# CILAB-MA/gpudrive_lab

Measured on AMD Instinct MI355X. Metric: agent-steps/sec at 1024 worlds x 64 agents; achieved HBM GB/s on obs kernel, higher is better.
Workload: dtype f32

## Files before the change

gpudrive_lab_amd/csrc/engine.cpp:

```cpp
#include <hip/hip_runtime.h>

#include <algorithm>
#include <cmath>
#include <cstdlib>
#include <cstdio>
#include <cstring>
#include <map>
#include <memory>
#include <stdexcept>
#include <atomic>
#include <exception>
#include <string>
#include <thread>
#include <vector>

#include "dev_mem.hpp"
#include "engine.hpp"
#include "gd_math.hpp"
#include "scene.hpp"
#ifdef GD_CLOCKS
namespace gd { void set_clocks_read(unsigned long long *out); void step_clocks_read(unsigned long long *out); }
#endif
#ifndef GD_GRID_MIN_CELL
#define GD_GRID_MIN_CELL 16.f
// ... 724 lines not shown
        d.pack_weights = rows ? weights : nullptr;
    }

    bool direct_pack_supported() const {
        if (params.disableClassicalObs) return false;
        if (params.roadObservationAlgorithm != GD_ROADS_K_NEAREST) return d.lin_on != 0;
        return true;
    }

    static void build_road_grid(WorldHost &world) {
        const std::vector<float> &xy = world.xy;
        const size_t n = xy.size() / 2;
        gd::GridHdr g{0.f, 0.f, 1.f, 1, 1, 0, 0, 0};
        std::vector<int32_t> off(2, 0);
        std::vector<uint16_t> items(n);
        if (n) {
            float minx = xy[0], maxx = xy[0], miny = xy[1], maxy = xy[1];
            for (size_t r = 1; r < n; r++) {
                minx = std::min(minx, xy[2 * r]); maxx = std::max(maxx, xy[2 * r]);
                miny = std::min(miny, xy[2 * r + 1]); maxy = std::max(maxy, xy[2 * r + 1]);
            }
            const float cell = std::max(GD_GRID_MIN_CELL, std::max(maxx - minx, maxy - miny) / 64.f + 1e-3f);
            g.ox = minx; g.oy = miny; g.inv_cell = 1.f / cell;
            g.nx = std::max(1, std::min(64, static_cast<int>((maxx - minx) * g.inv_cell) + 1));
            g.ny = std::max(1, std::min(64, static_cast<int>((maxy - miny) * g.inv_cell) + 1));
            const int nc = g.nx * g.ny;
            std::vector<int32_t> cell_of(n);
            off.assign(nc + 1, 0);
            for (size_t r = 0; r < n; r++) {
                const int cx = std::max(0, std::min(g.nx - 1, static_cast<int>((xy[2 * r] - g.ox) * g.inv_cell)));
                const int cy = std::max(0, std::min(g.ny - 1, static_cast<int>((xy[2 * r + 1] - g.oy) * g.inv_cell)));
                cell_of[r] = cy * g.nx + cx;
                off[cell_of[r] + 1]++;
            }
            for (int c = 0; c < nc; c++) off[c + 1] += off[c];
            std::vector<int32_t> fill(off.begin(), off.end() - 1);
            for (size_t r = 0; r < n; r++) items[fill[cell_of[r]]++] = static_cast<uint16_t>(r);
        }
        world.rgrid = g;
        world.rcell_off = std::move(off);
        world.rcell_items = std::move(items);
    }

    void upload_road_grids() {
        size_t ncell = 0, nitem = 0;
        std::vector<gd::GridHdr> hdr(W);
        for (int w = 0; w < W; w++) {
            world_host[w].rgrid.cell_base = static_cast<int>(ncell);
            world_host[w].rgrid.item_base = static_cast<int>(nitem);
            hdr[w] = world_host[w].rgrid;
            ncell += world_host[w].rcell_off.size();
            nitem += world_host[w].rcell_items.size();
        }
        rcell_off.fit(ncell, d.rcell_off);
        rcell_items.fit(nitem, d.rcell_items);
        rcell_xy.fit(nitem, d.rcell_xy);
        rcell_pos.fit(nitem, d.rcell_pos);
        std::vector<int32_t> co(ncell);
        std::vector<uint16_t> ci(nitem);
        std::vector<float> cxy(nitem * 2);
        std::vector<uint16_t> cpos(nitem);
        for (int w = 0; w < W; w++) {
            const WorldHost &x = world_host[w];
            std::copy(x.rcell_off.begin(), x.rcell_off.end(), co.begin() + hdr[w].cell_base);
            std::copy(x.rcell_items.begin(), x.rcell_items.end(), ci.begin() + hdr[w].item_base);
            for (size_t k = 0; k < x.rcell_items.size(); k++) {
                const size_t r = x.rcell_items[k], o = (static_cast<size_t>(hdr[w].item_base) + k) * 2;
                cxy[o] = x.xy[2 * r];
                cxy[o + 1] = x.xy[2 * r + 1];
                cpos[static_cast<size_t>(hdr[w].item_base) + r] = static_cast<uint16_t>(k);
            }
        }
        rcell_off.upload(co.data(), ncell);
        rcell_items.upload(ci.data(), nitem);
        rcell_xy.upload(cxy.data(), nitem);
        rcell_pos.upload(cpos.data(), nitem);
        HIP_CHECK(hipMemcpy(d_rgrid, hdr.data(), sizeof(gd::GridHdr) * W, hipMemcpyHostToDevice));
        std::vector<float> prev(static_cast<size_t>(W) * A * 4, 0.f);
        for (size_t i = 0; i < static_cast<size_t>(W) * A; i++) prev[i * 4 + 2] = INFINITY;
        HIP_CHECK(hipMemcpy(d.knn_prev, prev.data(), prev.size() * sizeof(float), hipMemcpyHostToDevice));
    }

    void reset_rank_state() {
        HIP_CHECK(hipMemset(d.cp_hdr, 0, sizeof(float4) * 2 * static_cast<size_t>(W) * A));
        HIP_CHECK(hipMemset(d.rk_fallback, 0, sizeof(int32_t) * (static_cast<size_t>(W) * A / 32)));
        HIP_CHECK(hipMemset(d.rk_streak, 0, sizeof(int32_t) * (static_cast<size_t>(W) * A / 32)));
        HIP_CHECK(hipMemset(d.rk_hist, 0, sizeof(int32_t) * GD_RANK_AUDIT));
        HIP_CHECK(hipMemset(d.rk_hist + GD_RH_LONG, 0, sizeof(int32_t) * (GD_RH_SIZE - GD_RH_LONG)));
    }

    void do_reset(const std::vector<int32_t> &flags) {
        upload_flags(d.reset_flags, flags);
        reset_flagged(false);
    }

    void reset_flagged(bool gated) {
        d.gate_any = gated ? 1 : 0;
        if (!gated) full_pass_next = false;
        try {
            launch(gd::KERNEL_RESET, false);
            run_rest(false);
        } catch (...) {
            d.gate_any = 0;
            throw;
        }
        d.gate_any = 0;
    }
};

namespace {

template <typename F>
int guarded(F &&f) {
    try {
        f();
        return GD_OK;
    } catch (const HipError &e) {
        return fail(GD_ERR_DEVICE, e.what());
    } catch (const std::invalid_argument &e) {
        const std::string m = e.what();
        return fail(m.find("cannot open") != std::string::npos ? GD_ERR_IO : GD_ERR_INVALID, m);
    } catch (const std::exception &e) {
        return fail(GD_ERR_PARSE, e.what());
    }
}

}

extern "C" {

const char *gd_version(void) { return "gpudrive_amd 0.1 (gfx950)"; }
const char *gd_last_error(void) { return g_last_error.c_str(); }

void gd_default_params(gd_params *p) {
    std::memset(p, 0, sizeof(*p));
    p->collisionBehaviour = GD_COLLISION_AGENT_STOP;
    p->maxNumControlledAgents = 10000;
    p->IgnoreNonVehicles = 0;
    p->roadObservationAlgorithm = GD_ROADS_K_NEAREST;
    p->initOnlyValidAgentsAtFirstStep = 1;
    p->isStaticAgentControlled = 0;
    p->dynamicsModel = GD_DYNAMICS_CLASSIC;
}

int gd_tensor_shape(int32_t id, int32_t W, int32_t A, gd_tensor_desc *out) {
    if (!out || id < 0 || id >= GD_T_COUNT || W < 1 || A < 2) return fail(GD_ERR_INVALID, "gd_tensor_shape: bad argument");
    const TensorSpec s = tensor_spec(id, W, A);
    out->data = nullptr;
    out->dtype = s.dtype;
    out->ndim = s.ndim;
    for (int i = 0; i < 5; i++) out->dims[i] = i < s.ndim ? s.dims[i] : 1;
    out->nbytes = spec_bytes(s);
    return GD_OK;
}

int gd_create(const gd_config *cfg, const gd_params *params, const char *const *scenes, gd_sim **out) {
    if (!cfg || !params || !scenes || !out) return fail(GD_ERR_INVALID, "gd_create: null argument");
    if (cfg->num_worlds < 1) return fail(GD_ERR_INVALID, "gd_create: num_worlds must be >= 1");
    if (cfg->max_agents != 64 && cfg->max_agents != 128)
        return fail(GD_ERR_INVALID, "gd_create: max_agents must be 64 or 128");
    if (params->rewardType == GD_REWARD_DENSE)
        return fail(GD_ERR_UNSUPPORTED, "RewardType::Dense is assert(false) in the reference (src/sim.cpp:579-583)");
    *out = nullptr;
    std::unique_ptr<gd_sim> s(new gd_sim());
    const int rc = guarded([&]() {
        int ndev = 0;
        HIP_CHECK(hipGetDeviceCount(&ndev));
        if (ndev < 1) throw HipError("no HIP device visible: the HIP path is mandatory, there is no CPU fallback");
        HIP_CHECK(hipSetDevice(cfg->device_id));
        s->cfg = *cfg;
        s->params = *params;
        s->W = cfg->num_worlds;
        s->A = cfg->max_agents;
        s->stream = static_cast<hipStream_t>(cfg->stream);
        const int W = s->W, A = s->A;
        for (int w = 0; w < W; w++) {
            if (!scenes[w]) throw std::invalid_argument("gd_create: null scene path");
            s->scenes.emplace_back(scenes[w]);
        }
        s->deleted.assign(static_cast<size_t>(W) * A, -1);
        s->world_host.resize(W);
        for (int id = 0; id < GD_T_COUNT; id++) {
            if (id == GD_T_BEV && !cfg->alloc_bev && !cfg->external[id]) continue;
            const int64_t bytes = spec_bytes(tensor_spec(id, W, A));
            if (!cfg->external[id]) s->exported_mem[id] = gd::DevMem(bytes);
            s->exported[id] = cfg->external[id] ? cfg->external[id] : s->exported_mem[id].get();
            HIP_CHECK(hipMemset(s->exported[id], 0, bytes));
        }
        gd::DevSim &d = s->d;
        d.W = W;
        d.A = A;
        d.p = *params;
        d.knn_order = cfg->knn_order;
        d.split_partner = (s->stream != nullptr && std::getenv("GPUDRIVE_SPLIT_PARTNER") != nullptr) ? 1 : 0;
        hipStream_t side = nullptr;
        HIP_CHECK(hipStreamCreateWithFlags(&side, hipStreamNonBlocking));
        s->side.reset(side);
        s->ev_fork = make_event(hipEventDisableTiming);
        s->ev_join = make_event(hipEventDisableTiming);
        d.step_dbg = 0;
#ifdef GD_DIAG
        if (const char *e = std::getenv("GPUDRIVE_STEP_DBG")) d.step_dbg = std::atoi(e);
#endif
        {
            (void)hipDeviceGetAttribute(&s->cu_count, hipDeviceAttributeMultiprocessorCount, cfg->device_id);
            d.set_fused_rows = 0;
            d.set_apw = 16;
        }
        d.lidar_half_angle = cfg->lidar_half_angle;
        {
            const float r = params->observationRadius;
            float k = r * r;
            while (k > 0.f && sqrtf(k) > r) k = std::nextafterf(k, 0.f);
            while (sqrtf(std::nextafterf(k, INFINITY)) <= r) k = std::nextafterf(k, INFINITY);
            d.radius_key_max = r >= 0.f ? k : -1.f;
        }
        d.action = static_cast<float *>(s->exported[GD_T_ACTION]);
        d.reward = static_cast<float *>(s->exported[GD_T_REWARD]);
        d.done = static_cast<int32_t *>(s->exported[GD_T_DONE]);
        d.info = static_cast<int32_t *>(s->exported[GD_T_INFO]);
        d.self_obs = static_cast<float *>(s->exported[GD_T_SELF_OBS]);
        d.abs_obs = static_cast<float *>(s->exported[GD_T_ABS_OBS]);
        d.partner = static_cast<float *>(s->exported[GD_T_PARTNER_OBS]);
        d.agent_map = static_cast<float *>(s->exported[GD_T_AGENT_MAP_OBS]);
        d.map_obs = static_cast<float *>(s->exported[GD_T_MAP_OBS]);
        d.lidar = static_cast<float *>(s->exported[GD_T_LIDAR]);
        d.bev = static_cast<float *>(s->exported[GD_T_BEV]);
        d.steps = static_cast<uint32_t *>(s->exported[GD_T_STEPS_REMAINING]);
        d.shape = static_cast<int32_t *>(s->exported[GD_T_SHAPE]);
        d.controlled = static_cast<int32_t *>(s->exported[GD_T_CONTROLLED_STATE]);
        d.resp_export = static_cast<int32_t *>(s->exported[GD_T_RESPONSE_TYPE]);
        d.traj = static_cast<float *>(s->exported[GD_T_EXPERT_TRAJECTORY]);
        d.means = static_cast<float *>(s->exported[GD_T_WORLD_MEANS]);
        d.metadata = static_cast<int32_t *>(s->exported[GD_T_METADATA]);
        d.deleted = static_cast<int32_t *>(s->exported[GD_T_DELETED_AGENTS]);
        d.map_name = static_cast<int32_t *>(s->exported[GD_T_MAP_NAME]);
        d.scenario_id = static_cast<int32_t *>(s->exported[GD_T_SCENARIO_ID]);
        const size_t WA = static_cast<size_t>(W) * A;
        d.px = s->alloc_internal<float>(WA); d.py = s->alloc_internal<float>(WA); d.pz = s->alloc_internal<float>(WA);
        d.qw = s->alloc_internal<float>(WA); d.qz = s->alloc_internal<float>(WA);
        d.vx = s->alloc_internal<float>(WA); d.vy = s->alloc_internal<float>(WA); d.vz = s->alloc_internal<float>(WA);
        d.collided = s->alloc_internal<int32_t>(WA);
        d.len = s->alloc_internal<float>(WA); d.wid = s->alloc_internal<float>(WA); d.hgt = s->alloc_internal<float>(WA);
        d.sc0 = s->alloc_internal<float>(WA); d.sc1 = s->alloc_internal<float>(WA);
        d.goal_x = s->alloc_internal<float>(WA); d.goal_y = s->alloc_internal<float>(WA);
        d.etype = s->alloc_internal<int32_t>(WA); d.agent_id = s->alloc_internal<int32_t>(WA);
        d.resp = s->alloc_internal<int32_t>(WA);
        d.sel_idx = s->alloc_internal<uint16_t>(static_cast<size_t>(WA) * GD_MAP_OBS_K);
        d.sel_hdr = s->alloc_internal<float4>(static_cast<size_t>(WA) * 2);
        d.sel_slot = s->alloc_internal<uint8_t>(static_cast<size_t>(WA) * GD_MAP_OBS_K);
        d.reset_flags = s->alloc_internal<int32_t>(W);
        d.rebuilt_flags = s->alloc_internal<int32_t>(W);
        d.any_reset = s->alloc_internal<int32_t>(1);
        d.gate_any = 0;
        d.road_off = s->d_road_off = s->alloc_internal<int32_t>(W + 1);
        d.live_list = s->alloc_internal<int32_t>(WA);
        d.live_count = 0;
        d.set_groups = s->alloc_internal<int32_t>(WA);
        d.set_group_count = 0;
        d.wave_order = s->alloc_internal<int32_t>(static_cast<size_t>(W) * (A / GD_MAP_OBS_AW));
        d.wave_cost = s->alloc_internal<uint32_t>(static_cast<size_t>(W) * (A / GD_MAP_OBS_AW));
        d.box_off = s->d_box_off = s->alloc_internal<int32_t>(W + 1);
        d.grid = s->d_grid = s->alloc_internal<gd::GridHdr>(W);
        d.rgrid = s->d_rgrid = s->alloc_internal<gd::GridHdr>(W);
        d.knn_prev = s->alloc_internal<float4>(WA);
        d.road_bbox = s->d_road_bbox = s->alloc_internal<float4>(W);
        d.road_rbmax = s->d_road_rbmax = s->alloc_internal<float>(W);
        d.bev_dirty = s->alloc_internal<int32_t>(WA);
        d.bev_list = s->alloc_internal<int32_t>(WA);
        d.bev_count = s->alloc_internal<int32_t>(2);
        d.bev_all_dirty = 0;
        HIP_CHECK(hipMemset(d.bev_dirty, 1, sizeof(int32_t) * WA));
        d.lidar_dirty = s->alloc_internal<int32_t>(WA);
        d.lidar_head = s->alloc_internal<float>(WA);
        HIP_CHECK(hipMemset(d.lidar_dirty, 1, sizeof(int32_t) * WA));
        HIP_CHECK(hipMemset(d.lidar_head, 0xff, sizeof(float) * WA));
        d.lin_apw = 2;
        if (const char *e = std::getenv("GPUDRIVE_LIN_AGENTS_PER_WAVE")) d.lin_apw = std::min(A / 4, std::max(1, std::atoi(e)));
        s->lin_cap = (static_cast<size_t>(W) + 64) * static_cast<size_t>(A) + 8 * 4 * static_cast<size_t>(d.lin_apw) + 64;
        s->d_lin_list = s->alloc_internal<int32_t>(s->lin_cap);
        s->d_lin_list_dyn = s->alloc_internal<int32_t>(s->lin_cap);
        d.lin_list = s->d_lin_list; d.lin_list_dyn = s->d_lin_list_dyn;
        d.lin_blocks = 0; d.lin_blocks_dyn = 0; d.lin_dyn_off = 0;
        d.lin_on = std::getenv("GPUDRIVE_LINEAR_LEGACY") == nullptr ? 1 : 0;
        d.pose_stamp = s->alloc_internal<uint4>(WA);
        d.pose_skip = std::getenv("GPUDRIVE_NO_POSE_SKIP") == nullptr ? 1 : 0;
        d.stat_skipped = s->alloc_internal<unsigned long long>(GD_SKIP_SLOTS);
        s->d_row_of_slot = s->alloc_internal<int32_t>(WA);
        s->d_slot_of_row = s->alloc_internal<int32_t>(WA);
        s->d_row_count = s->alloc_internal<int32_t>(1);
        d.bad_actions = s->alloc_internal<unsigned long long>(1);
        d.blk_off = s->d_blk_off = s->alloc_internal<int32_t>(W + 1);
        d.warm_k = 0;
        d.warm_all = 0;
        d.warm_flags = s->alloc_internal<int32_t>(W);
        d.warm_count = s->alloc_internal<unsigned long long>(1);
        d.rk_on = 0;
        d.rk_dbg = 0;
        d.rk_min_roads = 1536;
        d.rk_waves = 0;
        if (const char *e = std::getenv("GPUDRIVE_RANK_WAVES")) d.rk_waves = std::min(std::max((std::atoi(e) + 7) / 8 * 8, 8), GD_RANK_GRID);
        d.rk_scan_rows = 0;
        if (const char *e = std::getenv("GPUDRIVE_RANK_SCAN_ROWS")) d.rk_scan_rows = std::atoi(e) != 0 ? 1 : 0;
        d.rk_resident = std::max(gd::rank_resident_waves(A) / 8, 1);
        s->rk_possible = GD_MAP_OBS_AW == 32 && cfg->knn_order != GD_KNN_SET_ORDER &&
                         params->roadObservationAlgorithm == GD_ROADS_K_NEAREST && std::getenv("GPUDRIVE_NO_RANK_REPLAY") == nullptr;
#ifdef GD_DIAG
        if (const char *e = std::getenv("GPUDRIVE_RANK_DBG")) d.rk_dbg = std::atoi(e);
#endif
        for (int i = 0; i < gd_sim::kRing; i++) {
            void *pinned = nullptr;
            HIP_CHECK(hipHostMalloc(&pinned, sizeof(int32_t) * W, hipHostMallocDefault));
            s->h_flags[i].reset(static_cast<int32_t *>(pinned));
            s->flag_ev[i] = make_event(hipEventDisableTiming);
        }
        std::vector<int> all(W);
        for (int w = 0; w < W; w++) all[w] = w;
        s->rebuild_worlds(all);
        s->do_reset(std::vector<int32_t>(W, 1));
        HIP_CHECK(hipStreamSynchronize(s->stream));
    });
    if (rc != GD_OK) return rc;
    *out = s.release();
    return GD_OK;
}

void gd_destroy(gd_sim *sim) { delete sim; }

int gd_step(gd_sim *s) {
    if (!s) return fail(GD_ERR_INVALID, "gd_step: null sim");
    return guarded([&]() { s->step(); });
}

int gd_reset(gd_sim *s, const int32_t *idx, int32_t n) {
    if (!s || (n > 0 && !idx)) return fail(GD_ERR_INVALID, "gd_reset: bad argument");
    std::vector<int32_t> flags(s->W, 0);
    for (int i = 0; i < n; i++) {
        if (idx[i] < 0 || idx[i] >= s->W) return fail(GD_ERR_INVALID, "gd_reset: world index out of range");
        flags[idx[i]] = 1;
    }
    return guarded([&]() { s->do_reset(flags); });
}

int gd_set_maps(gd_sim *s, const char *const *scenes, int32_t n) {
    if (!s || !scenes) return fail(GD_ERR_INVALID, "gd_set_maps: null argument");
    if (n != s->W) return fail(GD_ERR_INVALID, "gd_set_maps: len(maps) must equal the number of worlds");
    const std::vector<std::string> old_scenes = s->scenes;
    const std::vector<int32_t> old_deleted = s->deleted;
    const int rc = guarded([&]() {
        for (int w = 0; w < n; w++) {
            if (!scenes[w]) throw std::invalid_argument("gd_set_maps: null scene path");
            s->scenes[w] = scenes[w];
        }
        std::fill(s->deleted.begin(), s->deleted.end(), -1);
        std::vector<int> all(s->W);
        for (int w = 0; w < s->W; w++) all[w] = w;
        s->rebuild_worlds(all);
        s->do_reset(std::vector<int32_t>(s->W, 1));
    });
    if (rc != GD_OK && rc != GD_ERR_DEVICE) {
        s->scenes = old_scenes;
        s->deleted = old_deleted;
    }
    return rc;
}

int gd_delete_agents(gd_sim *s, const int32_t *worlds, const int32_t *offsets, const int32_t *ids, int32_t nw) {
    if (!s || (nw > 0 && (!worlds || !offsets))) return fail(GD_ERR_INVALID, "gd_delete_agents: null argument");
    std::vector<int> touched;
    for (int i = 0; i < nw; i++) {
        const int w = worlds[i], cnt = offsets[i + 1] - offsets[i];
        if (w < 0 || w >= s->W) return fail(GD_ERR_INVALID, "gd_delete_agents: world index out of range");
        if (cnt < 0 || cnt > s->A) return fail(GD_ERR_INVALID, "gd_delete_agents: too many ids for one world");
    }
    return guarded([&]() {
        for (int i = 0; i < nw; i++) {
            const int w = worlds[i], cnt = offsets[i + 1] - offsets[i];
            for (int k = 0; k < cnt; k++) s->deleted[static_cast<size_t>(w) * s->A + k] = ids[offsets[i] + k];
            touched.push_back(w);
        }
        s->rebuild_worlds(touched);
        s->do_reset(std::vector<int32_t>(s->W, 1));
    });
}

int gd_tensor(gd_sim *s, int32_t id, gd_tensor_desc *out) {
    if (!s || !out || id < 0 || id >= GD_T_COUNT) return fail(GD_ERR_INVALID, "gd_tensor: bad argument");
    if (!s->exported[id]) return fail(GD_ERR_UNSUPPORTED, "tensor not allocated (set gd_config.alloc_bev for the BEV tensor)");
    gd_tensor_shape(id, s->W, s->A, out);
    out->data = s->exported[id];
    return GD_OK;
}

int gd_pack_observations(gd_sim *s, float *out, int64_t out_bytes) {
    if (!s || !out) return fail(GD_ERR_INVALID, "gd_pack_observations: null argument");
    const int64_t D = 6 + static_cast<int64_t>(s->A - 1) * 6 + GD_MAP_OBS_K * 13;
    const int64_t need = static_cast<int64_t>(s->W) * s->A * D * 4;
    if (out_bytes < need) return fail(GD_ERR_INVALID, "gd_pack_observations: output buffer too small");
    if (s->d.pack && s->d.pack_rows && s->d.pack_only)
        return fail(GD_ERR_UNSUPPORTED, "gd_pack_observations: learner rows are attached with only = 1: the raw rows are stale");
    return guarded([&]() {
        if (s->d.pack && !s->d.pack_rows) {
            if (out != s->d.pack) HIP_CHECK(hipMemcpyAsync(out, s->d.pack, need, hipMemcpyDeviceToDevice, s->stream));
            return;
        }
        gd::launch_pack_obs(s->d, s->stream, out);
        HIP_CHECK(hipGetLastError());
    });
}

int gd_attach_packed(gd_sim *s, float *out, int64_t out_bytes, int32_t only) {
    if (!s) return fail(GD_ERR_INVALID, "gd_attach_packed: null sim");
    const int64_t D = 6 + static_cast<int64_t>(s->A - 1) * 6 + GD_MAP_OBS_K * 13;
    if (out && out_bytes < static_cast<int64_t>(s->W) * s->A * D * 4)
        return fail(GD_ERR_INVALID, "gd_attach_packed: output buffer too small");
    if (out && !s->direct_pack_supported())
        return fail(GD_ERR_UNSUPPORTED, "gd_attach_packed: not available with disableClassicalObs or GPUDRIVE_LINEAR_LEGACY=1: use gd_pack_observations");
    return guarded([&]() {
        if (!out) s->detach_packed();
        else s->attach_packed(out, only != 0, false);
    });
}

int gd_set_learner_rows(gd_sim *s, const uint8_t *mask, int32_t n_rows) {
    if (!s) return fail(GD_ERR_INVALID, "gd_set_learner_rows: null sim");
    const size_t WA = static_cast<size_t>(s->W) * s->A;
    if (mask && (n_rows < 0 || static_cast<size_t>(n_rows) > WA))
        return fail(GD_ERR_INVALID, "gd_set_learner_rows: n_rows out of range");
    int32_t count = 0;
    const int rc = guarded([&]() {
        if (s->d.pack && s->d.pack_rows) s->detach_packed();
        HIP_CHECK(hipStreamSynchronize(s->stream));
        s->drop_graph();
        s->d.row_of_slot = nullptr;
        s->d.slot_of_row = nullptr;
        s->d.n_rows = 0;
        if (!mask) return;
        gd::launch_learner_rows(s->stream, mask, WA, s->d_row_of_slot, s->d_slot_of_row, s->d_row_count);
        HIP_CHECK(hipGetLastError());
        HIP_CHECK(hipMemcpyAsync(&count, s->d_row_count, sizeof(count), hipMemcpyDeviceToHost, s->stream));
        HIP_CHECK(hipStreamSynchronize(s->stream));
    });
    if (rc != GD_OK || !mask) return rc;
    if (count != n_rows) return fail(GD_ERR_INVALID, "gd_set_learner_rows: n_rows differs from the number of true slots of the mask");
    s->d.row_of_slot = s->d_row_of_slot;
    s->d.slot_of_row = s->d_slot_of_row;
    s->d.n_rows = count;
    return GD_OK;
}

int gd_attach_packed_rows(gd_sim *s, float *out, int64_t out_bytes, int32_t only) {
    if (!s || !out) return fail(GD_ERR_INVALID, "gd_attach_packed_rows: null argument (gd_attach_packed(sim, NULL, 0, 0) detaches)");
    if (!s->d.row_of_slot) return fail(GD_ERR_INVALID, "gd_attach_packed_rows: no learner rows set (gd_set_learner_rows)");
    const int64_t D = 6 + static_cast<int64_t>(s->A - 1) * 6 + GD_MAP_OBS_K * 13;
    if (out_bytes < static_cast<int64_t>(s->d.n_rows) * D * 4) return fail(GD_ERR_INVALID, "gd_attach_packed_rows: output buffer too small");
    if (!s->direct_pack_supported())
        return fail(GD_ERR_UNSUPPORTED, "gd_attach_packed_rows: not available with disableClassicalObs or GPUDRIVE_LINEAR_LEGACY=1");
    return guarded([&]() { s->attach_packed(out, only != 0, true); });
}

int gd_attach_packed_rows_conditioned(gd_sim *s, float *out, int64_t out_bytes, int32_t only, const float *weights) {
    if (!s || !out || !weights)
        return fail(GD_ERR_INVALID, "gd_attach_packed_rows_conditioned: null argument (gd_attach_packed(sim, NULL, 0, 0) detaches)");
    if (!s->d.row_of_slot) return fail(GD_ERR_INVALID, "gd_attach_packed_rows_conditioned: no learner rows set (gd_set_learner_rows)");
    const int64_t R = 6 + static_cast<int64_t>(s->A - 1) * 6 + GD_MAP_OBS_K * 13 + 3;
    if (out_bytes < static_cast<int64_t>(s->d.n_rows) * R * 4)
        return fail(GD_ERR_INVALID, "gd_attach_packed_rows_conditioned: output buffer too small");
    if (!s->direct_pack_supported())
        return fail(GD_ERR_UNSUPPORTED, "gd_attach_packed_rows_conditioned: not available with disableClassicalObs or GPUDRIVE_LINEAR_LEGACY=1");
    return guarded([&]() { s->attach_packed(out, only != 0, true, weights); });
}

int gd_set_discrete_actions(gd_sim *s, const int64_t *indices, const float *table, int32_t n_actions) {
    if (!s) return fail(GD_ERR_INVALID, "gd_set_discrete_actions: null sim");
    if (s->d.p.dynamicsModel == GD_DYNAMICS_STATE)
        return fail(GD_ERR_UNSUPPORTED, "gd_set_discrete_actions: the State dynamics model has no discrete action space");
    if (!s->d.row_of_slot) return fail(GD_ERR_INVALID, "gd_set_discrete_actions: no learner rows set (gd_set_learner_rows)");
    if (n_actions < 0 || (s->d.n_rows > 0 && (!indices || !table)))
        return fail(GD_ERR_INVALID, "gd_set_discrete_actions: bad argument");
    return guarded([&]() {
        gd::launch_discrete_actions(s->d, s->stream, indices, table, n_actions);
        HIP_CHECK(hipGetLastError());
    });
}

int gd_pack_observations_conditioned(gd_sim *s, const float *weights, float *out, int64_t out_bytes) {
    if (!s || !weights || !out) return fail(GD_ERR_INVALID, "gd_pack_observations_conditioned: null argument");
    const int64_t R = 6 + static_cast<int64_t>(s->A - 1) * 6 + GD_MAP_OBS_K * 13 + 3;
    if (out_bytes < static_cast<int64_t>(s->W) * s->A * R * 4)
        return fail(GD_ERR_INVALID, "gd_pack_observations_conditioned: output buffer too small");
    if (s->d.pack && s->d.pack_rows && s->d.pack_only)
        return fail(GD_ERR_UNSUPPORTED, "gd_pack_observations_conditioned: learner rows are attached with only = 1: the raw rows are stale");
    return guarded([&]() {
        gd::launch_pack_obs_conditioned(s->d, s->stream, weights, out);
        HIP_CHECK(hipGetLastError());
    });
}

int gd_expert_actions(gd_sim *s, float *actions, int32_t action_cols, float *pos_xy, float *vel_xy, float *yaw,
                      int32_t *valids) {
    if (!s) return fail(GD_ERR_INVALID, "gd_expert_actions: null sim");
    const int cols = s->d.p.dynamicsModel == GD_DYNAMICS_STATE ? 10 : 3;
    if (actions && action_cols != cols)
        return fail(GD_ERR_INVALID, "gd_expert_actions: action_cols does not match the dynamics model (10 for State, else 3)");
    return guarded([&]() {
        gd::launch_expert_actions(s->d, s->stream, actions, pos_xy, vel_xy, yaw, valids);
        HIP_CHECK(hipGetLastError());
    });
}

int gd_advance_log_playback(gd_sim *s, int32_t init_steps) {
    if (!s) return fail(GD_ERR_INVALID, "gd_advance_log_playback: null sim");
    if (init_steps < 0 || init_steps >= GD_EPISODE_LEN)
        return fail(GD_ERR_INVALID, "gd_advance_log_playback: the expert trajectory has 91 steps, init_steps must be < 91");
    return guarded([&]() {
        for (int t = 0; t < init_steps; t++) {
            gd::launch_set_log_actions(s->d, s->stream, t);
            HIP_CHECK(hipGetLastError());
            s->step();
        }
    });
}

int gd_record_expert(gd_sim *s, const gd_record_buffers *b, int32_t n_steps) {
    if (!s || !b) return fail(GD_ERR_INVALID, "gd_record_expert: null argument");
    if (!b->row_slot || !b->obs || !b->actions || !b->dead_mask || !b->partner_mask || !b->road_mask || !b->ego_global_pos ||
        !b->ego_global_rot || !b->dead || !b->goal_achieved || !b->off_road || !b->veh_collision || !b->any_alive)
        return fail(GD_ERR_INVALID, "gd_record_expert: every buffer is required");
    if (b->n_rows < 0) return fail(GD_ERR_INVALID, "gd_record_expert: n_rows must be >= 0");
    if (n_steps < 1 || n_steps > GD_EPISODE_LEN)
        return fail(GD_ERR_INVALID, "gd_record_expert: the expert trajectory has 91 steps, n_steps must be in [1, 91]");
    if (s->d.p.dynamicsModel == GD_DYNAMICS_STATE)
        return fail(GD_ERR_INVALID, "gd_record_expert: the State dynamics model's actions have 10 columns, the dataset's have 3");
    if (s->d.pack && s->d.pack_only)
        return fail(GD_ERR_UNSUPPORTED, "gd_record_expert: a packed buffer is attached with only = 1: the raw rows are stale");
    return guarded([&]() {
        std::vector<Event> ev;
        auto mark = [&]() {
            if (!b->kernel_ms) return;
            ev.push_back(make_event());
            HIP_CHECK(hipEventRecord(ev.back().get(), s->stream));
        };
        for (int t = 0; t <= n_steps; t++) {
            mark();
            gd::launch_record(s->d, s->stream, *b, t, t < n_steps);
            HIP_CHECK(hipGetLastError());
            mark();
            if (t == n_steps) break;
            gd::launch_set_log_actions(s->d, s->stream, t);
            HIP_CHECK(hipGetLastError());
            s->step();
        }
        if (b->kernel_ms) {
            HIP_CHECK(hipStreamSynchronize(s->stream));
            float sum = 0.f;
            for (size_t i = 0; i + 1 < ev.size(); i += 2) {
                float ms = 0.f;
                HIP_CHECK(hipEventElapsedTime(&ms, ev[i].get(), ev[i + 1].get()));
                sum += ms;
            }
            *b->kernel_ms = sum;
        }
    });
}

namespace {

const char *il_dataset_error(const gd_il_dataset *ds, int64_t *rows) {
    if (!ds) return "null argument";
    if (ds->max_agents != 64 && ds->max_agents != 128) return "max_agents must be 64 or 128";
    if (ds->rollout_len < 1 || ds->pred_len < 1 || ds->rollout_len + ds->pred_len > GD_EPISODE_LEN)
        return "rollout_len >= 1, pred_len >= 1 and rollout_len + pred_len <= 91 are required";
    if (ds->n_shards < 0 || ds->n_shards > GD_IL_MAX_SHARDS) return "0 to 8 shards";
    *rows = 0;
    for (int i = 0; i < ds->n_shards; i++) {
        const gd_il_shard &sh = ds->shard[i];
        if (sh.n_rows < 0) return "a shard's n_rows must be >= 0";
        if (!sh.obs || !sh.actions || !sh.dead_mask || !sh.partner_mask || !sh.road_mask || !sh.keep)
            return "every array of every shard is required";
        if (reinterpret_cast<uintptr_t>(sh.obs) % 16 != 0 || reinterpret_cast<uintptr_t>(sh.road_mask) % 8 != 0)
            return "obs must be 16-byte aligned and road_mask 8-byte aligned";
        *rows += sh.n_rows;
    }
    if (*rows > INT32_MAX / GD_EPISODE_LEN) return "too many rows";
    return nullptr;
}

}

int gd_il_index(const gd_il_dataset *ds, int32_t *counts, int32_t *kept, const int64_t *entry_offset, const int64_t *kept_ordinal,
                int32_t *entries, void *stream) {
    int64_t rows = 0;
    if (const char *e = il_dataset_error(ds, &rows)) return fail(GD_ERR_INVALID, std::string("gd_il_index: ") + e);
    if (entries ? (!entry_offset || !kept_ordinal) : (!counts || !kept))
        return fail(GD_ERR_INVALID, "gd_il_index: counts and kept (first launch) or entry_offset, kept_ordinal and entries "
                                    "(second launch) are required");
    return guarded([&]() {
        gd::launch_il_index(*ds, static_cast<hipStream_t>(stream), rows, counts, kept, entry_offset, kept_ordinal, entries);
        HIP_CHECK(hipGetLastError());
    });
}

int gd_il_batch(const gd_il_dataset *ds, const gd_il_batch_buffers *b, void *stream) {
    int64_t rows = 0;
    if (const char *e = il_dataset_error(ds, &rows)) return fail(GD_ERR_INVALID, std::string("gd_il_batch: ") + e);
    if (!b) return fail(GD_ERR_INVALID, "gd_il_batch: null argument");
// ... 700 lines not shown
        gd::launch_bc_train_rows(o, st, n, o.nll, o.actions, expert_actions, o.grad_nll);
        gd::launch_bc_backward(*p, *g, st, obs, partner_mask, road_mask, n, expert_actions, o.grad_nll, nullptr, o.grad);
        gd::launch_bc_adamw(o, st, o.grad);
        HIP_CHECK(hipGetLastError());
    });
}

int gd_bc_eval_accumulate(int32_t n, const float *nll, const float *actions, const float *expert_actions, float *acc, void *stream) {
    if (!nll || !actions || !expert_actions || !acc) return fail(GD_ERR_INVALID, "gd_bc_eval_accumulate: null argument");
    if (n < 1 || n > (1 << 20)) return fail(GD_ERR_INVALID, "gd_bc_eval_accumulate: n must be in [1, 2^20]");
    if (misaligned(nll, 4) || misaligned(actions, 4) || misaligned(expert_actions, 4) || misaligned(acc, 4))
        return fail(GD_ERR_INVALID, "gd_bc_eval_accumulate: float buffers must be 4-byte aligned");
    return guarded([&]() {
        gd::launch_bc_eval_accumulate(static_cast<hipStream_t>(stream), n, nll, actions, expert_actions, acc);
        HIP_CHECK(hipGetLastError());
    });
}

int gd_bc_hidden(const gd_bc_policy *p, const float *obs, const uint8_t *partner_mask, const uint8_t *road_mask, int32_t n, int32_t tap,
                 float *out, void *stream) {
    gd_bc_outputs none{};
    const char *why = bc_forward_problem(p, obs, partner_mask, road_mask, n, 1, nullptr, nullptr, nullptr, &none);
    if (!why && tap != GD_LP_TAP_FUSION && tap != GD_LP_TAP_RO) why = "tap must be GD_LP_TAP_FUSION or GD_LP_TAP_RO";
    if (!why && (!out || misaligned(out, 16))) why = "out is required, 16-byte aligned";
    if (why) return fail(GD_ERR_INVALID, std::string("gd_bc_hidden: ") + why);
    return guarded([&]() {
        gd::launch_bc_hidden(*p, static_cast<hipStream_t>(stream), obs, partner_mask, road_mask, n, tap, out);
        HIP_CHECK(hipGetLastError());
    });
}

static const char *lp_problem(const gd_bc_policy *p, const gd_lp_probe *lp, const float *obs, const uint8_t *partner_mask,
                              const uint8_t *road_mask, int32_t n, const uint8_t *mask, const int64_t *labels, const gd_lp_rows *rows,
                              int mode, const int32_t *acc) {
    if (!lp || !obs) return "null argument";
    if (lp->model < GD_LP_EARLY || lp->model > GD_LP_BASELINE) return "model must be GD_LP_EARLY, GD_LP_LATE or GD_LP_BASELINE";
    if (lp->exp != GD_IL_FUTURE_OTHER && lp->exp != GD_IL_FUTURE_EGO) return "exp must be GD_IL_FUTURE_OTHER or GD_IL_FUTURE_EGO";
    if (lp->reserved[0] != 0 || lp->reserved[1] != 0) return "reserved must be 0";
    if (lp->max_agents != 64 && lp->max_agents != 128) return "max_agents must be 64 or 128";
    if (lp->num_stack < 1 || lp->num_stack > 8) return "num_stack must be in [1, 8]";
    if (lp->model == GD_LP_BASELINE) {
        if (p) return "the baseline probe takes no policy";
        if (n < 1 || n > (1 << 20)) return "n must be in [1, 2^20]";
        if (misaligned(obs, 4)) return "float and int32 buffers must be 4-byte aligned";
        const int k = (lp->exp == GD_IL_FUTURE_OTHER ? 12 : 6) * lp->num_stack;
        if (k > 64) return "the baseline probe's in_features (12 num_stack for 'other') must not exceed 64";
        if (lp->in_features != k) return "in_features must be 6 num_stack ('ego') or 12 num_stack ('other') for the baseline probe";
    } else {
        gd_bc_outputs none{};
        if (const char *why = bc_forward_problem(p, obs, partner_mask, road_mask, n, 1, nullptr, nullptr, nullptr, &none)) return why;
        if (lp->max_agents != p->max_agents || lp->num_stack != p->num_stack) return "max_agents and num_stack must be the policy's";
        if (lp->in_features != 64) return "in_features must be 64 with a policy";
    }
    if (lp->num_partials < 1 || lp->num_partials > 4096) return "num_partials must be in [1, 4096]";
    if (!lp->packed || misaligned(lp->packed, 16)) return "packed is required, 16-byte aligned";
    if (rows && (misaligned(rows->logits, 16) || misaligned(rows->loss_row, 4) || misaligned(rows->pred, 8)))
        return "logits must be 16-byte aligned, loss_row 4-byte, pred 8-byte";
    if (mode == 0) {
        if (!rows || (!rows->logits && !rows->pred)) return "rows with logits or pred is required";
        if (rows->loss_row) return "loss_row needs labels (gd_lp_update, gd_lp_eval_accumulate)";
        return nullptr;
    }
    if (!mask || !labels || misaligned(labels, 8)) return "mask and labels are required, labels 8-byte aligned";
    if (!lp->part_f || !lp->part_d || !lp->part_i || misaligned(lp->part_f, 4) || misaligned(lp->part_d, 8) || misaligned(lp->part_i, 4))
        return "part_f, part_d and part_i are required (4-, 8- and 4-byte aligned)";
    if (misaligned(lp->stats, 4)) return "float and int32 buffers must be 4-byte aligned";
    if (mode == 2) return !acc || misaligned(acc, 8) ? "acc is required, 8-byte aligned" : nullptr;
    if (!(lp->beta1 >= 0.0 && lp->beta1 < 1.0) || !(lp->beta2 >= 0.0 && lp->beta2 < 1.0)) return "betas must be in [0, 1)";
    if (!(lp->eps > 0.f)) return "eps must be positive";
    if (!(lp->weight_decay >= 0.f) || !std::isfinite(lp->weight_decay)) return "weight_decay must be finite and not negative";
    if (!lp->weight || !lp->exp_avg || !lp->exp_avg_sq || !lp->lr || !lp->step || !lp->beta_pow || !lp->grad || !lp->stats || !lp->sums ||
        !lp->counts || !lp->scal)
        return "weight, exp_avg, exp_avg_sq, lr, step, beta_pow, grad, stats, sums, counts and scal are required";
    if (misaligned(lp->beta_pow, 8) || misaligned(lp->sums, 8) || misaligned(lp->weight, 4) || misaligned(lp->exp_avg, 4) ||
        misaligned(lp->exp_avg_sq, 4) || misaligned(lp->lr, 4) || misaligned(lp->step, 4) || misaligned(lp->grad, 4) ||
        misaligned(lp->counts, 4) || misaligned(lp->scal, 4))
        return "beta_pow and sums must be 8-byte aligned, the other buffers 4-byte aligned";
    return nullptr;
}

int gd_lp_forward(const gd_bc_policy *p, const gd_lp_probe *lp, const float *obs, const uint8_t *partner_mask, const uint8_t *road_mask,
                  int32_t n, const gd_lp_rows *rows, void *stream) {
    if (const char *why = lp_problem(p, lp, obs, partner_mask, road_mask, n, nullptr, nullptr, rows, 0, nullptr))
        return fail(GD_ERR_INVALID, std::string("gd_lp_forward: ") + why);
    return guarded([&]() {
        gd::launch_lp(p, *lp, static_cast<hipStream_t>(stream), obs, partner_mask, road_mask, n, nullptr, nullptr, rows, 0, nullptr);
        HIP_CHECK(hipGetLastError());
    });
}

int gd_lp_update(const gd_bc_policy *p, const gd_lp_probe *lp, const float *obs, const uint8_t *partner_mask, const uint8_t *road_mask,
                 int32_t n, const uint8_t *mask, const int64_t *labels, const gd_lp_rows *rows, void *stream) {
    if (const char *why = lp_problem(p, lp, obs, partner_mask, road_mask, n, mask, labels, rows, 1, nullptr))
        return fail(GD_ERR_INVALID, std::string("gd_lp_update: ") + why);
    return guarded([&]() {
        gd::launch_lp(p, *lp, static_cast<hipStream_t>(stream), obs, partner_mask, road_mask, n, mask, labels, rows, 1, nullptr);
        HIP_CHECK(hipGetLastError());
    });
}

int gd_lp_eval_accumulate(const gd_bc_policy *p, const gd_lp_probe *lp, const float *obs, const uint8_t *partner_mask,
                          const uint8_t *road_mask, int32_t n, const uint8_t *mask, const int64_t *labels, const gd_lp_rows *rows,
                          int32_t *acc, void *stream) {
    if (const char *why = lp_problem(p, lp, obs, partner_mask, road_mask, n, mask, labels, rows, 2, acc))
        return fail(GD_ERR_INVALID, std::string("gd_lp_eval_accumulate: ") + why);
    return guarded([&]() {
        gd::launch_lp(p, *lp, static_cast<hipStream_t>(stream), obs, partner_mask, road_mask, n, mask, labels, rows, 2, acc);
        HIP_CHECK(hipGetLastError());
    });
}

int gd_episode_step(gd_sim *s, const gd_episode_config *cfg, const gd_episode_buffers *b) {
    if (!s || !cfg || !b) return fail(GD_ERR_INVALID, "gd_episode_step: null argument");
    if (!b->controlled_mask || !b->agent_episode_returns || !b->episode_lengths || !b->collided_in_episode ||
        !b->offroad_in_episode || !b->live_agent_mask || !b->reward_out || !b->terminal_out || !b->truncated_out ||
        !b->mask_out || !b->done_worlds || !b->stats || !b->world_stats)
        return fail(GD_ERR_INVALID, "gd_episode_step: every buffer is required");
    if (cfg->reward_type < GD_EPISODE_REWARD_WEIGHTED || cfg->reward_type > GD_EPISODE_REWARD_LOG_DISTANCE)
        return fail(GD_ERR_INVALID, "gd_episode_step: unknown reward_type");
    if (cfg->reward_type == GD_EPISODE_REWARD_CONDITIONED && (!b->reward_weights || !b->weight_draws))
        return fail(GD_ERR_INVALID, "gd_episode_step: reward_conditioned needs reward_weights and weight_draws");
    if (cfg->reward_type == GD_EPISODE_REWARD_CONDITIONED &&
        (cfg->condition_mode < GD_CONDITION_RANDOM || cfg->condition_mode > GD_CONDITION_FIXED))
        return fail(GD_ERR_INVALID, "gd_episode_step: unknown condition_mode");
    if ((b->reward_rows || b->terminal_rows || b->truncated_rows || b->mask_rows) && !s->d.row_of_slot)
        return fail(GD_ERR_INVALID, "gd_episode_step: flat outputs need learner rows (gd_set_learner_rows)");
    return guarded([&]() {
        HIP_CHECK(hipMemsetAsync(s->d.any_reset, 0, sizeof(int32_t), s->stream));
        gd::launch_episode_step(s->d, s->stream, *cfg, *b);
        HIP_CHECK(hipGetLastError());
        if (cfg->auto_reset) s->reset_flagged(true);
    });
}

int gd_episode_set_warmup(gd_sim *s, int32_t init_steps, int32_t scope) {
    if (init_steps < 0 || init_steps >= GD_EPISODE_LEN)
        return fail(GD_ERR_INVALID, "gd_episode_set_warmup: init_steps must be in [0, 90] (the expert trajectory has 91 steps)");
    if (scope != GD_WARMUP_RESET_WORLDS && scope != GD_WARMUP_ALL_WORLDS)
        return fail(GD_ERR_INVALID, "gd_episode_set_warmup: unknown scope (GD_WARMUP_RESET_WORLDS or GD_WARMUP_ALL_WORLDS)");
    if (!s) return fail(GD_ERR_INVALID, "gd_episode_set_warmup: null sim");
    s->d.warm_k = init_steps;
    s->d.warm_all = scope == GD_WARMUP_ALL_WORLDS ? 1 : 0;
    return GD_OK;
}

int gd_episode_draw_weights(gd_sim *s, const gd_episode_config *cfg, const gd_episode_buffers *b, const int32_t *worlds,
                            int32_t n) {
    if (!s || !cfg || !b || !b->reward_weights || !b->weight_draws || (worlds && n < 0))
        return fail(GD_ERR_INVALID, "gd_episode_draw_weights: bad argument");
    if (cfg->condition_mode < GD_CONDITION_RANDOM || cfg->condition_mode > GD_CONDITION_FIXED)
        return fail(GD_ERR_INVALID, "gd_episode_draw_weights: unknown condition_mode");
    std::vector<int32_t> list;
    if (worlds) {
        list.assign(worlds, worlds + n);
        for (const int32_t w : list)
            if (w < 0 || w >= s->W) return fail(GD_ERR_INVALID, "gd_episode_draw_weights: world index out of range");
        std::sort(list.begin(), list.end());
        list.erase(std::unique(list.begin(), list.end()), list.end());
        if (list.empty()) return GD_OK;
    }
    return guarded([&]() {
        if (!worlds) {
            gd::launch_draw_weights(s->d, s->stream, *cfg, *b, nullptr, s->W);
            HIP_CHECK(hipGetLastError());
            return;
        }
        const gd::DevMem dl(list.size() * sizeof(int32_t));
        hipError_t e = hipMemcpyAsync(dl.get(), list.data(), list.size() * sizeof(int32_t), hipMemcpyHostToDevice, s->stream);
        if (e == hipSuccess) {
            gd::launch_draw_weights(s->d, s->stream, *cfg, *b, static_cast<const int32_t *>(dl.get()), static_cast<int>(list.size()));
            e = hipGetLastError();
        }
        const hipError_t es = hipStreamSynchronize(s->stream);
        HIP_CHECK(e);
        HIP_CHECK(es);
    });
}

int gd_sync(gd_sim *s) {
    if (!s) return fail(GD_ERR_INVALID, "gd_sync: null sim");
    return guarded([&]() { HIP_CHECK(hipStreamSynchronize(s->stream)); });
}

int gd_set_stream(gd_sim *s, void *stream) {
    if (!s) return fail(GD_ERR_INVALID, "gd_set_stream: null sim");
    return guarded([&]() {
        HIP_CHECK(hipStreamSynchronize(s->stream));
        s->drop_graph();
        HIP_CHECK(hipStreamSynchronize(s->side.get()));
        s->stream = static_cast<hipStream_t>(stream);
        s->d.split_partner = (s->stream != nullptr && std::getenv("GPUDRIVE_SPLIT_PARTNER") != nullptr) ? 1 : 0;
    });
}

int gd_attach_bev(gd_sim *s, float *bev) {
    if (!s || !bev) return fail(GD_ERR_INVALID, "gd_attach_bev: null argument");
    return guarded([&]() {
        if (s->d.bev && s->d.bev != bev) throw std::runtime_error("gd_attach_bev: a BEV tensor is already attached");
        HIP_CHECK(hipStreamSynchronize(s->stream));
        s->drop_graph();
        s->exported[GD_T_BEV] = bev;
        s->d.bev = bev;
        HIP_CHECK(hipMemsetAsync(s->d.bev_dirty, 1, sizeof(int32_t) * static_cast<size_t>(s->W) * s->A, s->stream));
        if (!s->params.disableClassicalObs) s->launch(gd::KERNEL_BEV, false);
    });
}

int gd_stat(gd_sim *s, int32_t which, int64_t *out) {
#ifdef GD_CLOCKS
    if (s && out && which >= 22 && which <= 29) {
        static unsigned long long clk[8];
        if (which == 22) gd::set_clocks_read(clk);
        *out = (int64_t)clk[which - 22];
        return GD_OK;
    }
#endif
#ifdef GD_CLOCKS
    if (s && out && which >= 32 && which <= 43) {
        static unsigned long long clk[12];
        if (which == 32) gd::step_clocks_read(clk);
        *out = (int64_t)clk[which - 32];
        return GD_OK;
    }
#endif
#ifdef GD_CLOCKS
    if (s && out && which >= 1000 && which < 1256) {
        *out = 0;
        if (s->rk_alloc) {
            int32_t v = 0;
            (void)hipStreamSynchronize(s->stream);
            if (hipMemcpy(&v, s->d.rk_hist + 256 + (which - 1000), sizeof(v), hipMemcpyDeviceToHost) != hipSuccess)
                return fail(GD_ERR_DEVICE, "gd_stat: reading the replay clocks failed");
            *out = v;
        }
        return GD_OK;
    }
#endif
#ifdef GD_WAVE_CLOCKS
    if (s && out && which >= 2000 && which < 2000 + 3 * GD_RANK_GRID) {
        *out = 0;
        if (s->rk_alloc) {
            int32_t v = 0;
            (void)hipStreamSynchronize(s->stream);
            if (hipMemcpy(&v, s->d.rk_hist + GD_RH_WAVES + (which - 2000), sizeof(v), hipMemcpyDeviceToHost) != hipSuccess)
                return fail(GD_ERR_DEVICE, "gd_stat: reading the ranking waves' clocks failed");
            *out = v;
        }
        return GD_OK;
    }
#endif
#if defined(GD_DIAG) || defined(GD_CLOCKS)
    constexpr int32_t kLastStat = 20;
#else
    constexpr int32_t kLastStat = 7;
#endif
    if (s && out && which == 30) {
        std::vector<unsigned long long> v(GD_SKIP_SLOTS, 0);
        (void)hipStreamSynchronize(s->stream);
        if (hipMemcpy(v.data(), s->d.stat_skipped, sizeof(unsigned long long) * v.size(), hipMemcpyDeviceToHost) != hipSuccess ||
            hipMemset(s->d.stat_skipped, 0, sizeof(unsigned long long) * v.size()) != hipSuccess)
            return fail(GD_ERR_DEVICE, "gd_stat: reading the skip counters failed");
        unsigned long long sum = 0;
        for (unsigned long long x : v) sum += x;
        *out = static_cast<int64_t>(sum) + s->host_skipped;
        s->host_skipped = 0;
        return GD_OK;
    }
    if (s && out && which == 31) {
        int32_t c = 0;
        (void)hipStreamSynchronize(s->stream);
        if (hipMemcpy(&c, s->d.bev_count, sizeof(c), hipMemcpyDeviceToHost) != hipSuccess)
            return fail(GD_ERR_DEVICE, "gd_stat: reading the raster count failed");
        *out = c;
        return GD_OK;
    }
    if (s && out && which == 44) {
        std::vector<int32_t> f(static_cast<size_t>(s->W) * s->A), n(static_cast<size_t>(s->W) * 2);
        (void)hipStreamSynchronize(s->stream);
        if (hipMemcpy(f.data(), s->d.lidar_dirty, sizeof(int32_t) * f.size(), hipMemcpyDeviceToHost) != hipSuccess ||
            hipMemcpy(n.data(), s->d.shape, sizeof(int32_t) * n.size(), hipMemcpyDeviceToHost) != hipSuccess)
            return fail(GD_ERR_DEVICE, "gd_stat: reading the LiDAR flags failed");
        int64_t c = 0;
        for (int w = 0; w < s->W; w++)
            for (int a = 0; a < n[static_cast<size_t>(w) * 2] && a < s->A; a++) c += f[static_cast<size_t>(w) * s->A + a] != 0;
        *out = c;
        return GD_OK;
    }
    if (s && out && which == 45) {
        unsigned long long v = 0;
        (void)hipStreamSynchronize(s->stream);
        if (hipMemcpy(&v, s->d.bad_actions, sizeof(v), hipMemcpyDeviceToHost) != hipSuccess)
            return fail(GD_ERR_DEVICE, "gd_stat: reading the action counter failed");
        *out = static_cast<int64_t>(v);
        return GD_OK;
    }
    if (s && out && which == 46) {
        unsigned long long v = 0;
        (void)hipStreamSynchronize(s->stream);
        if (hipMemcpy(&v, s->d.warm_count, sizeof(v), hipMemcpyDeviceToHost) != hipSuccess)
            return fail(GD_ERR_DEVICE, "gd_stat: reading the warm-up counter failed");
        *out = static_cast<int64_t>(v);
        return GD_OK;
    }
    if (s && out && which == 22) {
        *out = 0;
        if (s->rk_alloc) {
            int32_t v = 0;
            (void)hipStreamSynchronize(s->stream);
            if (hipMemcpy(&v, s->d.rk_hist + GD_RH_ROWS, sizeof(v), hipMemcpyDeviceToHost) != hipSuccess)
                return fail(GD_ERR_DEVICE, "gd_stat: reading the row counter failed");
            *out = v;
        }
        return GD_OK;
    }
    if (s && out && which == 21) {
        *out = 0;
        if (s->rk_alloc) {
            int32_t v = 0;
            (void)hipStreamSynchronize(s->stream);
            if (hipMemcpy(&v, s->d.rk_hist + GD_RANK_AUDIT, sizeof(v), hipMemcpyDeviceToHost) != hipSuccess)
                return fail(GD_ERR_DEVICE, "gd_stat: reading the audit counter failed");
            *out = v;
        }
        return GD_OK;
    }
    if (!s || !out || which < 0 || which > kLastStat) return fail(GD_ERR_INVALID, "gd_stat: bad argument");
#if defined(GD_DIAG) || defined(GD_CLOCKS)
    if (which >= 8) {
        *out = 0;
        if (s->rk_alloc) {
            int32_t v = 0;
            (void)hipStreamSynchronize(s->stream);
            (void)hipMemcpy(&v, s->d.rk_hist + 514 + (which - 8), sizeof(v), hipMemcpyDeviceToHost);
            (void)hipMemset(s->d.rk_hist + 514 + (which - 8), 0, sizeof(v));
            *out = v;
        }
        return GD_OK;
    }
#endif
    if (which == 7) {
        *out = s->d.rk_on;
        return GD_OK;
    }
    *out = which == 0 ? s->stat_graph_steps : which == 1 ? s->stat_plain_steps : which == 2 ? s->stat_captures
         : which == 3 ? s->d.set_fused_rows : which == 4 ? s->d.set_apw : which == 5 ? s->d.live_count : GD_MAP_OBS_AW;
    return GD_OK;
}

int gd_kernel_timing_enable(gd_sim *s, int32_t enable) {
    if (!s) return fail(GD_ERR_INVALID, "null sim");
    return guarded([&]() {
        HIP_CHECK(hipStreamSynchronize(s->stream));
        for (int k = 0; k < gd::KERNEL_TIMED; k++) {
            s->collect_timing(k);
            s->ev_ms[k] = 0;
            s->ev_launches[k] = 0;
            while (enable && s->ev_pool[k].size() < gd_sim::kEvRing) {
                s->ev_pool[k].push_back(EventPair{make_event(), make_event()});
            }
        }
        s->timing = enable != 0;
    });
}

int gd_kernel_timing_read(gd_sim *s, int32_t kernel, double *total_ms, int64_t *launches) {
    if (!s || kernel < 0 || kernel >= gd::KERNEL_TIMED) return fail(GD_ERR_INVALID, "gd_kernel_timing_read: bad argument");
    return guarded([&]() {
        HIP_CHECK(hipStreamSynchronize(s->stream));
        s->collect_timing(kernel);
        if (total_ms) *total_ms = s->ev_ms[kernel];
        if (launches) *launches = s->ev_launches[kernel];
    });
}

int gd_debug_get_state(gd_sim *s, float *out) {
    if (!s || !out) return fail(GD_ERR_INVALID, "null argument");
    return guarded([&]() {
        HIP_CHECK(hipStreamSynchronize(s->stream));
        const size_t WA = static_cast<size_t>(s->W) * s->A;
        std::vector<float> plane(WA);
        std::vector<int32_t> iplane(WA);
        const float *src[8] = {s->d.px, s->d.py, s->d.pz, s->d.qw, s->d.qz, s->d.vx, s->d.vy, s->d.vz};
        const int dstcol[8] = {0, 1, 2, 3, 6, 7, 8, 9};
        for (size_t i = 0; i < WA * 11; i++) out[i] = 0.f;
        for (int k = 0; k < 8; k++) {
            HIP_CHECK(hipMemcpy(plane.data(), src[k], WA * 4, hipMemcpyDeviceToHost));
            for (size_t i = 0; i < WA; i++) out[i * 11 + dstcol[k]] = plane[i];
        }
        for (size_t i = 0; i < WA; i++) {
            out[i * 11 + 4] = 0.f * out[i * 11 + 6];
            out[i * 11 + 5] = 0.f * out[i * 11 + 6];
        }
        HIP_CHECK(hipMemcpy(iplane.data(), s->d.collided, WA * 4, hipMemcpyDeviceToHost));
        for (size_t i = 0; i < WA; i++) out[i * 11 + 10] = static_cast<float>(iplane[i]);
    });
}

int gd_debug_road_path(gd_sim *s, int32_t *out) {
    if (!s || !out) return fail(GD_ERR_INVALID, "null argument");
    return guarded([&]() {
        HIP_CHECK(hipStreamSynchronize(s->stream));
        const size_t WA = static_cast<size_t>(s->W) * s->A;
        if (!s->rk_alloc || !s->d.rk_on) {
            for (size_t i = 0; i < WA; i++) out[i] = -2;
            return;
        }
        HIP_CHECK(hipMemcpy(out, s->d.rk_n, WA * sizeof(int32_t), hipMemcpyDeviceToHost));
        std::vector<int32_t> why(WA);
        HIP_CHECK(hipMemcpy(why.data(), s->d.rk_ticket, WA * sizeof(int32_t), hipMemcpyDeviceToHost));
        for (size_t i = 0; i < WA; i++) {
            if (out[i] > 0) out[i] = out[i] == (1 << 30) ? -3 : (out[i] & 0xffff);
            else if (out[i] == -1 && why[i] < -1) out[i] = -10 + (why[i] + 2);
            else if (out[i] == -1 && why[i] >= 0 && ((why[i] >> 30) & 1)) out[i] = -12;
        }
    });
}

int gd_debug_set_state(gd_sim *s, const float *in) {
    if (!s || !in) return fail(GD_ERR_INVALID, "null argument");
    return guarded([&]() {
        HIP_CHECK(hipStreamSynchronize(s->stream));
        const size_t WA = static_cast<size_t>(s->W) * s->A;
        std::vector<float> plane(WA);
        std::vector<int32_t> iplane(WA);
        float *dst[8] = {s->d.px, s->d.py, s->d.pz, s->d.qw, s->d.qz, s->d.vx, s->d.vy, s->d.vz};
        const int srccol[8] = {0, 1, 2, 3, 6, 7, 8, 9};
        for (int k = 0; k < 8; k++) {
            for (size_t i = 0; i < WA; i++) plane[i] = in[i * 11 + srccol[k]];
            HIP_CHECK(hipMemcpy(dst[k], plane.data(), WA * 4, hipMemcpyHostToDevice));
        }
        for (size_t i = 0; i < WA; i++) iplane[i] = in[i * 11 + 10] != 0.f;
        HIP_CHECK(hipMemcpy(s->d.collided, iplane.data(), WA * 4, hipMemcpyHostToDevice));
        s->full_pass_next = (s->params.roadObservationAlgorithm != GD_ROADS_K_NEAREST && s->d.lin_on != 0) || s->d.bev != nullptr ||
                            (s->d.lidar != nullptr && s->params.enableLidar);
    });
}

int gd_host_world_build(const char *scene, const gd_params *params, int32_t A, const int32_t *deleted, int32_t ndel,
                        gd_host_world *out) {
    if (!scene || !params || !out || A < 2 || A > GD_MAX_AGENTS_LIMIT) return fail(GD_ERR_INVALID, "gd_host_world_build: bad argument");
    std::memset(out, 0, sizeof(*out));
    return guarded([&]() {
        auto map = gd::load_scene(scene, params->polylineReductionThreshold);
        gd::HostWorld hw;
        gd::build_host_world(*map, *params, A, deleted, ndel, hw);
        out->num_agents = hw.num_agents;
        out->num_roads = hw.num_roads;
        out->num_collidable_roads = static_cast<int32_t>(hw.boxes.size());
        out->max_agents = A;
        std::memcpy(out->mean, hw.mean, sizeof(hw.mean));
        std::memcpy(out->map_name, hw.map_name, sizeof(hw.map_name));
        std::memcpy(out->scenario_id, hw.scenario_id, sizeof(hw.scenario_id));
        auto dupf = [](const std::vector<float> &v, size_t n) {
            float *p = static_cast<float *>(std::calloc(std::max<size_t>(n, 1), sizeof(float)));
            std::memcpy(p, v.data(), std::min(n, v.size()) * sizeof(float));
            return p;
        };
        auto dupi = [](const std::vector<int32_t> &v) {
            int32_t *p = static_cast<int32_t *>(std::calloc(std::max<size_t>(v.size(), 1), sizeof(int32_t)));
            std::memcpy(p, v.data(), v.size() * sizeof(int32_t));
            return p;
        };
        out->map_obs = dupf(hw.map_obs, static_cast<size_t>(GD_MAX_ROAD_ENTITIES) * 9);
        for (int r = hw.num_roads; r < GD_MAX_ROAD_ENTITIES; r++) { out->map_obs[r * 9 + 7] = -1.f; out->map_obs[r * 9 + 8] = -1.f; }
        out->trajectory = dupf(hw.trajectory, hw.trajectory.size());
        out->vehicle_size = dupf(hw.size, hw.size.size());
        out->goal = dupf(hw.goal, hw.goal.size());
        out->controlled = dupi(hw.controlled);
        out->response_type = dupi(hw.resp);
        out->agent_id = dupi(hw.agent_id);
        out->entity_type = dupi(hw.etype);
        out->metadata = dupi(hw.metadata);
    });
}

int gd_scene_cache_write(const char *scene, float polyline_reduction_threshold, const char *out_path) {
    if (!scene || !out_path) return fail(GD_ERR_INVALID, "gd_scene_cache_write: null argument");
    if (!gd::is_scene_cache_path(out_path)) return fail(GD_ERR_INVALID, "gd_scene_cache_write: the cache path must end in .gdsm");
    return guarded([&]() {
        auto map = gd::load_scene(scene, polyline_reduction_threshold);
        gd::write_scene_cache(*map, polyline_reduction_threshold, out_path);
    });
}

void gd_host_world_free(gd_host_world *w) {
    if (!w) return;
    std::free(w->map_obs); std::free(w->trajectory); std::free(w->vehicle_size); std::free(w->goal);
    std::free(w->controlled); std::free(w->response_type); std::free(w->agent_id); std::free(w->entity_type);
    std::free(w->metadata);
    std::memset(w, 0, sizeof(*w));
}

}
```

gpudrive_lab_amd/csrc/engine.hpp:

```cpp
#pragma once
#include <hip/hip_runtime.h>

#include <cstdint>

#include "../../include/gpudrive_amd.h"

#ifndef GD_MAP_OBS_AW
#define GD_MAP_OBS_AW 32
#endif

#define GD_RANK_CAP 1280
#define GD_RANK_NCP 40
#define GD_RANK_HEAP_DW 104
#define GD_RANK_CAP_LONG 2560
#define GD_RANK_KT_LONG 164
#define GD_RH_LONG 537
#define GD_RH_ROWS 538
#define GD_RH_CURSOR 544
#define GD_RH_CURSOR_STRIDE 32
#define GD_RH_SIZE (GD_RH_CURSOR + 8 * GD_RH_CURSOR_STRIDE)
#define GD_RANK_GRID (256 * 8 * 4)
#ifdef GD_CLOCKS
#define GD_WAVE_CLOCKS
#endif
#ifdef GD_WAVE_CLOCKS
#define GD_RH_WAVES GD_RH_SIZE
#define GD_RH_ALLOC (GD_RH_WAVES + 3 * GD_RANK_GRID)
#else
#define GD_RH_ALLOC GD_RH_SIZE
#endif
#define GD_RK_REC_ROW (1 << 16)
#define GD_RANK_NCH 320
#define GD_RANK_SPL 256
#define GD_RANK_KT 84
#define GD_RANK_AUDIT 536
#define GD_LIN_BLK 16
#define GD_SKIP_SLOTS 4096

#ifdef GD_DIAG
#define GD_DIAG_IS(field, value) ((field) == (value))
#else
#define GD_DIAG_IS(field, value) false
#endif

namespace gd {

enum { KERNEL_STATE = 0, KERNEL_MAP_OBS = 1, KERNEL_LIDAR = 2, KERNEL_BEV = 3, KERNEL_PARTNER = 4, KERNEL_RESET = 5, KERNEL_PADDING = 6, KERNEL_TIMED = 5 };

struct GridHdr {
    float ox, oy, inv_cell;
    int nx, ny;
    int cell_base;
    int item_base;
    int pad;
};

struct DevSim {
    int W, A;
    int knn_order;
    int set_fused_rows;
    int32_t *live_list;
    int live_count;
    int32_t *set_groups;
    int set_group_count;
    int set_apw;
    float lidar_half_angle;
    float radius_key_max;
    gd_params p;
    float *action, *reward, *self_obs, *abs_obs, *partner, *agent_map, *map_obs, *lidar, *bev, *traj, *means;
    int32_t *done, *info, *shape, *controlled, *resp_export, *metadata, *deleted, *map_name, *scenario_id;
    uint32_t *steps;
    float *px, *py, *pz, *qw, *qz, *vx, *vy, *vz;
    int32_t *collided;
    float *len, *wid, *hgt, *sc0, *sc1, *goal_x, *goal_y;
    int32_t *etype, *agent_id, *resp;
    uint16_t *sel_idx;
    float4 *sel_hdr;
    uint8_t *sel_slot;
    int32_t *reset_flags, *rebuilt_flags;
    int32_t *any_reset;
    int gate_any;
    const int32_t *road_off;
    int32_t *wave_order;
    uint32_t *wave_cost;
    const float2 *road_xy;
    const float4 *road_aux;
    const float4 *road_rec;
    const int32_t *box_off;
    const float4 *boxes;
    const GridHdr *grid;
    const int32_t *cell_off;
    const int32_t *cell_items;
    const float4 *cell_hdr;
    const GridHdr *rgrid;
    const int32_t *rcell_off;
    const uint16_t *rcell_items;
    const float2 *rcell_xy;
    const uint16_t *rcell_pos;
    float4 *knn_prev;
    const int32_t *lin_list, *lin_list_dyn;
    int lin_blocks, lin_blocks_dyn;
    int lin_dyn_off;
    const float4 *road_blk;
    const int32_t *blk_off;
    int lin_apw;
    int lin_on;
    uint4 *pose_stamp;
    int pose_skip;
    int32_t *bev_dirty;
    int32_t *bev_list;
    int32_t *bev_count;
    int bev_all_dirty;
    int32_t *lidar_dirty;
    float *lidar_head;
    float *pack;
    int pack_only;
    const int32_t *row_of_slot, *slot_of_row;
    int n_rows;
    int pack_rows;
    unsigned long long *bad_actions;
    unsigned long long *stat_skipped;
    int split_partner;
    int step_dbg;
    int rk_on;
    int rk_max_roads;
    int rk_min_roads;
    int rk_dbg;
    uint16_t *rk_E;
    int rk_nlong;
    int32_t *rk_longlist;
    int32_t *rk_longslot;
    uint16_t *rk_E_long;
    float *rk_kt_long;
    uint16_t *rk_spc;
    float *rk_kt;
    uint32_t *rk_heap;
    uint16_t *rk_cpe;
    int32_t *rk_hist;
    int rk_waves;
    int32_t *rk_ticket;
    int32_t *rk_order;
    int32_t *rk_list;
    uint16_t *rk_cpf;
    float *rk_cpt;
    float4 *rk_rec;
    int rk_scan_rows;
    int rk_resident;
    const float4 *road_bbox;
    const float *road_rbmax;
    int32_t *rk_n;
    int32_t *rk_fallback;
    int32_t *rk_streak;
    uint16_t *cp_road;
    float *cp_T;
    float4 *cp_hdr;
    int warm_k;
    int warm_all;
    int32_t *warm_flags;
    unsigned long long *warm_count;
    const float *pack_weights;
};

void launch_kernel(const DevSim &d, hipStream_t st, int which, bool move);
void launch_map_obs(const DevSim &d, hipStream_t st, bool move);
void launch_map_obs_rank(const DevSim &d, hipStream_t st);
int rank_resident_waves(int A);
void launch_map_obs_linear(const DevSim &d, hipStream_t st, bool move);
void launch_bev(const DevSim &d, hipStream_t st);
void launch_lidar(const DevSim &d, hipStream_t st);
void launch_pack_obs(const DevSim &d, hipStream_t st, float *out);
void launch_expert_actions(const DevSim &d, hipStream_t st, float *actions, float *pos, float *vel, float *yaw, int *valid);
void launch_set_log_actions(const DevSim &d, hipStream_t st, int t);
void launch_episode_step(const DevSim &d, hipStream_t st, const gd_episode_config &c, const gd_episode_buffers &b);
void launch_draw_weights(const DevSim &d, hipStream_t st, const gd_episode_config &c, const gd_episode_buffers &b,
                         const int32_t *worlds, int n);
void launch_pack_obs_rows(const DevSim &d, hipStream_t st, float *out,
                          const float *weights);
void launch_learner_rows(hipStream_t st, const uint8_t *mask, size_t slots, int32_t *row_of_slot, int32_t *slot_of_row,
                         int32_t *count);
void launch_discrete_actions(const DevSim &d, hipStream_t st, const int64_t *indices, const float *table, int n_actions);
void launch_pack_obs_conditioned(const DevSim &d, hipStream_t st, const float *weights, float *out);
void launch_record(const DevSim &d, hipStream_t st, const gd_record_buffers &b, int t, bool pre);
void launch_bc_rollout_row(const DevSim &d, hipStream_t st, const gd_bc_rollout_buffers &b, int t, int num_stack);
void launch_bc_rollout_actions(const DevSim &d, hipStream_t st, const gd_bc_rollout_buffers &b, int t);
void launch_bc_rollout_post(const DevSim &d, hipStream_t st, const gd_bc_rollout_buffers &b, int t, bool more);
void launch_bc_rollout_summary(hipStream_t st, const gd_bc_rollout_buffers &b);
void launch_policy_rollout_actions(const DevSim &d, hipStream_t st, const gd_policy_rollout_buffers &b, int t);
void launch_policy_rollout_book(const DevSim &d, hipStream_t st, const gd_policy_rollout_buffers &b, int t);
void launch_policy_rollout_finish(const DevSim &d, hipStream_t st, const gd_policy_rollout_buffers &b, int n_steps);
void launch_il_index(const gd_il_dataset &ds, hipStream_t st, int64_t rows, int32_t *counts, int32_t *kept,
                     const int64_t *entry_offset, const int64_t *kept_ordinal, int32_t *entries);
void launch_il_batch(const gd_il_dataset &ds, hipStream_t st, const gd_il_batch_buffers &b,
                     int split);
void launch_il_future(const gd_il_dataset &ds, const gd_il_future &fu, hipStream_t st, const gd_il_future_buffers &b,
                      int split);
void launch_rollout_store(const gd_rollout &ro, hipStream_t st, const float *obs, const float *value, const int64_t *action,
                          const float *logprob, const float *reward, const uint8_t *done, const uint8_t *mask,
                          bool streaming);
void launch_rollout_sort(const gd_rollout &ro, hipStream_t st, const int64_t *offset, int64_t *idxs);
void launch_rollout_gae(const gd_rollout &ro, hipStream_t st, const int64_t *idxs, float gamma, float gae_lambda, float *delta,
                        float *coef, float *adv);
void launch_rollout_gather(const gd_rollout &ro, hipStream_t st, const gd_rollout_batch &b);
long long policy_blob_floats(int ego_width, int n_actions);
void launch_policy_forward(const gd_policy &p, hipStream_t st, const float *obs, const float *u, bool deterministic,
                           int64_t *actions, float *logprob, float *entropy, float *value, float *logits_out);
void launch_policy_evaluate(const gd_policy &p, hipStream_t st, const float *obs, const int64_t *actions, unsigned char *winners,
                            float *logprob, float *entropy, float *value);
void launch_policy_forward(const gd_policy &p, const gd_dropout &d, hipStream_t st, const float *obs, const float *u,
                           bool deterministic, int64_t *actions, float *logprob, float *entropy, float *value,
                           float *logits_out);
void launch_policy_evaluate(const gd_policy &p, const gd_dropout &d, hipStream_t st, const float *obs, const int64_t *actions,
                            unsigned char *winners, float *logprob, float *entropy, float *value);
void launch_policy_forward_rows(const gd_policy &p, const gd_dropout *d, hipStream_t st, const float *obs, const float *u,
                                bool deterministic, int64_t *actions, float *logprob, float *entropy, float *value,
                                float *logits_out, const int32_t *rows, const int32_t *count);
void launch_live_rows(hipStream_t st, const uint8_t *mask, int n, int32_t *rows, int32_t *count, int32_t *scratch,
                      int32_t *count_copy);
void launch_policy_backward(const gd_policy &p, const gd_policy_grad &g, const gd_dropout &d, hipStream_t st, const float *obs,
                            const int64_t *actions, const float *d_logprob, const float *d_entropy, const float *d_value,
                            float *grad);
long long policy_grad_floats(int ego_width, int n_actions);
void launch_policy_backward(const gd_policy &p, const gd_policy_grad &g, hipStream_t st, const float *obs, const int64_t *actions,
                            const float *d_logprob, const float *d_entropy, const float *d_value, float *grad);
void launch_ppo_loss(const gd_ppo &o, hipStream_t st, const float *newlogprob, const float *entropy, const float *newvalue,
                     const float *old_logprob, const float *old_value, const float *adv, const float *ret, float *d_logprob,
                     float *d_entropy, float *d_value);
void launch_ppo_adam(const gd_ppo &o, hipStream_t st, const float *grad);
long long bc_blob_floats(int num_stack, int fusion_layers, int branch_layers, int head_layers, int n_components);
long long bc_scratch_floats(int max_agents, int chunk_rows);
void launch_bc_forward(const gd_bc_policy &p, hipStream_t st, const float *obs, const unsigned char *partner_mask,
                       const unsigned char *road_mask, int n, bool deterministic, const float *u, const float *z,
                       const float *expert_actions, const gd_bc_outputs &out);
void launch_bc_eval_accumulate(hipStream_t st, int n, const float *nll, const float *actions, const float *expert_actions,
                               float *acc);
void launch_bc_embed(const gd_bc_policy &p, hipStream_t st, const float *obs, int rows, float *X);
void launch_bc_self_layer(const gd_bc_policy &p, hipStream_t st, const unsigned char *pm, const unsigned char *rm, int rows,
                          int layer, float *X, float *Kb, float *Vb, float *osave, float *ml);
void launch_bc_cross_kv(const gd_bc_policy &p, hipStream_t st, int rows, const float *X, float *Kb, float *Vb);
void launch_bc_head(const gd_bc_policy &p, hipStream_t st, const unsigned char *partner_mask, const unsigned char *road_mask, int r0,
                    int rows, bool deterministic, const float *u, const float *z, const float *expert_actions,
                    const gd_bc_outputs &out, const float *X, const float *Kb, const float *Vb);
long long bc_grad_floats(int num_stack, int fusion_layers, int branch_layers, int head_layers, int n_components);
long long bc_grad_scratch_floats(int max_agents, int chunk_rows, int fusion_layers, int branch_layers, long long blob_floats);
void launch_bc_backward(const gd_bc_policy &p, const gd_bc_grad &g, hipStream_t st, const float *obs, const unsigned char *partner_mask,
                        const unsigned char *road_mask, int n, const float *expert_actions, const float *grad_nll, float *nll,
                        float *grad);
int bc_num_tensors(int fusion_layers, int branch_layers, int head_layers);
void launch_bc_train_rows(const gd_bc_opt &o, hipStream_t st, int n, const float *nll, const float *actions,
                          const float *expert_actions, float *grad_nll);
void launch_bc_adamw(const gd_bc_opt &o, hipStream_t st, const float *grad);
void launch_bc_hidden(const gd_bc_policy &p, hipStream_t st, const float *obs, const unsigned char *partner_mask,
                      const unsigned char *road_mask, int n, int tap, float *out);
void launch_lp(const gd_bc_policy *p, const gd_lp_probe &lp, hipStream_t st, const float *obs, const unsigned char *partner_mask,
               const unsigned char *road_mask, int n, const unsigned char *mask, const int64_t *labels, const gd_lp_rows *rows_out,
               int mode, int *acc);

}
```

gpudrive_lab_amd/csrc/kernels.hip:

```cpp
#include <hip/hip_runtime.h>

#include "engine.hpp"
#include "expert.hpp"
#include "gd_math.hpp"
#include "map_rows.hpp"
#include "pack_cols.hpp"

namespace gd {

namespace {

constexpr int K = GD_MAP_OBS_K;
constexpr int TRAJ = GD_TRAJECTORY_FLOATS;
constexpr int EPISODE = GD_EPISODE_LEN;

__device__ __forceinline__ int current_step(uint32_t t) {
    long long k = (long long)EPISODE - (long long)t;
    if (k < 0 || k > EPISODE) k = EPISODE;
    return (int)k;
}

struct Body {
    float px, py, pz, qw, qz, vx, vy, vz;
};

__device__ __forceinline__ void forward_classic(const float *act, float length, Body &b) {
    const float maxSpeed = FLT_MAX;
    const float dt = 0.1f;
    const float speed = len_3(b.vx, b.vy, b.vz);
    const float yaw = quat_to_yaw(quat_from_wz(b.qw, b.qz));
    const float v = fmaxf(fminf(speed + 0.5f * act[0] * dt, maxSpeed), -maxSpeed);
    const float tanDelta = p_tan(act[1]);
    const float beta = p_atan(0.5f * tanDelta);
    float sn, cs;
    p_sincos(yaw + beta, sn, cs);
    const float dx = v * cs, dy = v * sn;
    const float w = v * p_cos(beta) * tanDelta / length;
    const float new_yaw = angle_add(yaw, w * dt);
    const float new_speed = fmaxf(fminf(speed + act[0] * dt, maxSpeed), -maxSpeed);
    b.px += dx * dt;
    b.py += dy * dt;
    b.pz = 1.f;
    p_sincos(new_yaw / 2.f, b.qz, b.qw);
    p_sincos(new_yaw, sn, cs);
    b.vx = new_speed * cs;
    b.vy = new_speed * sn;
    b.vz = 0.f;
}

__device__ __forceinline__ void forward_bicycle(float *act, Body &b) {
    act[0] = fmaxf(-6.0f, fminf(act[0], 6.0f));
    act[1] = fmaxf(-3.0f, fminf(act[1], 3.0f));
    const float dt = 0.1f;
    const float yaw = quat_to_yaw(quat_from_wz(b.qw, b.qz));
    const float speed = len_3(b.vx, b.vy, b.vz);
    float sn, cs;
    p_sincos(yaw, sn, cs);
    b.px = (float)((double)(b.px + b.vx * dt) + 0.5 * act[0] * cs * dt * dt);
    b.py = (float)((double)(b.py + b.vy * dt) + 0.5 * act[0] * sn * dt * dt);
    const float delta_yaw = (float)(act[1] * ((double)(speed * dt) + 0.5 * act[0] * dt * dt));
    const float new_yaw = angle_add(yaw, delta_yaw);
    const float new_speed = speed + act[0] * dt;
    p_sincos(new_yaw, sn, cs);
    b.vx = new_speed * cs;
    b.vy = new_speed * sn;
    b.vz = 0.f;
    p_sincos(new_yaw / 2.f, b.qz, b.qw);
}

__device__ __forceinline__ void forward_delta(const float *act, Body &b) {
    const float dt = 0.1f;
    const float yaw = quat_to_yaw(quat_from_wz(b.qw, b.qz));
    float c, s;
    p_sincos(yaw, s, c);
    const float dx = act[0] * c - act[1] * s;
    const float dy = act[0] * s + act[1] * c;
    b.px = b.px + dx;
    b.py = b.py + dy;
    b.vx = dx / dt;
    b.vy = dy / dt;
    b.vz = 0.f;
    const float new_yaw = angle_add(yaw, act[2]);
    p_sincos(new_yaw / 2.f, b.qz, b.qw);
}

__device__ __forceinline__ void forward_state(const float *act, Body &b) {
    b.px = act[0]; b.py = act[1]; b.pz = act[2];
    b.vx = act[4]; b.vy = act[5]; b.vz = act[6];
    p_sincos(act[3] / 2.f, b.qz, b.qw);
}

__device__ __forceinline__ void reset_agent(const DevSim &d, size_t i) {
    const float *t = d.traj + i * TRAJ;
    d.px[i] = t[0];
    d.py[i] = t[1];
    d.pz[i] = 1.f;
    const float heading = t[4 * 91];
    d.qw[i] = p_cos(heading / 2.f);
    d.qz[i] = p_sin(heading / 2.f);
    const bool is_static = d.resp[i] == RESP_Static;
    d.vx[i] = is_static ? 0.f : t[2 * 91 + 0];
    d.vy[i] = is_static ? 0.f : t[2 * 91 + 1];
    d.vz[i] = 0.f;
    float *act = d.action + i * 10;
#pragma unroll
    for (int k = 0; k < 10; k++) act[k] = 0.f;
    if (d.p.dynamicsModel == GD_DYNAMICS_STATE) act[2] = 1.f;
    d.steps[i] = EPISODE;
    d.done[i] = 0;
    d.reward[i] = 0.f;
    int32_t *info = d.info + i * 5;
    info[0] = 0; info[1] = 0; info[2] = 0; info[3] = 0;
    info[4] = d.etype[i];
    d.resp_export[i] = d.resp[i];
    d.collided[i] = 0;
}

template <int A_T>
__global__ __launch_bounds__(A_T) void k_reset_worlds(DevSim d) {
    const int w = blockIdx.x, a = threadIdx.x;
    if (d.reset_flags[w] == 0) return;
    const int n = d.shape[w * 2 + 0];
    const size_t i = (size_t)w * A_T + a;
    if (a < n) reset_agent(d, i);
    __syncthreads();
    if (a == 0) d.reset_flags[w] = 0;
}

template <int A_T>
__global__ __launch_bounds__(A_T) void k_init_padding_rows(DevSim d) {
    const int w = blockIdx.x;
    if (d.rebuilt_flags[w] == 0) return;
    const int n = d.shape[w * 2 + 0];
    const int npad = A_T - n;
    for (int a = n + threadIdx.x; a < A_T; a += blockDim.x) {
        const size_t i = (size_t)w * A_T + a;
        d.steps[i] = 0;
        d.done[i] = 1;
        d.reward[i] = 0.f;
        int32_t *info = d.info + i * 5;
        info[0] = 0; info[1] = 0; info[2] = 0; info[3] = 0; info[4] = ET_None;
        d.resp_export[i] = RESP_Static;
        d.collided[i] = 0;
        float *so = d.self_obs + i * 8;
        so[0] = 0; so[1] = 0; so[2] = 0; so[3] = 0; so[4] = 0; so[5] = 0; so[6] = 0; so[7] = -1.f;
    }
    {
        float *base = d.partner + ((size_t)w * A_T + n) * (A_T - 1) * 9;
        const int total = npad * (A_T - 1) * 9;
        for (int e = threadIdx.x; e < total; e += blockDim.x) {
            const int c = e % 9;
            base[e] = c == 8 ? -1.f : 0.f;
        }
    }
    {
        float *base = d.agent_map + ((size_t)w * A_T + n) * K * 9;
        const int total = npad * K * 9;
        for (int e = threadIdx.x; e < total; e += blockDim.x) {
            const int c = e % 9;
            base[e] = c >= 7 ? -1.f : 0.f;
        }
    }
    __syncthreads();
    if (threadIdx.x == 0) d.rebuilt_flags[w] = 0;
}

constexpr int STEP_THREADS = 256;

#ifdef GD_CLOCKS
__device__ unsigned long long g_step_clk[8];
__device__ unsigned long long g_step_cnt[4];
#define STEP_PHASE(n) do { if (a == 0) { const unsigned long long t_ = __builtin_amdgcn_s_memtime(); atomicAdd(&g_step_clk[n], t_ - clk_prev); clk_prev = t_; } } while (0)
#else
#define STEP_PHASE(n) do {} while (0)
#endif

__device__ __forceinline__ void partner_row(float *o, const DevSim &d, int ego, int k, const float *s_px, const float *s_py, const float *s_qw,
                                            const float *s_qz, const float *s_speed, const float *s_len, const float *s_wid,
                                            const float *s_hgt, const int *s_etype, const int *s_id) {
    const int j = k < ego ? k : k + 1;
    const float ew = s_qw[ego], ez = s_qz[ego];
    const V2 r = rotate_yaw(ew, -ez, s_px[j] - s_px[ego], s_py[j] - s_py[ego]);
    if (r.x * r.x + r.y * r.y > d.radius_key_max) {
        o[0] = 0; o[1] = 0; o[2] = 0; o[3] = 0; o[4] = 0; o[5] = 0; o[6] = 0; o[7] = (float)ET_None; o[8] = -1.f;
        return;
    }
    const float rw = s_qw[j], rz = s_qz[j], iz = -ez;
    const float pw = ew * rw - iz * rz, pz = ew * rz + iz * rw;
    const float wz = pw * pz;
    float heading;
    if (wz != 0.f) heading = atan2f(2.0f * wz, 1.0f - 2.0f * (pz * pz));
    else heading = quat_to_yaw_row(quat_mul(quat_inv(quat_from_wz(ew, ez)), quat_from_wz(rw, rz)));
    o[0] = s_speed[j];
    o[1] = r.x; o[2] = r.y;
    o[3] = heading;
    o[4] = s_len[j]; o[5] = s_wid[j]; o[6] = s_hgt[j];
    o[7] = (float)s_etype[j];
    o[8] = (float)s_id[j];
}

template <int A_T>
__device__ __forceinline__ void partner_rows(const DevSim &d, int w, int n, int a, const float *s_px, const float *s_py,
                                             const float *s_qw, const float *s_qz, const float *s_speed, const float *s_len,
                                             const float *s_wid, const float *s_hgt, const int *s_etype, const int *s_id,
                                             bool write_const, float *s_rows) {
    float *base = d.partner + (size_t)w * A_T * (A_T - 1) * 9;
    typedef float f4 __attribute__((ext_vector_type(4)));
    if (!write_const && n < A_T) {
        const int m = n - 1;
        const int rows = n * m;
        for (int p0 = 0; p0 < rows; p0 += STEP_THREADS) {
            if (GD_DIAG_IS(d.step_dbg, 3)) break;
            const int p = p0 + a;
            if (p < rows) {
                const int ego = p / m;
                partner_row(s_rows + a * 9, d, ego, p - ego * m, s_px, s_py, s_qw, s_qz, s_speed, s_len, s_wid, s_hgt, s_etype, s_id);
            }
            __syncthreads();
            const int nf = min(STEP_THREADS, rows - p0) * 9;
            for (int f = a; f < nf; f += STEP_THREADS) {
                const int gf = p0 * 9 + f, ego = gf / (m * 9);
                __builtin_nontemporal_store(s_rows[f], base + (size_t)ego * (A_T - 1) * 9 + (gf - ego * m * 9));
            }
            __syncthreads();
        }
        return;
    }
    const int rows = n * (A_T - 1);
    for (int p0 = 0; p0 < rows; p0 += STEP_THREADS) {
        if (GD_DIAG_IS(d.step_dbg, 3)) break;
        const int p = p0 + a;
        if (p < rows) {
            const int ego = p / (A_T - 1), k = p - ego * (A_T - 1);
            float *o = s_rows + a * 9;
            if (k >= n - 1) {
                o[0] = 0; o[1] = 0; o[2] = 0; o[3] = 0; o[4] = 0; o[5] = 0; o[6] = 0; o[7] = (float)ET_None; o[8] = -2.f;
            } else {
                partner_row(o, d, ego, k, s_px, s_py, s_qw, s_qz, s_speed, s_len, s_wid, s_hgt, s_etype, s_id);
            }
        }
        __syncthreads();
        const int nf = min(STEP_THREADS, rows - p0) * 9;
        float *out = base + (size_t)p0 * 9;
        for (int q = a; q * 4 < nf; q += STEP_THREADS) {
            if (q * 4 + 4 <= nf) {
                __builtin_nontemporal_store(*reinterpret_cast<const f4 *>(s_rows + q * 4), reinterpret_cast<f4 *>(out + q * 4));
            } else {
                for (int e = q * 4; e < nf; e++) out[e] = s_rows[e];
            }
        }
        __syncthreads();
    }
}


template <int A_T, bool ROWS, bool COND = false>
__device__ __forceinline__ void packed_head(const DevSim &d, int w, int n, int a, const float *s_px, const float *s_py,
                                            const float *s_qw, const float *s_qz, const float *s_speed, const float *s_len,
                                            const float *s_wid, const float *s_self) {
    static_assert(ROWS || !COND, "the conditioned layout exists for the learner rows only");
    constexpr int D = 6 + (A_T - 1) * 6 + K * 13, PITCH = COND ? D + 3 : D;
    __shared__ __attribute__((aligned(16))) float s_head[STEP_THREADS / 64][COND ? 64 * 6 + 4 : 64 * 6];
    const int wave = a >> 6, lane = a & 63;
    float *stage = s_head[wave];
    typedef float f4 __attribute__((ext_vector_type(4)));
    for (int ego = wave; ego < n; ego += STEP_THREADS / 64) {
        size_t prow = (size_t)w * A_T + ego;
        if (ROWS) {
            const int r = d.row_of_slot[prow];
            if (r < 0) continue;
            prow = (size_t)r;
        }
        float *out = d.pack + prow * PITCH;
#pragma unroll
        for (int h = 0; h < A_T / 64; h++) {
            const int r = h * 64 + lane;
            float *o = stage + lane * 6 + (COND && h == 0 && lane > 0 ? 3 : 0);
            if (r == 0) {
#pragma unroll
                for (int c = 0; c < 6; c++) o[c] = pack_ego_col(s_self + ego * 8, c);
                if (COND) {
                    const float *wt = d.pack_weights + ((size_t)w * A_T + ego) * 3;
                    o[6] = wt[0]; o[7] = wt[1]; o[8] = wt[2];
                }
            } else {
                const int k = r - 1;
                float raw[6] = {0.f, 0.f, 0.f, 0.f, 0.f, 0.f};
                if (k < n - 1) {
                    const int j = k < ego ? k : k + 1;
                    const float ew = s_qw[ego], ez = s_qz[ego];
                    const V2 rel = rotate_yaw(ew, -ez, s_px[j] - s_px[ego], s_py[j] - s_py[ego]);
                    if (!(rel.x * rel.x + rel.y * rel.y > d.radius_key_max)) {
                        const float rw = s_qw[j], rz = s_qz[j], iz = -ez;
                        const float pw = ew * rw - iz * rz, pz = ew * rz + iz * rw;
                        const float wz = pw * pz;
                        float heading;
                        if (wz != 0.f) heading = atan2f(2.0f * wz, 1.0f - 2.0f * (pz * pz));
                        else heading = quat_to_yaw_row(quat_mul(quat_inv(quat_from_wz(ew, ez)), quat_from_wz(rw, rz)));
                        raw[0] = s_speed[j]; raw[1] = rel.x; raw[2] = rel.y; raw[3] = heading; raw[4] = s_len[j]; raw[5] = s_wid[j];
                    }
                }
                pack_partner_row(raw, o);
            }
            wave_sync();
            if (COND) {
                store_span(stage, out + (h == 0 ? 0 : h * (64 * 6) + 3), h == 0 ? 64 * 6 + 3 : 64 * 6, lane, 64);
            } else {
                for (int q = lane; q < 64 * 6 / 4; q += 64)
                    __builtin_nontemporal_store(*reinterpret_cast<const f4 *>(stage + q * 4), reinterpret_cast<f4 *>(out + h * (64 * 6) + q * 4));
            }
            wave_sync();
        }
    }
}

enum { WS_STEP = 0, WS_WARMUP = 1, WS_AFTER_WARMUP = 2 };

template <int A_T, bool MOVE, bool ROWS = false, int MODE = WS_STEP, bool COND = false>
__global__ __launch_bounds__(STEP_THREADS) void k_world_step(DevSim d) {
    constexpr bool OBS = MODE != WS_WARMUP;
    const int w = blockIdx.x, a = threadIdx.x;
    if (!MOVE && d.gate_any && *d.any_reset == 0) return;
    const int n = d.shape[w * 2 + 0];
    const size_t i = (size_t)w * A_T + a;
    const bool live = a < n;
    const GridHdr gh = d.grid[w];
    const int bbase = d.box_off[w];

    __shared__ float s_px[A_T], s_py[A_T], s_qw[A_T], s_qz[A_T], s_speed[A_T];
    __shared__ float s_len[A_T], s_wid[A_T], s_hgt[A_T], s_rad[A_T];
    __shared__ int s_etype[A_T], s_id[A_T], s_flags[A_T];
    __shared__ float s_obb[14][A_T];
    __shared__ int s_hit[A_T];
    __shared__ float s_self[A_T * 8];
    __shared__ __attribute__((aligned(16))) float s_stage[STEP_THREADS * 9];
    float *const s_opx = s_stage, *const s_opy = s_stage + A_T;
    unsigned long long *const s_moved = reinterpret_cast<unsigned long long *>(s_stage + 2 * A_T);
    constexpr int SVCAP = 6 * STEP_THREADS;
    static_assert(SVCAP <= STEP_THREADS * 9 && 3 * A_T <= STEP_THREADS * 9, "the staging buffer holds each of its tenants");
    unsigned int *const s_sv = reinterpret_cast<unsigned int *>(s_stage);
    __shared__ int s_nsv[2];
    __shared__ int s_c0[A_T], s_coff[A_T], s_wtot[A_T / 64];

#ifdef GD_CLOCKS
    unsigned long long clk_prev = __builtin_amdgcn_s_memtime();
    if (a == 0) atomicAdd(&g_step_clk[7], 1ull);
#endif
    int first = 0, last = 1;
    bool skip_collision = false;
    if (MODE == WS_WARMUP) {
        const bool flagged = d.reset_flags[w] != 0;
        const bool warm = flagged || d.warm_all != 0;
        if (flagged && live) reset_agent(d, i);
        __syncthreads();
        if (a == 0) {
            d.warm_flags[w] = warm ? 1 : 0;
            if (flagged) d.reset_flags[w] = 0;
            if (warm) atomicAdd(d.warm_count, 1ull);
        }
        if (!warm) return;
        first = -1;
        last = d.warm_k;
    }
    if (MODE == WS_AFTER_WARMUP) skip_collision = d.warm_flags[w] != 0;
    int it = first;
    do {
        const bool moving = MODE == WS_WARMUP ? it >= 0 : MOVE;
        if (MODE == WS_WARMUP && moving && a < A_T) {
            const int model = d.p.dynamicsModel;
            float act[10];
            expert_action(d.traj + i * TRAJ, it, model, act);
            const int cols = model == GD_DYNAMICS_STATE ? 10 : 3;
            for (int c = 0; c < cols; c++) d.action[i * 10 + c] = act[c];
        }
        Body b{};
        int collided = 0, done = 0, resp = RESP_Static, controlled = 0, etype = 0;
        uint32_t steps = 0;
        int32_t info0 = 0, info1 = 0, info2 = 0, info3 = 0;
        float sc0 = 0.f, sc1 = 0.f, length = 0.f, width = 0.f, height = 0.f, gx = 0.f, gy = 0.f;

        if (a < A_T) {
            b.px = d.px[i]; b.py = d.py[i]; b.pz = d.pz[i];
            b.qw = d.qw[i]; b.qz = d.qz[i];
            b.vx = d.vx[i]; b.vy = d.vy[i]; b.vz = d.vz[i];
            collided = d.collided[i];
            done = d.done[i];
            resp = d.resp[i];
            controlled = d.controlled[i];
            etype = d.etype[i];
            steps = d.steps[i];
            const int32_t *info = d.info + i * 5;
            info0 = info[0]; info1 = info[1]; info2 = info[2]; info3 = info[3];
            sc0 = d.sc0[i]; sc1 = d.sc1[i];
            length = d.len[i]; width = d.wid[i]; height = d.hgt[i];
            gx = d.goal_x[i]; gy = d.goal_y[i];
        }

#ifdef GD_CLOCKS
        asm volatile("s_waitcnt vmcnt(0)" ::: "memory");
#endif
        STEP_PHASE(0);
        if (moving && live) {
            if (collided) {
                if (d.p.collisionBehaviour == GD_COLLISION_AGENT_STOP) {
                    done = 1;
                    b.vx = 0.f; b.vy = 0.f; b.vz = 0.f;
                } else if (d.p.collisionBehaviour == GD_COLLISION_AGENT_REMOVED) {
                    done = 1;
                    b.px = kPadX; b.py = kPadY; b.pz = kPadZ;
                    b.vx = 0.f; b.vy = 0.f; b.vz = 0.f;
                } else {
                    collided = 0;
                    info0 = 0; info1 = 0; info2 = 0;
                }
            }
            if (resp != RESP_Static) {
                if (done) {
                    b.px = kPadX; b.py = kPadY; b.pz = kPadZ;
                    b.vx = 0.f; b.vy = 0.f; b.vz = 0.f;
                } else if (controlled) {
                    float act[10];
                    float *ap = d.action + i * 10;
#pragma unroll
                    for (int k = 0; k < 10; k++) act[k] = ap[k];
                    switch (d.p.dynamicsModel) {
                    case GD_DYNAMICS_INVERTIBLE_BICYCLE:
                        forward_bicycle(act, b);
                        ap[0] = act[0];
                        ap[1] = act[1];
                        break;
                    case GD_DYNAMICS_DELTA_LOCAL: forward_delta(act, b); break;
                    case GD_DYNAMICS_STATE: forward_state(act, b); break;
                    default: forward_classic(act, length, b); break;
                    }
                } else {
                    const float *t = d.traj + i * TRAJ;
                    const int k = current_step(steps);
                    b.px = t[2 * k]; b.py = t[2 * k + 1]; b.pz = 1.f;
                    b.vx = t[2 * 91 + 2 * k]; b.vy = t[2 * 91 + 2 * k + 1]; b.vz = 0.f;
                    const float heading = t[4 * 91 + k];
                    p_sincos(heading / 2.f, b.qz, b.qw);
                }
            }
        }

        STEP_PHASE(1);
        bool active = false, moved = false;
        const bool track_moves = OBS && (d.bev != nullptr || (d.lidar != nullptr && d.p.enableLidar != 0));
        float theta = 0.f;
        if (a < A_T) s_hit[a] = 0;
        if (live) {
            theta = quat_to_yaw(quat_from_wz(b.qw, b.qz));
            bool invalid;
            if (!controlled) {
                const float *t = d.traj + i * TRAJ;
                invalid = !(t[5 * 91 + current_step(steps)] != 0.f);
            } else {
                invalid = done && !collided;
            }
            active = !skip_collision && !(b.pz == kPadZ) && !invalid;
            s_px[a] = b.px; s_py[a] = b.py; s_qw[a] = b.qw; s_qz[a] = b.qz;
            s_speed[a] = len_3(b.vx, b.vy, b.vz);
            s_len[a] = length; s_wid[a] = width; s_hgt[a] = height;
            s_etype[a] = etype;
            s_id[a] = d.agent_id[i];
            s_rad[a] = sqrtf(sc0 * sc0 + sc1 * sc1);
            s_flags[a] = (active ? 1 : 0) | (resp == RESP_Static ? 2 : 0);
            if (track_moves) {
                const float old_px = d.px[i], old_py = d.py[i], old_pz = d.pz[i], old_qw = d.qw[i], old_qz = d.qz[i];
                s_opx[a] = old_px; s_opy[a] = old_py;
                moved = __float_as_uint(old_px) != __float_as_uint(b.px) || __float_as_uint(old_py) != __float_as_uint(b.py) ||
                        __float_as_uint(old_pz) != __float_as_uint(b.pz) ||
                        __float_as_uint(old_qw) != __float_as_uint(b.qw) || __float_as_uint(old_qz) != __float_as_uint(b.qz);
            }
            if (active) {
                const Obb o = obb_from_yaw(b.px, b.py, theta, sc0, sc1);
                const float *of = reinterpret_cast<const float *>(&o);
#pragma unroll
                for (int k = 0; k < 14; k++) s_obb[k][a] = of[k];
            }
        }
        if (track_moves && a < A_T) {
            const unsigned long long mv = __ballot(moved);
            if ((a & 63) == 0) s_moved[a >> 6] = mv;
        }
        __syncthreads();
        STEP_PHASE(2);
        if (OBS && d.bev != nullptr && live) {
            int dirty = (!moving || d.pose_skip == 0 || d.bev_all_dirty != 0 || moved) ? 1 : 0;
            if (!dirty) {
                const float rr = d.p.observationRadius * 1.001f + 0.05f, r2 = rr * rr;
                const float mx = s_px[a], my = s_py[a];
#pragma unroll
                for (int h = 0; h < A_T / 64; h++) {
                    for (unsigned long long m = s_moved[h]; m != 0ull && !dirty; m &= m - 1ull) {
                        const int j = h * 64 + __ffsll((long long)m) - 1;
                        const float dx = s_px[j] - mx, dy = s_py[j] - my, ox = s_opx[j] - mx, oy = s_opy[j] - my;
                        if (!(dx * dx + dy * dy > r2) || !(ox * ox + oy * oy > r2)) dirty = 1;
                    }
                }
            }
            d.bev_dirty[i] = dirty;
        }
        if (OBS && d.lidar != nullptr && d.p.enableLidar != 0 && live) {
            const float head = controlled ? d.action[i * 10 + 2] : 0.f;
            int dirty = (!moving || d.pose_skip == 0 || d.bev_all_dirty != 0 || moved || __float_as_uint(head) != __float_as_uint(d.lidar_head[i])) ? 1 : 0;
            if (!dirty) {
                const float mx = s_px[a], my = s_py[a];
#pragma unroll
                for (int h = 0; h < A_T / 64; h++) {
                    for (unsigned long long m = s_moved[h]; m != 0ull && !dirty; m &= m - 1ull) {
                        const int j = h * 64 + __ffsll((long long)m) - 1;
                        const float rr = (200.f + s_rad[j]) * 1.001f + 0.1f, r2 = rr * rr;
                        const float dx = s_px[j] - mx, dy = s_py[j] - my, ox = s_opx[j] - mx, oy = s_opy[j] - my;
                        if (!(dx * dx + dy * dy > r2) || !(ox * ox + oy * oy > r2)) dirty = 1;
                    }
                }
            }
            d.lidar_dirty[i] = dirty;
        }

        {
            constexpr int P = STEP_THREADS / A_T;
            const int ag = a % A_T, part = a / A_T;
            const int my_fl = ag < n ? s_flags[ag] : 0;
            if (my_fl & 1) {
                Obb me;
                {
                    float *mf = reinterpret_cast<float *>(&me);
#pragma unroll
                    for (int k = 0; k < 14; k++) mf[k] = s_obb[k][ag];
                }
                const float mx = s_px[ag], my = s_py[ag], my_rad = s_rad[ag];
                const int my_type = s_etype[ag];
                const bool me_static = (my_fl & 2) != 0;
                int hit = 0;
                for (int j = part; j < n; j += P) {
                    if (GD_DIAG_IS(d.step_dbg, 2)) break;
                    if (j == ag) continue;
                    const int fl = s_flags[j];
                    if (!(fl & 1)) continue;
                    if (me_static && (fl & 2)) continue;
                    const float dx = mx - s_px[j], dy = my - s_py[j];
                    const float rr = (my_rad + s_rad[j]) * 1.001f + 0.01f;
                    if (dx * dx + dy * dy > rr * rr) continue;
                    Obb ot;
                    float *of = reinterpret_cast<float *>(&ot);
#pragma unroll
                    for (int k = 0; k < 14; k++) of[k] = s_obb[k][j];
                    if (!obb_collided(me, ot)) continue;
                    const int otype = s_etype[j];
                    if (collision_pair_filtered(my_type, otype)) continue;
                    hit |= 1;
                    if (otype > ET_None && otype <= ET_StopSign) hit |= 2;
                    else if (otype == ET_Vehicle) hit |= 4;
                    else if (otype <= ET_Cyclist) hit |= 8;
                }
                if (hit) atomicOr(&s_hit[ag], hit);
            }
            STEP_PHASE(3);
            {
                int cnt = 0, c0 = 0;
                if (a < A_T && (my_fl & 1) && !(my_fl & 2) && !GD_DIAG_IS(d.step_dbg, 1)) {
                    const float fx = (s_px[a] - gh.ox) * gh.inv_cell, fy = (s_py[a] - gh.oy) * gh.inv_cell;
                    if (gh.nx > 0 && fx >= 0.f && fy >= 0.f && fx < (float)gh.nx && fy < (float)gh.ny) {
                        const int cell = (int)fy * gh.nx + (int)fx;
                        c0 = d.cell_off[gh.cell_base + cell];
                        cnt = d.cell_off[gh.cell_base + cell + 1] - c0;
                        c0 += gh.item_base;
                    }
                }
                int incl = cnt;
                incl += __builtin_amdgcn_update_dpp(0, incl, 0x111, 0xf, 0xf, false);
                incl += __builtin_amdgcn_update_dpp(0, incl, 0x112, 0xf, 0xf, false);
                incl += __builtin_amdgcn_update_dpp(0, incl, 0x114, 0xf, 0xf, false);
                incl += __builtin_amdgcn_update_dpp(0, incl, 0x118, 0xf, 0xf, false);
                incl += __builtin_amdgcn_update_dpp(0, incl, 0x142, 0xa, 0xf, false);
                incl += __builtin_amdgcn_update_dpp(0, incl, 0x143, 0xc, 0xf, false);
                constexpr int AW = A_T / 64;
                if (a < A_T && (a & 63) == 63) s_wtot[a >> 6] = incl;
                if (a == 0) s_nsv[0] = 0;
                __syncthreads();
                if (a < A_T) {
                    int base = 0;
#pragma unroll
                    for (int k = 0; k < AW; k++) base += (k < (a >> 6)) ? s_wtot[k] : 0;
                    s_c0[a] = c0;
                    s_coff[a] = base + incl - cnt;
                }
                int total = 0;
#pragma unroll
                for (int k = 0; k < AW; k++) total += s_wtot[k];
                __syncthreads();
#ifdef GD_CLOCKS
                if (a == 0) atomicAdd(&g_step_cnt[0], (unsigned long long)total);
#endif
                auto box_test = [&](unsigned int entry) {
#ifdef GD_CLOCKS
                    atomicAdd(&g_step_cnt[1], 1ull);
#endif
                    const int g = (int)(entry & 0xffu), rtype = (int)(entry >> 28);
                    const size_t r = (size_t)(bbase + (int)((entry >> 8) & 0xfffffu));
                    const float4 q1 = d.boxes[r * 5 + 1], q2 = d.boxes[r * 5 + 2], q3 = d.boxes[r * 5 + 3], q4 = d.boxes[r * 5 + 4];
                    const float tmp[16] = {q1.x, q1.y, q1.z, q1.w, q2.x, q2.y, q2.z, q2.w, q3.x, q3.y, q3.z, q3.w, q4.x, q4.y, q4.z, q4.w};
                    Obb ro, me;
                    float *of = reinterpret_cast<float *>(&ro), *mf = reinterpret_cast<float *>(&me);
#pragma unroll
                    for (int k = 0; k < 14; k++) { of[k] = tmp[k]; mf[k] = s_obb[k][g]; }
                    if (obb_collided(me, ro)) atomicOr(&s_hit[g], 1 | ((rtype > ET_None && rtype <= ET_StopSign) ? 2 : 0));
                };
                constexpr int U = SVCAP / STEP_THREADS;
                int trip = 0;
#pragma clang loop unroll(disable)
                for (int t0 = 0; t0 < total; t0 += SVCAP, trip ^= 1) {
                    int agu[U];
                    float4 hdr[U];
                    bool on[U];
#pragma unroll
                    for (int u = 0; u < U; u++) {
                        const int t = t0 + u * STEP_THREADS + a;
                        on[u] = t < total;
                        int lo = 0;
#pragma unroll
                        for (int st = A_T / 2; st > 0; st >>= 1)
                            if (s_coff[lo + st] <= t) lo += st;
                        agu[u] = lo;
                        hdr[u] = d.cell_hdr[on[u] ? s_c0[lo] + (t - s_coff[lo]) : 0];
                    }
#pragma unroll
                    for (int u = 0; u < U; u++) {
                        const int g = agu[u];
                        const unsigned int packed = __float_as_uint(hdr[u].w);
                        const int rtype = (int)(packed & 0xffu);
                        const float dx = s_px[g] - hdr[u].x, dy = s_py[g] - hdr[u].y;
                        const float rr = (s_rad[g] + hdr[u].z) * 1.001f + 0.01f;
                        if (on[u] && !collision_pair_filtered(s_etype[g], rtype) && !(dx * dx + dy * dy > rr * rr))
                            s_sv[atomicAdd(&s_nsv[trip], 1)] = (unsigned int)g | (packed >> 8) << 8 | (packed & 0xfu) << 28;
                    }
                    __syncthreads();
                    const int nsv = s_nsv[trip];
                    if (a == 0) s_nsv[trip ^ 1] = 0;
                    for (int e = a; e < nsv; e += STEP_THREADS) box_test(s_sv[e]);
                    __syncthreads();
                }
            }
            __syncthreads();
            STEP_PHASE(4);
            if (live && active) {
                const int hit = s_hit[a];
                if (hit & 1) collided = 1;
                if (hit & 2) info0 = 1;
                if (hit & 4) info1 = 1;
                if (hit & 8) info2 = 1;
            }
        }

        if (live) {
            const float dist = len_2(b.px - gx, b.py - gy);
            if (d.p.rewardType == GD_REWARD_DISTANCE_BASED) d.reward[i] = -dist;
            else if (d.p.rewardType == GD_REWARD_ON_GOAL_ACHIEVED) d.reward[i] = dist < d.p.distanceToGoalThreshold ? 1.f : 0.f;
            if (moving) --steps;
            const int32_t num_remaining = (int32_t)steps;
            if (num_remaining == EPISODE && done != 1) {
                done = 0;
            } else {
                if (num_remaining == 0) done = 1;
                if (done != 1 || info3 != 1) {
                    if (dist < d.p.distanceToGoalThreshold) { done = 1; info3 = 1; }
                }
            }
            d.px[i] = b.px; d.py[i] = b.py; d.pz[i] = b.pz;
            d.qw[i] = b.qw; d.qz[i] = b.qz;
            d.vx[i] = b.vx; d.vy[i] = b.vy; d.vz[i] = b.vz;
            d.collided[i] = collided;
            d.done[i] = done;
            d.steps[i] = steps;
            int32_t *info = d.info + i * 5;
            info[0] = info0; info[1] = info1; info[2] = info2; info[3] = info3;

            if (OBS) {
                const Quat rot = quat_from_wz(b.qw, b.qz);
                const V3 g = quat_rotate(quat_inv(rot), V3{gx - b.px, gy - b.py, 0.f});
                float *so = d.self_obs + i * 8;
                so[0] = s_speed[a];
                so[1] = length; so[2] = width; so[3] = height;
                so[4] = g.x; so[5] = g.y;
                so[6] = collided ? 1.f : 0.f;
                so[7] = (float)s_id[a];
                if (d.pack != nullptr) {
                    float *ss = s_self + a * 8;
                    ss[0] = s_speed[a]; ss[1] = length; ss[2] = width; ss[3] = height; ss[4] = g.x; ss[5] = g.y; ss[6] = collided ? 1.f : 0.f;
                }
                float *ao = d.abs_obs + i * 14;
                ao[0] = b.px; ao[1] = b.py; ao[2] = b.pz;
                ao[3] = rot.w; ao[4] = rot.x; ao[5] = rot.y; ao[6] = rot.z;
                ao[7] = theta;
                ao[8] = gx; ao[9] = gy;
                ao[10] = length; ao[11] = width; ao[12] = height;
                ao[13] = (float)s_id[a];
            }
        }

#ifdef GD_CLOCKS
        asm volatile("s_waitcnt vmcnt(0)" ::: "memory");
#endif
        STEP_PHASE(5);
        if (OBS && !d.p.disableClassicalObs && !d.split_partner && !d.pack_only)
            partner_rows<A_T>(d, w, n, a, s_px, s_py, s_qw, s_qz, s_speed, s_len, s_wid, s_hgt, s_etype, s_id, !moving || d.pose_skip == 0, s_stage);
        if (OBS && d.pack != nullptr && !d.p.disableClassicalObs) {
            __syncthreads();
            packed_head<A_T, ROWS, COND>(d, w, n, a, s_px, s_py, s_qw, s_qz, s_speed, s_len, s_wid, s_self);
        }
#ifdef GD_CLOCKS
        asm volatile("s_waitcnt vmcnt(0)" ::: "memory");
#endif
        STEP_PHASE(6);
        if (MODE == WS_WARMUP) __syncthreads();
    } while (MODE == WS_WARMUP && ++it < last);
}

template <int A_T>
__global__ __launch_bounds__(STEP_THREADS) void k_partner_rows(DevSim d) {
    const int w = blockIdx.x, a = threadIdx.x;
    if (d.gate_any && *d.any_reset == 0) return;
    const int n = d.shape[w * 2 + 0];
    __shared__ float s_px[A_T], s_py[A_T], s_qw[A_T], s_qz[A_T], s_speed[A_T], s_len[A_T], s_wid[A_T], s_hgt[A_T];
    __shared__ int s_etype[A_T], s_id[A_T];
    if (a < n) {
        const size_t i = (size_t)w * A_T + a;
        s_px[a] = d.px[i]; s_py[a] = d.py[i]; s_qw[a] = d.qw[i]; s_qz[a] = d.qz[i];
        s_speed[a] = len_3(d.vx[i], d.vy[i], d.vz[i]);
        s_len[a] = d.len[i]; s_wid[a] = d.wid[i]; s_hgt[a] = d.hgt[i];
        s_etype[a] = d.etype[i];
        s_id[a] = d.agent_id[i];
    }
    __syncthreads();
    __shared__ __attribute__((aligned(16))) float s_rows[STEP_THREADS * 9];
    partner_rows<A_T>(d, w, n, a, s_px, s_py, s_qw, s_qz, s_speed, s_len, s_wid, s_hgt, s_etype, s_id, true, s_rows);
}

}

#ifdef GD_CLOCKS
void step_clocks_read(unsigned long long *out) {
    unsigned long long z[8] = {0, 0, 0, 0, 0, 0, 0, 0};
    (void)hipDeviceSynchronize();
    (void)hipMemcpyFromSymbol(out, HIP_SYMBOL(g_step_clk), sizeof(z));
    (void)hipMemcpyToSymbol(HIP_SYMBOL(g_step_clk), z, sizeof(z));
    (void)hipMemcpyFromSymbol(out + 8, HIP_SYMBOL(g_step_cnt), 4 * sizeof(unsigned long long));
    (void)hipMemcpyToSymbol(HIP_SYMBOL(g_step_cnt), z, 4 * sizeof(unsigned long long));
}
#endif

template <int A_T>
static void launch_all(const DevSim &d, hipStream_t st, int which, bool move) {
    const dim3 grid(d.W), block(A_T);
    const bool warmup = d.gate_any && d.warm_k > 0;
    switch (which) {
    case KERNEL_RESET:
        if (warmup) hipLaunchKernelGGL((k_world_step<A_T, false, false, WS_WARMUP>), grid, dim3(STEP_THREADS), 0, st, d);
        else hipLaunchKernelGGL(k_reset_worlds<A_T>, grid, block, 0, st, d);
        break;
    case KERNEL_PADDING: hipLaunchKernelGGL(k_init_padding_rows<A_T>, grid, block, 0, st, d); break;
    case KERNEL_STATE:
        if (warmup && !move) {
            if (d.pack != nullptr && d.pack_rows && d.pack_weights)
                hipLaunchKernelGGL((k_world_step<A_T, false, true, WS_AFTER_WARMUP, true>), grid, dim3(STEP_THREADS), 0, st, d);
            else if (d.pack != nullptr && d.pack_rows) hipLaunchKernelGGL((k_world_step<A_T, false, true, WS_AFTER_WARMUP>), grid, dim3(STEP_THREADS), 0, st, d);
            else hipLaunchKernelGGL((k_world_step<A_T, false, false, WS_AFTER_WARMUP>), grid, dim3(STEP_THREADS), 0, st, d);
            break;
        }
        if (d.pack != nullptr && d.pack_rows && d.pack_weights) {
            if (move) hipLaunchKernelGGL((k_world_step<A_T, true, true, WS_STEP, true>), grid, dim3(STEP_THREADS), 0, st, d);
            else hipLaunchKernelGGL((k_world_step<A_T, false, true, WS_STEP, true>), grid, dim3(STEP_THREADS), 0, st, d);
            break;
        }
        if (d.pack != nullptr && d.pack_rows) {
            if (move) hipLaunchKernelGGL((k_world_step<A_T, true, true>), grid, dim3(STEP_THREADS), 0, st, d);
            else hipLaunchKernelGGL((k_world_step<A_T, false, true>), grid, dim3(STEP_THREADS), 0, st, d);
            break;
        }
        if (move) hipLaunchKernelGGL((k_world_step<A_T, true>), grid, dim3(STEP_THREADS), 0, st, d);
        else hipLaunchKernelGGL((k_world_step<A_T, false>), grid, dim3(STEP_THREADS), 0, st, d);
        break;
    case KERNEL_MAP_OBS: launch_map_obs(d, st, move); break;
    case KERNEL_PARTNER: hipLaunchKernelGGL(k_partner_rows<A_T>, grid, dim3(STEP_THREADS), 0, st, d); break;
    }
}

void launch_kernel(const DevSim &d, hipStream_t st, int which, bool move) {
    if (d.A == 64) launch_all<64>(d, st, which, move);
    else launch_all<128>(d, st, which, move);
}

}
```

gpudrive_lab_amd/csrc/map_obs_rank.hip:

```cpp
#include <hip/hip_runtime.h>

#include <algorithm>
#include <type_traits>

#include "engine.hpp"
#include "gd_math.hpp"
#include "rank_cand.hpp"
#include "rank_heap.hpp"

namespace gd {

namespace {

constexpr int K = GD_MAP_OBS_K;
constexpr int CAP = GD_RANK_CAP;
constexpr int NCP = GD_RANK_NCP;
constexpr int SPL = GD_RANK_SPL;
constexpr int KT = GD_RANK_KT;
constexpr int TILE = 32;
constexpr int CAP_LONG = GD_RANK_CAP_LONG;
template <int CAP_T>
struct RankGeo {
    static constexpr bool LONG = CAP_T > CAP;
    static constexpr int NG = CAP_T / 64;
    static constexpr int NMAX = CAP_T - 8;
    static constexpr int NB = CAP_T;
    static constexpr int NLIN = CAP_T * 3 / 5;
    static constexpr int TSH = LONG ? 6 : 5;
    static constexpr int RSH = LONG ? 4 : 5;
    static constexpr int KTN = LONG ? GD_RANK_KT_LONG : GD_RANK_KT;
};
constexpr int NB = RankGeo<CAP>::NB;
static_assert(K + (NCP - 1) * TILE >= CAP && K + (NCP - 1) * 64 >= CAP_LONG, "a checkpoint slot for every tile of candidates");
static_assert(CAP % 64 == 0 && NB % 128 == 0 && CAP < 2047 && CAP_LONG % 640 == 0 && CAP_LONG < 4095, "geometry; less + 1 fits 11 / 12 bits");
static_assert(SPL >= K + 31 && SPL <= CAP && KT >= CAP / 16 + 1, "every slot the finish looks up; an entry per 16 slots + the last");
constexpr int RK_FAR = 1 << 30;
constexpr int RK_TIES = 1 << 30;

__device__ __forceinline__ void wave_sync() {
    __builtin_amdgcn_fence(__ATOMIC_RELEASE, "wavefront");
    __builtin_amdgcn_wave_barrier();
    __builtin_amdgcn_fence(__ATOMIC_ACQUIRE, "wavefront");
}

__device__ __forceinline__ int wave_incl_scan(int v) {
    v += __builtin_amdgcn_update_dpp(0, v, 0x111, 0xf, 0xf, false);
    v += __builtin_amdgcn_update_dpp(0, v, 0x112, 0xf, 0xf, false);
    v += __builtin_amdgcn_update_dpp(0, v, 0x114, 0xf, 0xf, false);
    v += __builtin_amdgcn_update_dpp(0, v, 0x118, 0xf, 0xf, false);
    v += __builtin_amdgcn_update_dpp(0, v, 0x142, 0xa, 0xf, false);
    v += __builtin_amdgcn_update_dpp(0, v, 0x143, 0xc, 0xf, false);
    return v;
}

__device__ __forceinline__ int wave_incl_max_nonneg(int v) {
    v = max(v, __builtin_amdgcn_update_dpp(0, v, 0x111, 0xf, 0xf, false));
    v = max(v, __builtin_amdgcn_update_dpp(0, v, 0x112, 0xf, 0xf, false));
    v = max(v, __builtin_amdgcn_update_dpp(0, v, 0x114, 0xf, 0xf, false));
    v = max(v, __builtin_amdgcn_update_dpp(0, v, 0x118, 0xf, 0xf, false));
    v = max(v, __builtin_amdgcn_update_dpp(0, v, 0x142, 0xa, 0xf, false));
    v = max(v, __builtin_amdgcn_update_dpp(0, v, 0x143, 0xc, 0xf, false));
    return v;
}

#define GD_DPP_SELF(v, ctrl, rows) __builtin_amdgcn_update_dpp((v), (v), (ctrl), (rows), 0xf, false)
__device__ __forceinline__ int wave_max(int v) {
    v = max(v, GD_DPP_SELF(v, 0x111, 0xf));
    v = max(v, GD_DPP_SELF(v, 0x112, 0xf));
    v = max(v, GD_DPP_SELF(v, 0x114, 0xf));
    v = max(v, GD_DPP_SELF(v, 0x118, 0xf));
    v = max(v, GD_DPP_SELF(v, 0x142, 0xa));
    v = max(v, GD_DPP_SELF(v, 0x143, 0xc));
    return __builtin_amdgcn_readlane(v, 63);
}
__device__ __forceinline__ float wave_max_nonneg(float f) { return __int_as_float(wave_max(__float_as_int(f))); }
__device__ __forceinline__ float wave_min_nonneg(float f) { return __int_as_float(~wave_max(~__float_as_int(f))); }
__device__ __forceinline__ int wave_sum(int v) { return __builtin_amdgcn_readlane(wave_incl_scan(v), 63); }
__device__ __forceinline__ unsigned long long wave_ballot(bool p) { return __builtin_amdgcn_ballot_w64(p); }
__device__ __forceinline__ int bits_below_lane(unsigned long long b) {
    return (int)__builtin_amdgcn_mbcnt_hi((unsigned int)(b >> 32), __builtin_amdgcn_mbcnt_lo((unsigned int)b, 0u));
}

#ifndef GD_NT_FINISH_LOAD
#define GD_NT_FINISH_LOAD 1
#endif
#ifndef GD_NT_REPLAY_LOAD
#define GD_NT_REPLAY_LOAD 1
#endif
typedef unsigned int u4v __attribute__((ext_vector_type(4)));
typedef unsigned int u2v __attribute__((ext_vector_type(2)));
template <typename T>
__device__ __forceinline__ T stream_load(const T *p) { return __builtin_nontemporal_load(p); }
template <typename T>
__device__ __forceinline__ void stream_store(T v, T *p) { __builtin_nontemporal_store(v, p); }
__device__ __forceinline__ uint4 stream_load(const uint4 *p) {
    const u4v v = __builtin_nontemporal_load(reinterpret_cast<const u4v *>(p));
    return make_uint4(v.x, v.y, v.z, v.w);
}
__device__ __forceinline__ void stream_store(uint4 v, uint4 *p) {
    u4v t; t.x = v.x; t.y = v.y; t.z = v.z; t.w = v.w;
    __builtin_nontemporal_store(t, reinterpret_cast<u4v *>(p));
}
__device__ __forceinline__ uint2 stream_load(const uint2 *p) {
    const u2v v = __builtin_nontemporal_load(reinterpret_cast<const u2v *>(p));
    return make_uint2(v.x, v.y);
}
__device__ __forceinline__ void stream_store(uint2 v, uint2 *p) {
    u2v t; t.x = v.x; t.y = v.y;
    __builtin_nontemporal_store(t, reinterpret_cast<u2v *>(p));
}

__device__ __forceinline__ int audited(const DevSim &d, int idx, int size) {
    if ((unsigned int)idx < (unsigned int)size) return idx;
    atomicAdd(&d.rk_hist[GD_RANK_AUDIT], 1);
    return idx < 0 ? 0 : size - 1;
}

__device__ __forceinline__ bool rank_lt(unsigned int a, unsigned int b, unsigned int tm = 31u) { return (a | tm) < b; }

template <int A_T>
__global__ __launch_bounds__(256) void k_knn_scan(DevSim d) {
    if (d.gate_any && *d.any_reset == 0) return;
    constexpr int HALVES = A_T / 64;
    const int w = blockIdx.x / HALVES, a0 = (blockIdx.x % HALVES) * 64;
    const int xl = d.rk_scan_rows ? (int)(blockIdx.x & 7) : rank_cand::deal_list((int)blockIdx.x, (int)gridDim.x);
    if (blockIdx.x == 0 && threadIdx.x == 0) d.rk_hist[GD_RH_ROWS] = 0;
    const int tid = threadIdx.x, wave = tid >> 6, lane = tid & 63;
    const int n = d.shape[w * 2 + 0];
    if (a0 >= n) return;
    const int a = a0 + lane;
    const bool live = a < n;
    const size_t i = (size_t)w * A_T + a;
    const size_t WA = (size_t)d.W * A_T;
    const int r0 = d.road_off[w];
    const int R = d.road_off[w + 1] - r0;

    __shared__ unsigned short s_first[NCP][64];
    __shared__ float s_thr[NCP][64];
    __shared__ int s_ncp[64];
    __shared__ unsigned int s_needy[2];
    __shared__ float4 s_hdr[64];
    __shared__ float s_bx[64], s_by[64], s_bm[64];
    __shared__ unsigned int s_hist[4][256];

    float ex = 0.f, ey = 0.f;
    if (live) { ex = d.px[i]; ey = d.py[i]; }
    unsigned long long ranked = 0ull;
    bool own_cp = false;
    bool listed = false;
    int list_base = 0;
    if (wave == 0) {
        int ncp = 0;
        float4 h0 = make_float4(0.f, 0.f, __int_as_float(0), 0.f), h1 = h0;
        if (live) { h0 = d.cp_hdr[i]; h1 = d.cp_hdr[WA + i]; }
        s_hdr[lane] = h0;
        wave_sync();
        if (live) {
            const float4 bb = d.road_bbox[w];
            const float ddx = fmaxf(fmaxf(bb.x - ex, ex - bb.z), 0.f), ddy = fmaxf(fmaxf(bb.y - ey, ey - bb.w), 0.f);
            const float far = d.p.observationRadius * 1.01f + 1.f;
            int state = 1, reason = -1;
            if (R >= K && ddx * ddx + ddy * ddy > far * far) {
                state = RK_FAR;
                d.sel_hdr[i * 2] = make_float4(ex, ey, d.qw[i], d.qz[i]);
                d.sel_hdr[i * 2 + 1] = make_float4(__int_as_float(0), __int_as_float(r0), 0.f, 0.f);
                d.cp_hdr[i] = make_float4(ex, ey, __int_as_float(0), 0.f);
            } else {
                const int n0 = __float_as_int(h0.z), n1 = __float_as_int(h1.z);
                const float m0 = n0 > 0 ? sqrtf((ex - h0.x) * (ex - h0.x) + (ey - h0.y) * (ey - h0.y)) : __builtin_inff();
                const float m1 = n1 > 0 ? sqrtf((ex - h1.x) * (ex - h1.x) + (ey - h1.y) * (ey - h1.y)) : __builtin_inff();
                int set = m1 < m0 ? 1 : 0;
                float move = set ? m1 : m0;
                int n_cp = set ? n1 : n0;
                size_t src = i;
                if (move > rank_cand::CP_MOVE_MAX) {
                    float best = move;
                    int donor = -1;
                    for (int j = 0; j < 64; j++) {
                        const float4 hj = s_hdr[j];
                        const float dj = __float_as_int(hj.z) > 0 ? sqrtf((ex - hj.x) * (ex - hj.x) + (ey - hj.y) * (ey - hj.y)) : __builtin_inff();
                        if (dj < best) { best = dj; donor = j; }
                    }
                    if (donor >= 0) {
                        move = best;
                        set = 0;
                        n_cp = __float_as_int(s_hdr[donor].z);
                        src = (size_t)w * A_T + a0 + donor;
                    }
                }
                const bool eligible = R >= K && R >= d.rk_min_roads && R <= d.rk_max_roads;
                const int grp = (int)(i / 32);
                const bool bypass = eligible && d.rk_streak[grp] >= 3 && ((d.rk_hist[513] + grp) & 63) != 0;
                const float iw = d.qw[i], iz = d.qz[i];
                const float z2 = iz * iz;
                const float det = (1.f - 2.f * z2) * (1.f - 2.f * z2) + 4.f * z2 * (iw * iw);
                const float margin = 1.00001f / fminf(det, 1.f);
                if (!eligible || bypass) {
                    state = 0;
                    ncp = 0;
                    reason = bypass ? -5 : -2;
                    d.rk_fallback[i / 32] = 1;
                } else if (n_cp <= 0 || move > rank_cand::CP_MOVE_MAX) {
                    ncp = -1;
                    s_bx[lane] = ex; s_by[lane] = ey; s_bm[lane] = margin;
                } else if (src == i && !d.rk_scan_rows) {
                    ncp = n_cp;
                    own_cp = true;
                    d.rk_rec[i] = make_float4(move, margin, __int_as_float(n_cp | set << 8), 0.f);
                } else {
                    ncp = n_cp;
                    float t = 1.f;
                    const unsigned short *cr = d.cp_road + ((size_t)set * WA + src) * NCP;
                    const float *ct = d.cp_T + ((size_t)set * WA + src) * NCP;
                    unsigned int fmax = 0u;
                    for (int q = 0; q < ncp; q++) {
                        t = ct[q];
                        fmax = rank_cand::running_max(fmax, cr[q]);
                        s_first[q][lane] = (unsigned short)fmax;
                        s_thr[q][lane] = rank_cand::cp_threshold(t, move, margin);
                    }
                    d.rk_rec[i] = make_float4(move, t, __int_as_float(n_cp | GD_RK_REC_ROW), 0.f);
                }
            }
            d.rk_n[i] = state;
            d.rk_ticket[i] = reason;
            if (state == RK_FAR) ncp = 0;
        }
        s_ncp[lane] = own_cp ? 0 : ncp;
        {
            const unsigned long long nd = __ballot(ncp < 0);
            if (lane == 0) { s_needy[0] = (unsigned int)nd; s_needy[1] = (unsigned int)(nd >> 32); }
        }
        if (ncp < 0) ncp = 1;
        ranked = __ballot(ncp > 0);
        listed = ncp > 0;
        if (ranked != 0ull && lane == 0) list_base = atomicAdd(&d.rk_hist[528 + xl], __popcll(ranked));
    }
    __syncthreads();
    {
        const unsigned long long needy = (unsigned long long)s_needy[0] | (unsigned long long)s_needy[1] << 32;
        if (needy != 0ull) {
            constexpr int BASE = (127 - 2) << 4;
            unsigned int *hist = s_hist[wave];
            int turn = 0;
            for (unsigned long long rest = needy; rest != 0ull; rest &= rest - 1ull, turn++) {
                if ((turn & 3) != wave) continue;
                const int al = __ffsll((long long)rest) - 1;
                const float bx = s_bx[al], by = s_by[al], mg = s_bm[al];
#pragma unroll
                for (int k = 0; k < 4; k++) hist[k * 64 + lane] = 0u;
                if (lane == 0) { s_first[0][al] = (unsigned short)((K / 32) * 32); s_thr[0][al] = __builtin_inff(); }
                const float ratio = exp2f(log2f(fmaxf((float)R / 256.f, 1.f)) / (float)(NCP - 2));
                float pf = 256.f, tlast = __builtin_inff();
                int pq = 256, q = 1;
                float2 nxt = lane < R ? d.road_xy[r0 + lane] : make_float2(0.f, 0.f);
                for (int rb = 0; rb < R; rb += 64) {
                    const float2 xy = nxt;
                    if (rb + 64 + lane < R) nxt = d.road_xy[r0 + rb + 64 + lane];
                    if (rb + lane < R) {
                        const float dx = xy.x - bx, dy = xy.y - by;
                        const float d2 = __builtin_fmaf(dx, dx, dy * dy);
                        atomicAdd(&hist[min(255, max(0, (int)(__float_as_uint(d2) >> 19) - BASE))], 1u);
                    }
                    if (rb + 64 == pq && q < NCP && pq < R) {
                        wave_sync();
                        const uint4 h = reinterpret_cast<const uint4 *>(hist)[lane];
                        const int own = (int)(h.x + h.y + h.z + h.w);
                        const int incl = wave_incl_scan(own), excl = incl - own;
                        int jb = 0, before = excl;
                        if (before + (int)h.x < K) { before += (int)h.x; jb = 1;
                            if (before + (int)h.y < K) { before += (int)h.y; jb = 2;
                                if (before + (int)h.z < K) { jb = 3; } } }
                        const unsigned long long cross = __ballot(excl < K && incl >= K);
                        const int Lc = __ffsll((long long)cross) - 1;
                        const int bucket = 4 * Lc + __builtin_amdgcn_readlane(jb, Lc);
                        const float T = bucket >= 255 ? __builtin_inff() : __uint_as_float((unsigned int)(bucket + 1 + BASE) << 19);
                        if (lane == 0) {
                            const float reach = sqrtf(T) * 1.0001f + 1e-3f;
                            float thr = reach * reach * 1.0001f * mg * 1.001f;
                            if (!(thr >= 0.f)) thr = __builtin_inff();
                            s_first[q][al] = (unsigned short)min(pq, 65535);
                            s_thr[q][al] = thr;
                        }
                        tlast = T;
                        q++;
                        pf *= ratio;
                        pq = max(pq + 64, ((int)pf + 63) & ~63);
                    }
                }
                if (lane == 0) {
                    s_ncp[al] = q;
                    d.rk_rec[(size_t)w * A_T + a0 + al] = make_float4(0.f, tlast < 1e30f ? tlast : 1.f, __int_as_float(q | GD_RK_REC_ROW), 0.f);
                }
            }
            __syncthreads();
        }
    }
    if (wave == 0 && ranked != 0ull) {
        list_base = __builtin_amdgcn_readfirstlane(list_base);
        if (listed)
            d.rk_list[(size_t)xl * WA + audited(d, list_base + __popcll(ranked & ((1ull << lane) - 1ull)), (int)WA)] = (int)i;
    }
    const int ncp = s_ncp[lane];
    if (__syncthreads_or(ncp > 0 ? 1 : 0) == 0) return;
    {
        unsigned short *rowf = d.rk_cpf + ((size_t)w * A_T + a0) * NCP;
        float *rowt = d.rk_cpt + ((size_t)w * A_T + a0) * NCP;
        for (int e = tid; e < 64 * NCP; e += 256) {
            const int ag = e / NCP, q = e - ag * NCP;
            if (q < s_ncp[ag]) {
                rowf[e] = s_first[q][ag];
                rowt[e] = s_thr[q][ag];
            }
        }
    }
}

template <int CAP_T>
struct RankLds {
    union {
        struct {
            float ckey[CAP_T];
            unsigned short cidx[CAP_T];
        } c;
        struct {
            float skey[CAP_T];
            unsigned short spos[CAP_T];
        } s;
        unsigned short spc[CAP_T];
    };
    unsigned int cnt2[RankGeo<CAP_T>::NB / 2];
};
static_assert(sizeof(RankLds<CAP>) <= 10240 && sizeof(RankLds<CAP_LONG>) <= 20480, "sixteen / eight waves per CU");
constexpr int LSTN = (GD_MAX_ROAD_ENTITIES + GD_LIN_BLK - 1) / GD_LIN_BLK + 15;
constexpr int LSTN4 = (LSTN + 3) & ~3;
static_assert(LSTN4 <= 1024 && NCP < 64 && rank_cand::CHUNK % GD_LIN_BLK == 0 && 64 % GD_LIN_BLK == 0, "block and count share 16 bits; a block inside one chunk; whole blocks per pass");
constexpr size_t CAND_TABLES = LSTN4 * sizeof(unsigned short) + (NCP + 2) * sizeof(float);
static_assert(CAND_TABLES <= sizeof(RankLds<CAP>::cnt2) && CAND_TABLES <= sizeof(RankLds<CAP_LONG>::cnt2), "the tables fit the idle counters of both instantiations");
constexpr int CP_EPL = ((GD_MAX_ROAD_ENTITIES + rank_cand::CHUNK - 1) / rank_cand::CHUNK + 63) / 64;
static_assert(64 * CP_EPL * (sizeof(unsigned int) + sizeof(uint2)) <= sizeof(float) * CAP, "the chunk table fits the candidate keys of both instantiations");

struct RankIn {
    int i, state, r0, R, b0, li;
    float ex, ey, iw, iz;
    unsigned int cfirst;
    float cthr;
    float rec_move, rec_y;
    int rec_pack;
};
template <typename T>
__device__ __forceinline__ T uniform_load(const T *p) {
    return *reinterpret_cast<const __attribute__((address_space(4))) T *>(reinterpret_cast<uintptr_t>(p));
}
template <int A_T>
__device__ __forceinline__ RankIn rank_fetch(const DevSim &d, const int *list, int li, int count, int lane) {
    RankIn in;
    in.li = li;
    in.i = li < count ? uniform_load(list + li) : 0;
    in.state = li < count ? uniform_load(d.rk_n + in.i) : 0;
    const int w = in.i / A_T;
    in.r0 = uniform_load(d.road_off + w);
    in.R = uniform_load(d.road_off + w + 1) - in.r0;
    in.ex = uniform_load(d.px + in.i); in.ey = uniform_load(d.py + in.i);
    in.iw = uniform_load(d.qw + in.i); in.iz = -uniform_load(d.qz + in.i);
    in.b0 = uniform_load(d.blk_off + w);
    const float *rec = reinterpret_cast<const float *>(d.rk_rec + in.i);
    in.rec_move = uniform_load(rec); in.rec_y = uniform_load(rec + 1); in.rec_pack = __float_as_int(uniform_load(rec + 2));
    const bool has_row = (in.rec_pack & GD_RK_REC_ROW) != 0;
    const size_t own = ((size_t)((in.rec_pack >> 8) & 1) * d.W * A_T + in.i) * NCP, row = (size_t)in.i * NCP;
    const unsigned short *pf = has_row ? d.rk_cpf + row : d.cp_road + own;
    const float *pt = has_row ? d.rk_cpt + row : d.cp_T + own;
    in.cfirst = rank_cand::NO_CP;
    in.cthr = __builtin_inff();
    if (in.state == 1 && lane < min(in.rec_pack & 0xff, NCP)) {
        in.cfirst = pf[(unsigned int)lane];
        in.cthr = pt[(unsigned int)lane];
    }
    return in;
}

#ifdef GD_CLOCKS
struct PhaseClock {
    unsigned int prev, sum[8];
    __device__ __forceinline__ void mark(int n) {
        const unsigned int t = (unsigned int)__builtin_amdgcn_s_memtime();
        sum[n] += t - prev;
        prev = t;
    }
};
#define GD_PHASE(n) clk.mark(n)
#else
struct PhaseClock {};
#define GD_PHASE(n)
#endif
__device__ __forceinline__ int rank_draw(int *cursor, int lane) {
    int e = 0;
    if (lane == 0) e = atomicAdd(cursor, 1);
    return e;
}
template <int A_T, int CAP_T>
__device__ __forceinline__ void rank_agent(const DevSim &d, const RankIn &in, int lane, RankLds<CAP_T> &L, PhaseClock &clk, int drawn,
                                           int count, const int *list, RankIn &nxt) {
    using G = RankGeo<CAP_T>;
    constexpr int NB = G::NB, NLIN = G::NLIN, NMAX = G::NMAX;
    constexpr unsigned int TM = (1u << G::RSH) - 1u;
    if (__builtin_amdgcn_readfirstlane(in.state) != 1) {
        nxt = rank_fetch<A_T>(d, list, __builtin_amdgcn_readfirstlane(drawn), count, lane);
        return;
    }
    auto uni = [](int v) -> int { return __builtin_amdgcn_readfirstlane(v); };
    auto unif = [](float v) -> float { return __int_as_float(__builtin_amdgcn_readfirstlane(__float_as_int(v))); };
    const int i = uni(in.i), r0 = uni(in.r0), R = uni(in.R);
    const int group = i / 32;
    constexpr int NG = G::NG;

    const float ex = unif(in.ex), ey = unif(in.ey), iw = unif(in.iw), iz = unif(in.iz);
    unsigned short *const lst = reinterpret_cast<unsigned short *>(L.cnt2);
    float *const tthr = reinterpret_cast<float *>(L.cnt2) + LSTN4 / 2;
    unsigned int cfirst = in.cfirst;
    float cthr = in.cthr, t_last_in = unif(in.rec_y);
    if (!(uni(in.rec_pack) & GD_RK_REC_ROW)) {
        const int n_own = min(uni(in.rec_pack) & 0xff, NCP);
        const bool have = lane < n_own;
        t_last_in = __int_as_float(__builtin_amdgcn_readlane(__float_as_int(cthr), n_own - 1));
        const unsigned int fmax = (unsigned int)wave_incl_max_nonneg(have ? (int)cfirst : 0);
        cthr = have ? rank_cand::cp_threshold(cthr, unif(in.rec_move), unif(in.rec_y)) : __builtin_inff();
        cfirst = have ? fmax : rank_cand::NO_CP;
    }
    if (lane <= NCP) tthr[lane + 1] = lane < NCP ? cthr : t_last_in;
    if (lane == 63) tthr[0] = __builtin_inff();
    const float creach = rank_cand::block_reach(cthr);
    const int nblk = (R + GD_LIN_BLK - 1) / GD_LIN_BLK;
    const int nch = rank_cand::chunks_of(R), epl = (nch + 63) >> 6;
    unsigned int *const tmax = reinterpret_cast<unsigned int *>(L.c.ckey);
    uint2 *const tcp = reinterpret_cast<uint2 *>(L.c.ckey + 64 * CP_EPL);
#pragma unroll
    for (int u = 0; u < CP_EPL; u++)
        if (u < epl) tmax[u * 64 + lane] = 0u;
    wave_sync();
    if (lane < NCP && rank_cand::cp_table_takes(cfirst, nch)) atomicMax(&tmax[rank_cand::cp_table_chunk(cfirst)], rank_cand::cp_table_entry(lane));
    wave_sync();
    {
        int own[CP_EPL], run = 0;
#pragma unroll
        for (int u = 0; u < CP_EPL; u++) own[u] = u < epl ? (int)tmax[lane * epl + u] : 0;
#pragma unroll
        for (int u = 0; u < CP_EPL; u++) { run = max(run, own[u]); own[u] = run; }
        const int before = __builtin_amdgcn_ds_bpermute(((lane - 1) & 63) << 2, wave_incl_max_nonneg(run));
#pragma unroll
        for (int u = 0; u < CP_EPL; u++)
            if (u < epl) {
                const int cnt = lane ? max(own[u], before) : own[u];
                const int reach = __builtin_amdgcn_ds_bpermute(((cnt - 1) & 63) << 2, __float_as_int(creach));
                tcp[lane * epl + u] = make_uint2((unsigned int)cnt, (unsigned int)reach);
            }
    }
    wave_sync();
    const float4 *blk = d.road_blk + uni(in.b0);
    int nsv = 0;
    constexpr int CU = 4;
#pragma clang loop unroll(disable)
    for (int b0 = 0; b0 < nblk; b0 += 64 * CU) {
        float4 c[CU];
        uint2 cp[CU];
#pragma unroll
        for (int u = 0; u < CU; u++) {
            const int bc = min(b0 + u * 64 + lane, nblk - 1);
            c[u] = blk[(unsigned int)bc];
            cp[u] = tcp[rank_cand::chunk_base_of_block(bc, GD_LIN_BLK) / rank_cand::CHUNK];
        }
        static_assert(CU == 4, "operand list");
        asm volatile("" : "+v"(c[0].x), "+v"(c[0].y), "+v"(c[0].z), "+v"(c[1].x), "+v"(c[1].y), "+v"(c[1].z), "+v"(c[2].x), "+v"(c[2].y), "+v"(c[2].z),
                     "+v"(c[3].x), "+v"(c[3].y), "+v"(c[3].z));
#pragma unroll
        for (int u = 0; u < CU; u++) {
            const int bb = b0 + u * 64;
            if (bb < nblk) {
                const int b = bb + lane;
                const bool sv = b < nblk && rank_cand::block_survives(b, GD_LIN_BLK, K, c[u].x, c[u].y, c[u].z, ex, ey, __uint_as_float(cp[u].y));
                const unsigned long long m = wave_ballot(sv);
                const int upto = nsv + __popcll(m);
                if (upto <= LSTN4) {
                    if (sv) lst[nsv + bits_below_lane(m)] = (unsigned short)((unsigned int)b | cp[u].x << 10);
                    nsv = upto;
                } else if (lane == 0) {
                    atomicAdd(&d.rk_hist[GD_RANK_AUDIT], 1);
                }
            }
        }
    }
    wave_sync();
    const int next_entry = uni(drawn);
    int nin = 0;
    {
        constexpr int BPP = 64 / GD_LIN_BLK, PB = 2;
        const int np = (nsv + BPP - 1) / BPP, nfast = np - 1;
        const int sub = lane / GD_LIN_BLK, o = lane % GD_LIN_BLK;
        const float2 *rxy = d.road_xy + r0;
        auto store = [&](bool cand, int r, float key, unsigned long long m, bool guard) {
            const int pos = nin + bits_below_lane(m);
            if (cand && (!guard || pos < CAP_T)) {
                L.c.cidx[pos] = (unsigned short)r;
                L.c.ckey[pos] = key;
            }
            nin += __popcll(m);
        };
        int p = 0;
        if (nfast >= 2 * PB) {
            const unsigned int *lsub = reinterpret_cast<const unsigned int *>(L.cnt2) + sub / 2;
            const unsigned int sh = (unsigned int)(sub & 1) * 16u;
            const unsigned int o8 = (unsigned int)o * (unsigned int)sizeof(float2);
            static_assert(BPP == 4, "two words per pass");
            struct Ents { unsigned int e[PB]; };
            struct Batch { unsigned int off[PB]; float thr[PB]; float2 xy[PB]; };
            auto entries = [&](Ents &en, int p0) {
#pragma unroll
                for (int u = 0; u < PB; u++) en.e[u] = lsub[min(p0 + u, nfast - 1) * (BPP / 2)];
            };
            auto issue = [&](Batch &bt, const Ents &en) {
#pragma unroll
                for (int u = 0; u < PB; u++) {
                    bt.off[u] = __builtin_amdgcn_ubfe(en.e[u], sh, 10u) * (unsigned int)(GD_LIN_BLK * sizeof(float2)) + o8;
                    bt.thr[u] = tthr[__builtin_amdgcn_ubfe(en.e[u], sh + 10u, 6u)];
                    bt.xy[u] = *reinterpret_cast<const float2 *>(reinterpret_cast<const char *>(rxy) + bt.off[u]);
                }
            };
            auto take = [&](const Batch &bt) {
#pragma unroll
                for (int u = 0; u < PB; u++) {
                    const int r = (int)(bt.off[u] / (unsigned int)sizeof(float2));
                    __builtin_assume(r >= 0 && r < R);
                    const bool cand = rank_cand::is_candidate(r, K, R, bt.xy[u].x, bt.xy[u].y, ex, ey, bt.thr[u]);
                    store(cand, r, ego_dist2(ex, ey, iw, iz, bt.xy[u].x, bt.xy[u].y), wave_ballot(cand), false);
                }
            };
            Ents ea, eb;
            Batch ba, bb;
            entries(ea, 0);
            entries(eb, PB);
            issue(ba, ea);
#pragma clang loop unroll(disable)
            for (; p + 2 * PB <= nfast && nin + 2 * PB * 64 <= CAP_T; p += 2 * PB) {
                issue(bb, eb);
                entries(ea, p + 2 * PB);
                take(ba);
                issue(ba, ea);
                entries(eb, p + 3 * PB);
                take(bb);
            }
        }
#pragma clang loop unroll(disable)
        for (; p < np; p += 2 * PB) {
            int r[2 * PB];
            float thr[2 * PB];
            float2 xy[2 * PB];
#pragma unroll
            for (int u = 0; u < 2 * PB; u++) {
                r[u] = R; thr[u] = 0.f; xy[u] = make_float2(0.f, 0.f);
                if (p + u < np) {
                    const int e = (p + u) * BPP + sub;
                    const unsigned int ent = lst[min(e, LSTN4 - 1)];
                    const bool on = e < nsv;
                    r[u] = on ? (int)(ent & 1023u) * GD_LIN_BLK + o : R;
                    thr[u] = tthr[on ? min((int)(ent >> 10), NCP) : 0];
                    xy[u] = rxy[(unsigned int)min(r[u], R - 1)];
                }
            }
#pragma unroll
            for (int u = 0; u < 2 * PB; u++) {
                if (p + u < np) {
                    const bool cand = rank_cand::is_candidate(r[u], K, R, xy[u].x, xy[u].y, ex, ey, thr[u]);
                    store(cand, r[u], ego_dist2(ex, ey, iw, iz, xy[u].x, xy[u].y), wave_ballot(cand), true);
                }
            }
        }
    }
    wave_sync();
    nxt = rank_fetch<A_T>(d, list, next_entry, count, lane);
    {
        const int total = nin;
        if (total > NMAX) {
            if (lane == 0) {
                bool passed_on = false;
                if (!G::LONG && total <= RankGeo<CAP_LONG>::NMAX) {
                    const int slot = atomicAdd(&d.rk_hist[GD_RH_LONG], 1);
                    if (slot < d.rk_nlong) {
                        d.rk_longlist[slot] = i;
                        passed_on = true;
                    }
                }
                if (!passed_on) {
                    d.rk_n[i] = 0;
                    d.rk_ticket[i] = -3;
                    d.rk_fallback[group] = 1;
                }
            }
            return;
        }
    }
#ifdef GD_CLOCKS
    clk.sum[7] += (unsigned int)((nsv + 3) / 4) << 8;
#endif
    const int bin = 255 - min(255, (nin - K) / 5);
    int ticket = 0;
    if (lane == 0) ticket = bin << 20 | atomicAdd(&d.rk_hist[bin], 1);
    GD_PHASE(1);
    if (GD_DIAG_IS(d.rk_dbg, 1)) return;
    if (lane <= (nin - K) >> G::TSH) {
        const int road = (int)L.c.cidx[K - 1 + (lane << G::TSH)];
        d.cp_road[(size_t)i * NCP + lane] = (unsigned short)(lane ? min(65535, (road + 1 + 31) & ~31) : (K / 32) * 32);
    }
    constexpr int GQ = 5;
    static_assert(NG % GQ == 0, "whole groups");
    const float kmax = d.radius_key_max;
    int ci[NG];
    float key[NG];
    const float t_last = unif(tthr[NCP + 1]);
    float split = (t_last > 0.f && t_last < 1e30f) ? t_last * 1.5f : 1.f;
// ... 392 lines not shown
        }
        if (lane < AWR) rank_heap::fill_pairs<K>(H, w);
        if (wave_ties && __ballot(on && rank_heap::any_tie(w, tm)) != 0ull) {
            tt = rank_heap::track_of(w, tm);
            if (!on) tt.tg = rank_heap::NO_TIE;
        }
    }
    const bool heap_ties = __ballot(tt.tl()) != 0ull;
    GD_RPHASE(1);
    if (on) {
        if (heap_ties) rank_heap::make_heap<K, true>(H, tm);
        else rank_heap::make_heap<K, false>(H, tm);
    }
    GD_RPHASE(2);
    unsigned int r[8];
#pragma unroll
    for (int j = 1; j < 8; j++) r[j] = H.get(j);
    unsigned int last = H.get(K);
    if (lane < AWR) H.set(K, 0u);
    unsigned short *cpe = d.rk_cpe + (size_t)i * NCP;
    if (on) cpe[0] = (unsigned short)r[1];

    int nmax = n;
#pragma unroll
    for (int off = 32; off > 0; off >>= 1) nmax = max(nmax, __shfl_xor(nmax, off));
    const uint4 *blocks = reinterpret_cast<const uint4 *>(E + K);
    uint4 cur = on ? (GD_NT_REPLAY_LOAD ? stream_load(blocks) : blocks[0]) : make_uint4(0u, 0u, 0u, 0u);
    uint4 nxt = on ? (GD_NT_REPLAY_LOAD ? stream_load(blocks + 1) : blocks[1]) : make_uint4(0u, 0u, 0u, 0u);
#ifdef GD_CLOCKS
    int n_ins = 0;
    int blk_all = 0, blk_ties = 0, blk_checked = 0;
    int n_chk = 0, n_redo = 0;
    const auto wave_any = [&](bool f) -> bool {
        const bool a = __ballot(f) != 0ull;
        n_chk++;
        n_redo += a ? 1 : 0;
        return a;
    };
#else
    const auto wave_any = [](bool f) -> bool { return __ballot(f) != 0ull; };
#endif
    auto replay = [&](auto mixed_tag) {
        constexpr bool MIXED = decltype(mixed_tag)::value;
        static_assert(TILE == 32, "four blocks of eight candidates per checkpoint");
#pragma clang loop unroll(disable)
        for (int p0 = K; p0 < nmax; p0 += TILE) {
#pragma clang loop unroll(disable)
            for (int pb = p0; pb < min(p0 + TILE, nmax); pb += 8) {
                const uint4 w8 = cur;
                cur = nxt;
                nxt = GD_NT_REPLAY_LOAD ? stream_load(blocks + ((pb - K) >> 3) + 2) : blocks[((pb - K) >> 3) + 2];
                const unsigned int wd[4] = {w8.x, w8.y, w8.z, w8.w};
                const int left = n - pb;
                int ins;
                if (MIXED && __ballot(on && rank_heap::block_has_tie(wd, left, tm)) != 0ull) {
                    ins = rank_heap::block_rounds<K, rank_heap::TIES>(H, r, last, wd, left, tm, tt);
#ifdef GD_CLOCKS
                    blk_ties++;
#endif
                } else if (MIXED && __ballot(tt.tl()) != 0ull) {
                    ins = rank_heap::block_rounds<K, rank_heap::CHECKED>(H, r, last, wd, left, tm, tt, wave_any);
#ifdef GD_CLOCKS
                    blk_checked++;
#endif
                } else {
                    ins = rank_heap::block_rounds<K, rank_heap::PLAIN>(H, r, last, wd, left, tm, tt);
                }
#ifdef GD_CLOCKS
                n_ins += ins;
                blk_all++;
#else
                (void)ins;
#endif
            }
            const int after = p0 - K + TILE;
            if (p0 + TILE - 1 < n && (after & ((1 << tsh) - 1)) == 0) cpe[after >> tsh] = (unsigned short)r[1];
        }
    };
    if (wave_ties) replay(std::true_type{});
    else replay(std::false_type{});
    GD_RPHASE(3);
#ifdef GD_CLOCKS
    {
        const int tot_ins = wave_sum(n_ins), tot_cand = wave_sum(on ? n - K : 0), longest = wave_max(on ? n - K : 0);
        if (lane == 0) {
            atomicAdd(&d.rk_hist[526], tot_ins);
            atomicAdd(&d.rk_hist[525], tot_cand);
            if (blockIdx.x == 0) atomicAdd(&d.rk_hist[524], longest);
        }
    }
#endif
    if (lane < AWR) {
        H.set(K, last);
#pragma unroll
        for (int j = 1; j < 8; j++) H.set(j, r[j]);
    }
    if (on) {
        unsigned int *out = d.rk_heap + (size_t)i * GD_RANK_HEAP_DW;
#pragma clang loop unroll(disable)
        for (int j = 0; j < GD_RANK_HEAP_DW; j += 4) {
            uint4 v;
            v.x = j + 0 <= K / 2 ? H.pair(j + 0) : 0u;
            v.y = j + 1 <= K / 2 ? H.pair(j + 1) : 0u;
            v.z = j + 2 <= K / 2 ? H.pair(j + 2) : 0u;
            v.w = j + 3 <= K / 2 ? H.pair(j + 3) : 0u;
            stream_store(v, reinterpret_cast<uint4 *>(out + j));
        }
    }
#ifdef GD_CLOCKS
    GD_RPHASE(4);
    const int w_chk = wave_sum(n_chk), w_redo = wave_sum(n_redo);
    if (lane == 0) {
        const int total = (int)(rclk.prev - rclk.first);
        if (blockIdx.x < 32) {
            int *row = d.rk_hist + 256 + blockIdx.x * 7;
            for (int k = 0; k < 5; k++) row[k] = (int)rclk.ph[k];
            row[5] = (wave_ties ? 1 : 0) | (blk_ties << 1) | (blk_checked << 10) | (blk_all << 20);
            row[6] = total;
        }
        atomicAdd(&d.rk_hist[480], wave_ties ? 1 : 0);
        atomicAdd(&d.rk_hist[481], 1);
        atomicMax(&d.rk_hist[482], total);
        atomicMax(&d.rk_hist[wave_ties ? 483 : 484], total);
        atomicAdd(&d.rk_hist[485], blk_ties);
        atomicAdd(&d.rk_hist[486], wave_ties ? blk_all : 0);
        atomicAdd(&d.rk_hist[487], blk_checked);
        atomicAdd(&d.rk_hist[488], w_chk);
        atomicAdd(&d.rk_hist[489], w_redo);
    }
#endif
}

template <int A_T>
__global__ __launch_bounds__(256) void k_knn_finish(DevSim d) {
    if (d.gate_any && *d.any_reset == 0) return;
    const int tid = threadIdx.x, wave = tid >> 6, lane = tid & 63;
    const int li = blockIdx.x * 4 + wave;
    const int ranked_agents = d.rk_hist[512];
    const int i = d.rk_order[min(li, d.W * A_T - 1)];
    constexpr int NP = (K + 63) / 64;
    const int w = i / A_T;
    const int fell_back = d.rk_fallback[i / 32];
    const int packed = d.rk_n[i];
    const int r0 = d.road_off[w], r1 = d.road_off[w + 1];
    const float ex = d.px[i], ey = d.py[i];
    const float qw = d.qw[i], qz = d.qz[i];
    const uint32_t steps_left = d.steps[i];
    const int long_slot = d.rk_longslot[i];
    const unsigned int *hp = d.rk_heap + (size_t)i * GD_RANK_HEAP_DW;
    unsigned int hpair[NP];
#pragma unroll
    for (int ps = 0; ps < NP; ps++) hpair[ps] = GD_NT_FINISH_LOAD ? stream_load(hp + min((ps * 64 + lane + 1) >> 1, GD_RANK_HEAP_DW - 1)) : hp[min((ps * 64 + lane + 1) >> 1, GD_RANK_HEAP_DW - 1)];
    static_assert(SPL == 256, "four slots per lane");
    const uint2 spc4 = GD_NT_FINISH_LOAD ? stream_load(reinterpret_cast<const uint2 *>(d.rk_spc + (size_t)i * SPL) + lane) : reinterpret_cast<const uint2 *>(d.rk_spc + (size_t)i * SPL)[lane];
    const unsigned int cp_e = d.rk_cpe[(size_t)i * NCP + min(lane, NCP - 1)];
    const unsigned short cp_r = d.cp_road[(size_t)i * NCP + min(lane, NCP - 1)];
    static_assert(NP == 4, "operand list");
    asm volatile("" ::"v"(fell_back), "v"(packed), "v"(ex), "v"(ey), "v"(qw), "v"(qz), "v"(steps_left), "v"(long_slot), "v"(hpair[0]),
                 "v"(hpair[1]), "v"(hpair[2]), "v"(hpair[3]), "v"(spc4.x), "v"(spc4.y), "v"(cp_e), "v"(cp_r), "s"(r0), "s"(r1));
    if (li >= ranked_agents || fell_back != 0) return;
    const int n = packed & 0xffff, nle = (packed >> 16) & 0xfff;
    if (packed <= 0 || packed == RK_FAR || n < K) return;
    const bool is_long = ((packed >> 29) & 1) != 0;
    const int rsh = is_long ? 4 : 5, tsh = is_long ? 6 : 5;
    const unsigned int tm = (1u << rsh) - 1u;
    const int cp_slot = (int)(cp_e >> rsh) - 1 + (int)(cp_e & tm);
    const int ncp = 1 + ((n - K) >> tsh);
    const float *kt_row = is_long ? d.rk_kt_long + (size_t)long_slot * GD_RANK_KT_LONG : d.rk_kt + (size_t)i * KT;
    float cp_t = 0.f;
    if (lane < ncp) cp_t = kt_row[min(max((cp_slot + 15) >> 4, 0), (n + 15) >> 4)];
    __shared__ unsigned short s_spc[4][SPL];
    __shared__ unsigned short s_don[4][K];
    __shared__ unsigned int s_bm[4][GD_RANK_NCH];
    __shared__ unsigned short s_wp[4][GD_RANK_NCH];
    __shared__ unsigned int s_sorted[4][K];
    unsigned short *don = s_don[wave];
    unsigned int *bm = s_bm[wave];
    const unsigned long long lower = (1ull << lane) - 1ull;
    {
        reinterpret_cast<uint2 *>(s_spc[wave])[lane] = spc4;
#pragma unroll
        for (int k = 0; k < GD_RANK_NCH / 64; k++) bm[k * 64 + lane] = 0u;
    }
    wave_sync();

    int road[NP];
    bool inr[NP];
    unsigned long long fl[NP];
    int m = 0;
#pragma unroll
    for (int ps = 0; ps < NP; ps++) {
        const int t = ps * 64 + lane, g = t + 1;
        road[ps] = 0;
        inr[ps] = false;
        if (t < K) {
            const unsigned int p2 = hpair[ps];
            const unsigned int e = (g & 1) ? p2 >> 16 : p2 & 0xffffu;
            const int less = (int)(e >> rsh) - 1;
            road[ps] = s_spc[wave][audited(d, less + (int)(e & tm), min(n, SPL))];
            inr[ps] = less < nle;
        }
        fl[ps] = __ballot(inr[ps]);
        m += __popcll(fl[ps]);
    }
    if (m < K) {
        int above = 0;
#pragma unroll
        for (int ps = NP - 1; ps >= 0; ps--) {
            const int t = ps * 64 + lane;
            if (t < K && t >= m && inr[ps]) don[above + __popcll(fl[ps] & ~lower & ~(1ull << lane))] = (unsigned short)road[ps];
            above += __popcll(fl[ps]);
        }
        wave_sync();
        int before = 0;
        int in_before = 0;
#pragma unroll
        for (int ps = 0; ps < NP; ps++) {
            const int t = ps * 64 + lane;
            if (t < m && !inr[ps]) {
                const int h = (t - before) - __popcll(fl[ps] & lower) + (before - in_before);
                road[ps] = don[h];
            }
            before += 64;
            in_before += __popcll(fl[ps]);
        }
    }
    const int R = r1 - r0;
#pragma unroll
    for (int ps = 0; ps < NP; ps++) {
        const int t = ps * 64 + lane;
        if (t < m) atomicOr(&bm[audited(d, road[ps], R) >> 5], 1u << (road[ps] & 31));
    }
    wave_sync();
    {
        constexpr int WL = GD_RANK_NCH / 64;
        unsigned int own[WL];
        int sum = 0;
#pragma unroll
        for (int k = 0; k < WL; k++) { own[k] = bm[lane * WL + k]; sum += __popc(own[k]); }
        int run = wave_incl_scan(sum) - sum;
#pragma unroll
        for (int k = 0; k < WL; k++) { s_wp[wave][lane * WL + k] = (unsigned short)run; run += __popc(own[k]); }
    }
    wave_sync();
#pragma unroll
    for (int ps = 0; ps < NP; ps++) {
        const int t = ps * 64 + lane;
        if (t < m) {
            const int rd = min(max(road[ps], 0), R - 1);
            const int place = (int)s_wp[wave][rd >> 5] + __popc(bm[rd >> 5] & ((1u << (rd & 31)) - 1u));
            s_sorted[wave][audited(d, place, m)] = (unsigned int)rd | (unsigned int)t << 16;
        }
    }
    wave_sync();
#pragma unroll
    for (int ps = 0; ps < NP; ps++) {
        const int q = ps * 64 + lane;
        if (q < K) {
            const unsigned int v = q < m ? s_sorted[wave][q] : (unsigned int)q << 16;
            d.sel_idx[(size_t)i * K + q] = (unsigned short)(v & 0xffffu);
            d.sel_slot[(size_t)i * K + q] = (unsigned char)(v >> 16);
        }
    }
    const bool at_start = steps_left == (uint32_t)GD_EPISODE_LEN;
    const size_t WA = (size_t)d.W * A_T;
    if (lane < ncp) {
        (void)audited(d, cp_slot, n);
        d.cp_T[(size_t)i * NCP + lane] = cp_t;
        if (at_start) {
            d.cp_T[(WA + i) * NCP + lane] = cp_t;
            d.cp_road[(WA + i) * NCP + lane] = cp_r;
        }
    }
    if (lane == 0) {
        d.rk_streak[i / 32] = 0;
        d.cp_hdr[i] = make_float4(ex, ey, __int_as_float(ncp), 0.f);
        if (at_start) d.cp_hdr[WA + i] = make_float4(ex, ey, __int_as_float(ncp), 0.f);
        d.sel_hdr[(size_t)i * 2] = make_float4(ex, ey, qw, qz);
        d.sel_hdr[(size_t)i * 2 + 1] = make_float4(__int_as_float(m), __int_as_float(r0), __int_as_float(1), 0.f);
    }
}

}

#ifndef GD_RANK_LONG_GRID
#define GD_RANK_LONG_GRID 2048
#endif
int rank_resident_waves(int A) {
    int per_cu = 0, dev = 0;
    hipDeviceProp_t prop;
    const hipError_t e = A == 64 ? hipOccupancyMaxActiveBlocksPerMultiprocessor(&per_cu, k_knn_rank<64, CAP>, 64, 0)
                                 : hipOccupancyMaxActiveBlocksPerMultiprocessor(&per_cu, k_knn_rank<128, CAP>, 64, 0);
    if (e != hipSuccess || hipGetDevice(&dev) != hipSuccess || hipGetDeviceProperties(&prop, dev) != hipSuccess) {
        (void)hipGetLastError();
        return GD_RANK_GRID;
    }
    return std::max(per_cu, 1) * std::max(prop.multiProcessorCount, 1);
}

void launch_map_obs_rank(const DevSim &d, hipStream_t st) {
    if (d.live_count == 0) return;
    const dim3 glong(std::min(std::max(d.rk_nlong, 1), GD_RANK_LONG_GRID));
    const dim3 gr(d.rk_waves > 0 ? d.rk_waves : std::min((d.live_count + 7) / 8 * 8, GD_RANK_GRID)), g4((d.live_count + 3) / 4), gw(d.W * (d.A / 64));
    if (d.A == 64) {
        hipLaunchKernelGGL((k_knn_scan<64>), gw, dim3(256), 0, st, d);
        hipLaunchKernelGGL((k_knn_rank<64, CAP>), gr, dim3(64), 0, st, d);
        if (d.rk_nlong > 0) hipLaunchKernelGGL((k_knn_rank<64, CAP_LONG>), glong, dim3(64), 0, st, d);
    } else {
        hipLaunchKernelGGL((k_knn_scan<128>), gw, dim3(256), 0, st, d);
        hipLaunchKernelGGL((k_knn_rank<128, CAP>), gr, dim3(64), 0, st, d);
        if (d.rk_nlong > 0) hipLaunchKernelGGL((k_knn_rank<128, CAP_LONG>), glong, dim3(64), 0, st, d);
    }
    hipLaunchKernelGGL(k_knn_order, dim3((d.live_count + 255) / 256), dim3(256), 0, st, d);
    hipLaunchKernelGGL(k_knn_replay, dim3((d.live_count + AWR - 1) / AWR), dim3(64), 0, st, d);
    if (d.A == 64) hipLaunchKernelGGL((k_knn_finish<64>), g4, dim3(256), 0, st, d);
    else hipLaunchKernelGGL((k_knn_finish<128>), g4, dim3(256), 0, st, d);
}

}
```

Before: 70.41 million.

## Fold the k-NN rank setup (scan) into the world-step kernel

```diff
diff --git a/gpudrive_lab_amd/csrc/engine.cpp b/gpudrive_lab_amd/csrc/engine.cpp
--- a/gpudrive_lab_amd/csrc/engine.cpp
+++ b/gpudrive_lab_amd/csrc/engine.cpp
@@ -1050,6 +1050,8 @@
         if (const char *e = std::getenv("GPUDRIVE_RANK_WAVES")) d.rk_waves = std::min(std::max((std::atoi(e) + 7) / 8 * 8, 8), GD_RANK_GRID);
         d.rk_scan_rows = 0;
         if (const char *e = std::getenv("GPUDRIVE_RANK_SCAN_ROWS")) d.rk_scan_rows = std::atoi(e) != 0 ? 1 : 0;
+        d.rk_scan_kernel = 0;
+        if (const char *e = std::getenv("GPUDRIVE_RANK_SCAN_KERNEL")) d.rk_scan_kernel = std::atoi(e) != 0 ? 1 : 0;
         d.rk_resident = std::max(gd::rank_resident_waves(A) / 8, 1);
         s->rk_possible = GD_MAP_OBS_AW == 32 && cfg->knn_order != GD_KNN_SET_ORDER &&
                          params->roadObservationAlgorithm == GD_ROADS_K_NEAREST && std::getenv("GPUDRIVE_NO_RANK_REPLAY") == nullptr;
@@ -2356,6 +2358,10 @@
         *out = static_cast<int64_t>(v);
         return GD_OK;
     }
+    if (s && out && which == 47) {
+        *out = gd::rank_setup_folded(s->d) ? 1 : 0;
+        return GD_OK;
+    }
     if (s && out && which == 22) {
         *out = 0;
         if (s->rk_alloc) {
diff --git a/gpudrive_lab_amd/csrc/engine.hpp b/gpudrive_lab_amd/csrc/engine.hpp
--- a/gpudrive_lab_amd/csrc/engine.hpp
+++ b/gpudrive_lab_amd/csrc/engine.hpp
@@ -145,6 +145,7 @@
     float *rk_cpt;
     float4 *rk_rec;
     int rk_scan_rows;
+    int rk_scan_kernel;
     int rk_resident;
     const float4 *road_bbox;
     const float *road_rbmax;
@@ -160,6 +161,11 @@
     unsigned long long *warm_count;
     const float *pack_weights;
 };
+
+inline bool rank_setup_folded(const DevSim &d) {
+    return d.rk_scan_kernel == 0 && d.rk_on != 0 && d.live_count != 0 && d.p.disableClassicalObs == 0 &&
+           d.p.roadObservationAlgorithm == GD_ROADS_K_NEAREST && d.knn_order != GD_KNN_SET_ORDER;
+}
 
 void launch_kernel(const DevSim &d, hipStream_t st, int which, bool move);
 void launch_map_obs(const DevSim &d, hipStream_t st, bool move);
diff --git a/gpudrive_lab_amd/csrc/kernels.hip b/gpudrive_lab_amd/csrc/kernels.hip
--- a/gpudrive_lab_amd/csrc/kernels.hip
+++ b/gpudrive_lab_amd/csrc/kernels.hip
@@ -5,6 +5,7 @@
 #include "gd_math.hpp"
 #include "map_rows.hpp"
 #include "pack_cols.hpp"
+#include "rank_setup.hpp"
 
 namespace gd {
 
@@ -254,15 +255,17 @@
 }
 
 
-template <int A_T, bool ROWS, bool COND = false>
+template <bool COND>
+constexpr int HEAD_STAGE = COND ? 64 * 6 + 4 : 64 * 6;
+template <int A_T, bool ROWS, bool COND = false, bool EXT = false>
 __device__ __forceinline__ void packed_head(const DevSim &d, int w, int n, int a, const float *s_px, const float *s_py,
                                             const float *s_qw, const float *s_qz, const float *s_speed, const float *s_len,
-                                            const float *s_wid, const float *s_self) {
+                                            const float *s_wid, const float *s_self, float *ext = nullptr) {
     static_assert(ROWS || !COND, "the conditioned layout exists for the learner rows only");
     constexpr int D = 6 + (A_T - 1) * 6 + K * 13, PITCH = COND ? D + 3 : D;
-    __shared__ __attribute__((aligned(16))) float s_head[STEP_THREADS / 64][COND ? 64 * 6 + 4 : 64 * 6];
+    __shared__ __attribute__((aligned(16))) float s_head[EXT ? 1 : STEP_THREADS / 64][EXT ? 4 : HEAD_STAGE<COND>];
     const int wave = a >> 6, lane = a & 63;
-    float *stage = s_head[wave];
+    float *stage = EXT ? ext + wave * HEAD_STAGE<COND> : s_head[wave];
     typedef float f4 __attribute__((ext_vector_type(4)));
     for (int ego = wave; ego < n; ego += STEP_THREADS / 64) {
         size_t prow = (size_t)w * A_T + ego;
@@ -316,9 +319,10 @@
 
 enum { WS_STEP = 0, WS_WARMUP = 1, WS_AFTER_WARMUP = 2 };
 
-template <int A_T, bool MOVE, bool ROWS = false, int MODE = WS_STEP, bool COND = false>
+template <int A_T, bool MOVE, bool ROWS = false, int MODE = WS_STEP, bool COND = false, bool FOLD = false>
 __global__ __launch_bounds__(STEP_THREADS) void k_world_step(DevSim d) {
     constexpr bool OBS = MODE != WS_WARMUP;
+    static_assert(OBS || !FOLD, "the set-up runs where the observation phases do");
     const int w = blockIdx.x, a = threadIdx.x;
     if (!MOVE && d.gate_any && *d.any_reset == 0) return;
     const int n = d.shape[w * 2 + 0];
@@ -330,16 +334,31 @@
     __shared__ float s_px[A_T], s_py[A_T], s_qw[A_T], s_qz[A_T], s_speed[A_T];
     __shared__ float s_len[A_T], s_wid[A_T], s_hgt[A_T], s_rad[A_T];
     __shared__ int s_etype[A_T], s_id[A_T], s_flags[A_T];
-    __shared__ float s_obb[14][A_T];
+    __shared__ float s_obb_own[FOLD ? 1 : 14][FOLD ? 1 : A_T];
     __shared__ int s_hit[A_T];
     __shared__ float s_self[A_T * 8];
-    __shared__ __attribute__((aligned(16))) float s_stage[STEP_THREADS * 9];
+    constexpr int STAGE_OBB = STEP_THREADS * 9, STAGE_HEAD = STAGE_OBB + 14 * A_T, STAGE_TENANTS = STAGE_HEAD + (STEP_THREADS / 64) * HEAD_STAGE<COND>;
+    constexpr int STAGE_FLOATS = !FOLD ? STEP_THREADS * 9 : STAGE_TENANTS * sizeof(float) >= sizeof(rank_setup::Rows) ? STAGE_TENANTS : (int)(sizeof(rank_setup::Rows) / sizeof(float));
+    static_assert(STAGE_OBB % 4 == 0 && STAGE_HEAD % 4 == 0, "16-byte aligned tenants");
+    __shared__ __attribute__((aligned(16))) float s_stage[STAGE_FLOATS];
+    float(*const s_obb)[A_T] = FOLD ? reinterpret_cast<float(*)[A_T]>(s_stage + STAGE_OBB) : reinterpret_cast<float(*)[A_T]>(&s_obb_own[0][0]);
     float *const s_opx = s_stage, *const s_opy = s_stage + A_T;
     unsigned long long *const s_moved = reinterpret_cast<unsigned long long *>(s_stage + 2 * A_T);
     constexpr int SVCAP = 6 * STEP_THREADS;
     static_assert(SVCAP <= STEP_THREADS * 9 && 3 * A_T <= STEP_THREADS * 9, "the staging buffer holds each of its tenants");
     unsigned int *const s_sv = reinterpret_cast<unsigned int *>(s_stage);
     __shared__ int s_nsv[2];
+    __shared__ rank_setup::Half s_half[A_T / 64];
+    float4 su_h0 = make_float4(0.f, 0.f, 0.f, 0.f), su_h1 = su_h0;
+    int su_streak = 0;
+    rank_setup::WorldIn su_in = {};
+    if constexpr (FOLD) {
+        if (a < A_T) {
+            su_h0 = d.cp_hdr[i]; su_h1 = d.cp_hdr[(size_t)d.W * A_T + i];
+            su_streak = d.rk_streak[i / 32];
+            su_in = rank_setup::world_in(d, w);
+        }
+    }
     __shared__ int s_c0[A_T], s_coff[A_T], s_wtot[A_T / 64];
 
 #ifdef GD_CLOCKS
@@ -444,6 +463,11 @@
             }
         }
 
+        rank_setup::Listed su_listed = {};
+        if constexpr (FOLD) {
+            if (a < A_T) su_listed = rank_setup::decide_half<A_T>(d, w, a & ~63, a & 63, b.px, b.py, b.qw, b.qz, live, su_h0, su_h1, su_streak, su_in, s_half[a >> 6]);
+        }
+
         STEP_PHASE(1);
         bool active = false, moved = false;
         const bool track_moves = OBS && (d.bev != nullptr || (d.lidar != nullptr && d.p.enableLidar != 0));
@@ -704,16 +728,24 @@
 #ifdef GD_CLOCKS
         asm volatile("s_waitcnt vmcnt(0)" ::: "memory");
 #endif
+        if constexpr (FOLD) {
+#pragma unroll
+            for (int h = 0; h < A_T / 64; h++)
+                if (rank_setup::rows_needed(s_half[h])) rank_setup::rows_half<A_T>(d, w, h * 64, s_half[h], *reinterpret_cast<rank_setup::Rows *>(s_stage));
+        }
         STEP_PHASE(5);
         if (OBS && !d.p.disableClassicalObs && !d.split_partner && !d.pack_only)
             partner_rows<A_T>(d, w, n, a, s_px, s_py, s_qw, s_qz, s_speed, s_len, s_wid, s_hgt, s_etype, s_id, !moving || d.pose_skip == 0, s_stage);
         if (OBS && d.pack != nullptr && !d.p.disableClassicalObs) {
             __syncthreads();
-            packed_head<A_T, ROWS, COND>(d, w, n, a, s_px, s_py, s_qw, s_qz, s_speed, s_len, s_wid, s_self);
+            packed_head<A_T, ROWS, COND, FOLD>(d, w, n, a, s_px, s_py, s_qw, s_qz, s_speed, s_len, s_wid, s_self, FOLD ? s_stage + STAGE_HEAD : nullptr);
         }
 #ifdef GD_CLOCKS
         asm volatile("s_waitcnt vmcnt(0)" ::: "memory");
 #endif
+        if constexpr (FOLD) {
+            if (a < A_T) rank_setup::list_half<A_T>(d, w, a & ~63, a & 63, su_listed);
+        }
         STEP_PHASE(6);
         if (MODE == WS_WARMUP) __syncthreads();
     } while (MODE == WS_WARMUP && ++it < last);
@@ -752,6 +784,13 @@
 }
 #endif
 
+template <int A_T, bool MOVE, int MODE, bool FOLD>
+static void launch_state(const DevSim &d, hipStream_t st, dim3 grid, int rows) {
+    if (rows == 2) hipLaunchKernelGGL((k_world_step<A_T, MOVE, true, MODE, true, FOLD>), grid, dim3(STEP_THREADS), 0, st, d);
+    else if (rows == 1) hipLaunchKernelGGL((k_world_step<A_T, MOVE, true, MODE, false, FOLD>), grid, dim3(STEP_THREADS), 0, st, d);
+    else hipLaunchKernelGGL((k_world_step<A_T, MOVE, false, MODE, false, FOLD>), grid, dim3(STEP_THREADS), 0, st, d);
+}
+
 template <int A_T>
 static void launch_all(const DevSim &d, hipStream_t st, int which, bool move) {
     const dim3 grid(d.W), block(A_T);
@@ -762,27 +801,21 @@
         else hipLaunchKernelGGL(k_reset_worlds<A_T>, grid, block, 0, st, d);
         break;
     case KERNEL_PADDING: hipLaunchKernelGGL(k_init_padding_rows<A_T>, grid, block, 0, st, d); break;
-    case KERNEL_STATE:
+    case KERNEL_STATE: {
+        const bool fold = rank_setup_folded(d);
+        const int rows = d.pack != nullptr && d.pack_rows ? (d.pack_weights ? 2 : 1) : 0;
         if (warmup && !move) {
-            if (d.pack != nullptr && d.pack_rows && d.pack_weights)
-                hipLaunchKernelGGL((k_world_step<A_T, false, true, WS_AFTER_WARMUP, true>), grid, dim3(STEP_THREADS), 0, st, d);
-            else if (d.pack != nullptr && d.pack_rows) hipLaunchKernelGGL((k_world_step<A_T, false, true, WS_AFTER_WARMUP>), grid, dim3(STEP_THREADS), 0, st, d);
-            else hipLaunchKernelGGL((k_world_step<A_T, false, false, WS_AFTER_WARMUP>), grid, dim3(STEP_THREADS), 0, st, d);
-            break;
-        }
-        if (d.pack != nullptr && d.pack_rows && d.pack_weights) {
-            if (move) hipLaunchKernelGGL((k_world_step<A_T, true, true, WS_STEP, true>), grid, dim3(STEP_THREADS), 0, st, d);
-            else hipLaunchKernelGGL((k_world_step<A_T, false, true, WS_STEP, true>), grid, dim3(STEP_THREADS), 0, st, d);
-            break;
-        }
-        if (d.pack != nullptr && d.pack_rows) {
-            if (move) hipLaunchKernelGGL((k_world_step<A_T, true, true>), grid, dim3(STEP_THREADS), 0, st, d);
-            else hipLaunchKernelGGL((k_world_step<A_T, false, true>), grid, dim3(STEP_THREADS), 0, st, d);
-            break;
-        }
-        if (move) hipLaunchKernelGGL((k_world_step<A_T, true>), grid, dim3(STEP_THREADS), 0, st, d);
-        else hipLaunchKernelGGL((k_world_step<A_T, false>), grid, dim3(STEP_THREADS), 0, st, d);
+            if (fold) launch_state<A_T, false, WS_AFTER_WARMUP, true>(d, st, grid, rows);
+            else launch_state<A_T, false, WS_AFTER_WARMUP, false>(d, st, grid, rows);
+        } else if (move) {
+            if (fold) launch_state<A_T, true, WS_STEP, true>(d, st, grid, rows);
+            else launch_state<A_T, true, WS_STEP, false>(d, st, grid, rows);
+        } else {
+            if (fold) launch_state<A_T, false, WS_STEP, true>(d, st, grid, rows);
+            else launch_state<A_T, false, WS_STEP, false>(d, st, grid, rows);
+        }
         break;
+    }
     case KERNEL_MAP_OBS: launch_map_obs(d, st, move); break;
     case KERNEL_PARTNER: hipLaunchKernelGGL(k_partner_rows<A_T>, grid, dim3(STEP_THREADS), 0, st, d); break;
     }
diff --git a/gpudrive_lab_amd/csrc/map_obs_rank.hip b/gpudrive_lab_amd/csrc/map_obs_rank.hip
--- a/gpudrive_lab_amd/csrc/map_obs_rank.hip
+++ b/gpudrive_lab_amd/csrc/map_obs_rank.hip
@@ -7,6 +7,7 @@
 #include "gd_math.hpp"
 #include "rank_cand.hpp"
 #include "rank_heap.hpp"
+#include "rank_setup.hpp"
 
 namespace gd {
 
@@ -34,7 +35,7 @@
 static_assert(K + (NCP - 1) * TILE >= CAP && K + (NCP - 1) * 64 >= CAP_LONG, "a checkpoint slot for every tile of candidates");
 static_assert(CAP % 64 == 0 && NB % 128 == 0 && CAP < 2047 && CAP_LONG % 640 == 0 && CAP_LONG < 4095, "geometry; less + 1 fits 11 / 12 bits");
 static_assert(SPL >= K + 31 && SPL <= CAP && KT >= CAP / 16 + 1, "every slot the finish looks up; an entry per 16 slots + the last");
-constexpr int RK_FAR = 1 << 30;
+constexpr int RK_FAR = rank_setup::RK_FAR;
 constexpr int RK_TIES = 1 << 30;
 
 __device__ __forceinline__ void wave_sync() {
@@ -123,197 +124,19 @@
     if (d.gate_any && *d.any_reset == 0) return;
     constexpr int HALVES = A_T / 64;
     const int w = blockIdx.x / HALVES, a0 = (blockIdx.x % HALVES) * 64;
-    const int xl = d.rk_scan_rows ? (int)(blockIdx.x & 7) : rank_cand::deal_list((int)blockIdx.x, (int)gridDim.x);
-    if (blockIdx.x == 0 && threadIdx.x == 0) d.rk_hist[GD_RH_ROWS] = 0;
-    const int tid = threadIdx.x, wave = tid >> 6, lane = tid & 63;
+    const int wave = threadIdx.x >> 6, lane = threadIdx.x & 63;
     const int n = d.shape[w * 2 + 0];
-    if (a0 >= n) return;
-    const int a = a0 + lane;
-    const bool live = a < n;
-    const size_t i = (size_t)w * A_T + a;
-    const size_t WA = (size_t)d.W * A_T;
-    const int r0 = d.road_off[w];
-    const int R = d.road_off[w + 1] - r0;
-
-    __shared__ unsigned short s_first[NCP][64];
-    __shared__ float s_thr[NCP][64];
-    __shared__ int s_ncp[64];
-    __shared__ unsigned int s_needy[2];
-    __shared__ float4 s_hdr[64];
-    __shared__ float s_bx[64], s_by[64], s_bm[64];
-    __shared__ unsigned int s_hist[4][256];
-
-    float ex = 0.f, ey = 0.f;
-    if (live) { ex = d.px[i]; ey = d.py[i]; }
-    unsigned long long ranked = 0ull;
-    bool own_cp = false;
-    bool listed = false;
-    int list_base = 0;
+    __shared__ rank_setup::Half s_half;
+    __shared__ rank_setup::Rows s_rows;
+    rank_setup::Listed listed;
     if (wave == 0) {
-        int ncp = 0;
-        float4 h0 = make_float4(0.f, 0.f, __int_as_float(0), 0.f), h1 = h0;
-        if (live) { h0 = d.cp_hdr[i]; h1 = d.cp_hdr[WA + i]; }
-        s_hdr[lane] = h0;
-        wave_sync();
-        if (live) {
-            const float4 bb = d.road_bbox[w];
-            const float ddx = fmaxf(fmaxf(bb.x - ex, ex - bb.z), 0.f), ddy = fmaxf(fmaxf(bb.y - ey, ey - bb.w), 0.f);
-            const float far = d.p.observationRadius * 1.01f + 1.f;
-            int state = 1, reason = -1;
-            if (R >= K && ddx * ddx + ddy * ddy > far * far) {
-                state = RK_FAR;
-                d.sel_hdr[i * 2] = make_float4(ex, ey, d.qw[i], d.qz[i]);
-                d.sel_hdr[i * 2 + 1] = make_float4(__int_as_float(0), __int_as_float(r0), 0.f, 0.f);
-                d.cp_hdr[i] = make_float4(ex, ey, __int_as_float(0), 0.f);
-            } else {
-                const int n0 = __float_as_int(h0.z), n1 = __float_as_int(h1.z);
-                const float m0 = n0 > 0 ? sqrtf((ex - h0.x) * (ex - h0.x) + (ey - h0.y) * (ey - h0.y)) : __builtin_inff();
-                const float m1 = n1 > 0 ? sqrtf((ex - h1.x) * (ex - h1.x) + (ey - h1.y) * (ey - h1.y)) : __builtin_inff();
-                int set = m1 < m0 ? 1 : 0;
-                float move = set ? m1 : m0;
-                int n_cp = set ? n1 : n0;
-                size_t src = i;
-                if (move > rank_cand::CP_MOVE_MAX) {
-                    float best = move;
-                    int donor = -1;
-                    for (int j = 0; j < 64; j++) {
-                        const float4 hj = s_hdr[j];
-                        const float dj = __float_as_int(hj.z) > 0 ? sqrtf((ex - hj.x) * (ex - hj.x) + (ey - hj.y) * (ey - hj.y)) : __builtin_inff();
-                        if (dj < best) { best = dj; donor = j; }
-                    }
-                    if (donor >= 0) {
-                        move = best;
-                        set = 0;
-                        n_cp = __float_as_int(s_hdr[donor].z);
-                        src = (size_t)w * A_T + a0 + donor;
-                    }
-                }
-                const bool eligible = R >= K && R >= d.rk_min_roads && R <= d.rk_max_roads;
-                const int grp = (int)(i / 32);
-                const bool bypass = eligible && d.rk_streak[grp] >= 3 && ((d.rk_hist[513] + grp) & 63) != 0;
-                const float iw = d.qw[i], iz = d.qz[i];
-                const float z2 = iz * iz;
-                const float det = (1.f - 2.f * z2) * (1.f - 2.f * z2) + 4.f * z2 * (iw * iw);
-                const float margin = 1.00001f / fminf(det, 1.f);
-                if (!eligible || bypass) {
-                    state = 0;
-                    ncp = 0;
-                    reason = bypass ? -5 : -2;
-                    d.rk_fallback[i / 32] = 1;
-                } else if (n_cp <= 0 || move > rank_cand::CP_MOVE_MAX) {
-                    ncp = -1;
-                    s_bx[lane] = ex; s_by[lane] = ey; s_bm[lane] = margin;
-                } else if (src == i && !d.rk_scan_rows) {
-                    ncp = n_cp;
-                    own_cp = true;
-                    d.rk_rec[i] = make_float4(move, margin, __int_as_float(n_cp | set << 8), 0.f);
-                } else {
-                    ncp = n_cp;
-                    float t = 1.f;
-                    const unsigned short *cr = d.cp_road + ((size_t)set * WA + src) * NCP;
-                    const float *ct = d.cp_T + ((size_t)set * WA + src) * NCP;
-                    unsigned int fmax = 0u;
-                    for (int q = 0; q < ncp; q++) {
-                        t = ct[q];
-                        fmax = rank_cand::running_max(fmax, cr[q]);
-                        s_first[q][lane] = (unsigned short)fmax;
-                        s_thr[q][lane] = rank_cand::cp_threshold(t, move, margin);
-                    }
-                    d.rk_rec[i] = make_float4(move, t, __int_as_float(n_cp | GD_RK_REC_ROW), 0.f);
-                }
-            }
-            d.rk_n[i] = state;
-            d.rk_ticket[i] = reason;
-            if (state == RK_FAR) ncp = 0;
-        }
-        s_ncp[lane] = own_cp ? 0 : ncp;
-        {
-            const unsigned long long nd = __ballot(ncp < 0);
-            if (lane == 0) { s_needy[0] = (unsigned int)nd; s_needy[1] = (unsigned int)(nd >> 32); }
-        }
-        if (ncp < 0) ncp = 1;
-        ranked = __ballot(ncp > 0);
-        listed = ncp > 0;
-        if (ranked != 0ull && lane == 0) list_base = atomicAdd(&d.rk_hist[528 + xl], __popcll(ranked));
+        const size_t i = (size_t)w * A_T + a0 + lane, WA = (size_t)d.W * A_T;
+        listed = rank_setup::decide_half<A_T>(d, w, a0, lane, d.px[i], d.py[i], d.qw[i], d.qz[i], a0 + lane < n, d.cp_hdr[i], d.cp_hdr[WA + i],
+                                              d.rk_streak[i / 32], rank_setup::world_in(d, w), s_half);
     }
     __syncthreads();
-    {
-        const unsigned long long needy = (unsigned long long)s_needy[0] | (unsigned long long)s_needy[1] << 32;
-        if (needy != 0ull) {
-            constexpr int BASE = (127 - 2) << 4;
-            unsigned int *hist = s_hist[wave];
-            int turn = 0;
-            for (unsigned long long rest = needy; rest != 0ull; rest &= rest - 1ull, turn++) {
-                if ((turn & 3) != wave) continue;
-                const int al = __ffsll((long long)rest) - 1;
-                const float bx = s_bx[al], by = s_by[al], mg = s_bm[al];
-#pragma unroll
-                for (int k = 0; k < 4; k++) hist[k * 64 + lane] = 0u;
-                if (lane == 0) { s_first[0][al] = (unsigned short)((K / 32) * 32); s_thr[0][al] = __builtin_inff(); }
-                const float ratio = exp2f(log2f(fmaxf((float)R / 256.f, 1.f)) / (float)(NCP - 2));
-                float pf = 256.f, tlast = __builtin_inff();
-                int pq = 256, q = 1;
-                float2 nxt = lane < R ? d.road_xy[r0 + lane] : make_float2(0.f, 0.f);
-                for (int rb = 0; rb < R; rb += 64) {
-                    const float2 xy = nxt;
-                    if (rb + 64 + lane < R) nxt = d.road_xy[r0 + rb + 64 + lane];
-                    if (rb + lane < R) {
-                        const float dx = xy.x - bx, dy = xy.y - by;
-                        const float d2 = __builtin_fmaf(dx, dx, dy * dy);
-                        atomicAdd(&hist[min(255, max(0, (int)(__float_as_uint(d2) >> 19) - BASE))], 1u);
-                    }
-                    if (rb + 64 == pq && q < NCP && pq < R) {
-                        wave_sync();
-                        const uint4 h = reinterpret_cast<const uint4 *>(hist)[lane];
-                        const int own = (int)(h.x + h.y + h.z + h.w);
-                        const int incl = wave_incl_scan(own), excl = incl - own;
-                        int jb = 0, before = excl;
-                        if (before + (int)h.x < K) { before += (int)h.x; jb = 1;
-                            if (before + (int)h.y < K) { before += (int)h.y; jb = 2;
-                                if (before + (int)h.z < K) { jb = 3; } } }
-                        const unsigned long long cross = __ballot(excl < K && incl >= K);
-                        const int Lc = __ffsll((long long)cross) - 1;
-                        const int bucket = 4 * Lc + __builtin_amdgcn_readlane(jb, Lc);
-                        const float T = bucket >= 255 ? __builtin_inff() : __uint_as_float((unsigned int)(bucket + 1 + BASE) << 19);
-                        if (lane == 0) {
-                            const float reach = sqrtf(T) * 1.0001f + 1e-3f;
-                            float thr = reach * reach * 1.0001f * mg * 1.001f;
-                            if (!(thr >= 0.f)) thr = __builtin_inff();
-                            s_first[q][al] = (unsigned short)min(pq, 65535);
-                            s_thr[q][al] = thr;
-                        }
-                        tlast = T;
-                        q++;
-                        pf *= ratio;
-                        pq = max(pq + 64, ((int)pf + 63) & ~63);
-                    }
-                }
-                if (lane == 0) {
-                    s_ncp[al] = q;
-                    d.rk_rec[(size_t)w * A_T + a0 + al] = make_float4(0.f, tlast < 1e30f ? tlast : 1.f, __int_as_float(q | GD_RK_REC_ROW), 0.f);
-                }
-            }
-            __syncthreads();
-        }
-    }
-    if (wave == 0 && ranked != 0ull) {
-        list_base = __builtin_amdgcn_readfirstlane(list_base);
-        if (listed)
-            d.rk_list[(size_t)xl * WA + audited(d, list_base + __popcll(ranked & ((1ull << lane) - 1ull)), (int)WA)] = (int)i;
-    }
-    const int ncp = s_ncp[lane];
-    if (__syncthreads_or(ncp > 0 ? 1 : 0) == 0) return;
-    {
-        unsigned short *rowf = d.rk_cpf + ((size_t)w * A_T + a0) * NCP;
-        float *rowt = d.rk_cpt + ((size_t)w * A_T + a0) * NCP;
-        for (int e = tid; e < 64 * NCP; e += 256) {
-            const int ag = e / NCP, q = e - ag * NCP;
-            if (q < s_ncp[ag]) {
-                rowf[e] = s_first[q][ag];
-                rowt[e] = s_thr[q][ag];
-            }
-        }
-    }
+    if (rank_setup::rows_needed(s_half)) rank_setup::rows_half<A_T>(d, w, a0, s_half, s_rows);
+    if (wave == 0) rank_setup::list_half<A_T>(d, w, a0, lane, listed);
 }
 
 template <int CAP_T>
@@ -1312,12 +1135,13 @@
     if (d.live_count == 0) return;
     const dim3 glong(std::min(std::max(d.rk_nlong, 1), GD_RANK_LONG_GRID));
     const dim3 gr(d.rk_waves > 0 ? d.rk_waves : std::min((d.live_count + 7) / 8 * 8, GD_RANK_GRID)), g4((d.live_count + 3) / 4), gw(d.W * (d.A / 64));
+    const bool scan = !rank_setup_folded(d);
     if (d.A == 64) {
-        hipLaunchKernelGGL((k_knn_scan<64>), gw, dim3(256), 0, st, d);
+        if (scan) hipLaunchKernelGGL((k_knn_scan<64>), gw, dim3(256), 0, st, d);
         hipLaunchKernelGGL((k_knn_rank<64, CAP>), gr, dim3(64), 0, st, d);
         if (d.rk_nlong > 0) hipLaunchKernelGGL((k_knn_rank<64, CAP_LONG>), glong, dim3(64), 0, st, d);
     } else {
-        hipLaunchKernelGGL((k_knn_scan<128>), gw, dim3(256), 0, st, d);
+        if (scan) hipLaunchKernelGGL((k_knn_scan<128>), gw, dim3(256), 0, st, d);
         hipLaunchKernelGGL((k_knn_rank<128, CAP>), gr, dim3(64), 0, st, d);
         if (d.rk_nlong > 0) hipLaunchKernelGGL((k_knn_rank<128, CAP_LONG>), glong, dim3(64), 0, st, d);
     }
diff --git a/gpudrive_lab_amd/csrc/rank_setup.hpp b/gpudrive_lab_amd/csrc/rank_setup.hpp
--- /dev/null
+++ b/gpudrive_lab_amd/csrc/rank_setup.hpp
@@ -0,0 +1,314 @@
+#pragma once
+
+#include "rank_cand.hpp"
+
+namespace gd {
+namespace rank_setup {
+
+constexpr int RK_FAR = 1 << 30;
+
+enum {
+    FAR = 0,
+    FALLBACK = 1,
+    AFRESH = 2,
+    OWN = 3,
+    ROW = 4
+};
+
+struct Decision {
+    int kind;
+    int state, reason;
+    int set, n_cp;
+    int donor;
+    float move, margin;
+};
+
+template <typename H4>
+GD_RC_FN Decision decide(int self, float ex, float ey, float iw, float iz, const H4 &h0, const H4 &h1, const H4 &bb, const H4 *hdrs,
+                         int R, int K, float radius, int min_roads, int max_roads, int streak, int selections, int grp,
+                         bool scan_rows) {
+#pragma clang fp contract(off)
+    Decision o;
+    o.kind = FAR; o.state = 1; o.reason = -1; o.set = 0; o.n_cp = 0; o.donor = -1; o.move = 0.f; o.margin = 0.f;
+    const float ddx = fmaxf(fmaxf(bb.x - ex, ex - bb.z), 0.f), ddy = fmaxf(fmaxf(bb.y - ey, ey - bb.w), 0.f);
+    const float far = radius * 1.01f + 1.f;
+    if (R >= K && ddx * ddx + ddy * ddy > far * far) {
+        o.state = RK_FAR;
+        return o;
+    }
+    const int n0 = (int)rank_cand::f32_bits(h0.z), n1 = (int)rank_cand::f32_bits(h1.z);
+    const float m0 = n0 > 0 ? sqrtf((ex - h0.x) * (ex - h0.x) + (ey - h0.y) * (ey - h0.y)) : __builtin_inff();
+    const float m1 = n1 > 0 ? sqrtf((ex - h1.x) * (ex - h1.x) + (ey - h1.y) * (ey - h1.y)) : __builtin_inff();
+    int set = m1 < m0 ? 1 : 0;
+    float move = set ? m1 : m0;
+    int n_cp = set ? n1 : n0;
+    if (move > rank_cand::CP_MOVE_MAX) {
+        float best = move;
+        int donor = -1;
+        for (int j = 0; j < 64; j++) {
+            const H4 hj = hdrs[j];
+            const float dj = (int)rank_cand::f32_bits(hj.z) > 0 ? sqrtf((ex - hj.x) * (ex - hj.x) + (ey - hj.y) * (ey - hj.y)) : __builtin_inff();
+            if (dj < best) { best = dj; donor = j; }
+        }
+        if (donor >= 0) {
+            move = best;
+            set = 0;
+            n_cp = (int)rank_cand::f32_bits(hdrs[donor].z);
+            o.donor = donor;
+        }
+    }
+    const bool eligible = R >= K && R >= min_roads && R <= max_roads;
+    const bool bypass = eligible && streak >= 3 && ((selections + grp) & 63) != 0;
+    const float z2 = iz * iz;
+    const float det = (1.f - 2.f * z2) * (1.f - 2.f * z2) + 4.f * z2 * (iw * iw);
+    o.margin = 1.00001f / fminf(det, 1.f);
+    o.move = move; o.set = set; o.n_cp = n_cp;
+    if (!eligible || bypass) {
+        o.kind = FALLBACK;
+        o.state = 0;
+        o.reason = bypass ? -5 : -2;
+    } else if (n_cp <= 0 || move > rank_cand::CP_MOVE_MAX) {
+        o.kind = AFRESH;
+    } else if ((o.donor < 0 || o.donor == self) && !scan_rows) {
+        o.kind = OWN;
+    } else {
+        o.kind = ROW;
+    }
+    return o;
+}
+GD_RC_FN int own_record_bits(const Decision &o) { return o.n_cp | o.set << 8; }
+
+}
+}
+
+#if defined(__HIPCC__)
+#include "engine.hpp"
+
+namespace gd {
+namespace rank_setup {
+
+constexpr int K = GD_MAP_OBS_K;
+constexpr int NCP = GD_RANK_NCP;
+
+
+struct Half {
+    float4 hdr[64];
+    int ncp[64];
+    float p0[64], p1[64], p2[64];
+    unsigned int needy[2];
+    unsigned int copied[2];
+};
+struct Rows {
+    unsigned int hist[4][256];
+    float thr[NCP][64];
+    unsigned short first[NCP][64];
+};
+static_assert(sizeof(Half) % 16 == 0 && sizeof(Rows) % 16 == 0, "callers lay them over 16-byte aligned LDS");
+
+struct Listed {
+    unsigned long long ranked;
+    int xl;
+};
+
+__device__ __forceinline__ void wave_sync() {
+    __builtin_amdgcn_fence(__ATOMIC_RELEASE, "wavefront");
+    __builtin_amdgcn_wave_barrier();
+    __builtin_amdgcn_fence(__ATOMIC_ACQUIRE, "wavefront");
+}
+__device__ __forceinline__ int wave_incl_scan(int v) {
+    v += __builtin_amdgcn_update_dpp(0, v, 0x111, 0xf, 0xf, false);
+    v += __builtin_amdgcn_update_dpp(0, v, 0x112, 0xf, 0xf, false);
+    v += __builtin_amdgcn_update_dpp(0, v, 0x114, 0xf, 0xf, false);
+    v += __builtin_amdgcn_update_dpp(0, v, 0x118, 0xf, 0xf, false);
+    v += __builtin_amdgcn_update_dpp(0, v, 0x142, 0xa, 0xf, false);
+    v += __builtin_amdgcn_update_dpp(0, v, 0x143, 0xc, 0xf, false);
+    return v;
+}
+
+struct WorldIn {
+    float4 bbox;
+    int r0, r1;
+    int selections;
+};
+__device__ __forceinline__ WorldIn world_in(const DevSim &d, int w) {
+    WorldIn in;
+    in.bbox = d.road_bbox[w];
+    in.r0 = d.road_off[w]; in.r1 = d.road_off[w + 1];
+    in.selections = d.rk_hist[513];
+    return in;
+}
+template <int A_T>
+__device__ __forceinline__ Listed decide_half(const DevSim &d, int w, int a0, int lane, float ex, float ey, float iw, float iz, bool live,
+                                              float4 h0, float4 h1, int streak, const WorldIn &in, Half &s) {
+#pragma clang fp contract(off)
+    constexpr int HALVES = A_T / 64;
+    const int blk = w * HALVES + a0 / 64;
+    Listed out;
+    out.ranked = 0ull;
+    out.xl = d.rk_scan_rows ? (blk & 7) : rank_cand::deal_list(blk, d.W * HALVES);
+    if (blk == 0 && lane == 0) d.rk_hist[GD_RH_ROWS] = 0;
+    const size_t i = (size_t)w * A_T + a0 + lane;
+    const int r0 = in.r0;
+    const int R = in.r1 - r0;
+    int ncp = 0;
+    bool own_cp = false, copy = false;
+    if (!live) { h0 = make_float4(0.f, 0.f, __int_as_float(0), 0.f); h1 = h0; }
+    s.hdr[lane] = h0;
+    wave_sync();
+    if (live) {
+        const int grp = (int)(i / 32);
+        const Decision o = decide(lane, ex, ey, iw, iz, h0, h1, in.bbox, s.hdr, R, K, d.p.observationRadius,
+                                  d.rk_min_roads, d.rk_max_roads, streak, in.selections, grp, d.rk_scan_rows != 0);
+        if (o.kind == FAR) {
+            d.sel_hdr[i * 2] = make_float4(ex, ey, iw, iz);
+            d.sel_hdr[i * 2 + 1] = make_float4(__int_as_float(0), __int_as_float(r0), 0.f, 0.f);
+            d.cp_hdr[i] = make_float4(ex, ey, __int_as_float(0), 0.f);
+        } else if (o.kind == FALLBACK) {
+            d.rk_fallback[i / 32] = 1;
+        } else if (o.kind == AFRESH) {
+            ncp = -1;
+            s.p0[lane] = ex; s.p1[lane] = ey; s.p2[lane] = o.margin;
+        } else if (o.kind == OWN) {
+            ncp = o.n_cp;
+            own_cp = true;
+            d.rk_rec[i] = make_float4(o.move, o.margin, __int_as_float(own_record_bits(o)), 0.f);
+        } else {
+            ncp = o.n_cp;
+            copy = true;
+            s.p0[lane] = o.move; s.p1[lane] = __int_as_float((o.donor >= 0 ? o.donor : lane) | o.set << 8); s.p2[lane] = o.margin;
+        }
+        d.rk_n[i] = o.state;
+        d.rk_ticket[i] = o.reason;
+    }
+    s.ncp[lane] = own_cp ? 0 : ncp;
+    {
+        const unsigned long long nd = __ballot(ncp < 0), cp = __ballot(copy);
+        if (lane == 0) {
+            s.needy[0] = (unsigned int)nd; s.needy[1] = (unsigned int)(nd >> 32);
+            s.copied[0] = (unsigned int)cp; s.copied[1] = (unsigned int)(cp >> 32);
+        }
+    }
+    if (ncp < 0) ncp = 1;
+    out.ranked = __ballot(ncp > 0);
+    return out;
+}
+
+template <int A_T>
+__device__ __forceinline__ void list_half(const DevSim &d, int w, int a0, int lane, const Listed &l) {
+    if (l.ranked == 0ull) return;
+    const size_t WA = (size_t)d.W * A_T;
+    int base = 0;
+    if (lane == 0) base = atomicAdd(&d.rk_hist[528 + l.xl], __popcll(l.ranked));
+    base = __builtin_amdgcn_readfirstlane(base);
+    if ((l.ranked >> lane) & 1ull) {
+        int at = base + __popcll(l.ranked & ((1ull << lane) - 1ull));
+        if ((unsigned int)at >= (unsigned int)WA) {
+            atomicAdd(&d.rk_hist[GD_RANK_AUDIT], 1);
+            at = at < 0 ? 0 : (int)WA - 1;
+        }
+        d.rk_list[(size_t)l.xl * WA + at] = (int)((size_t)w * A_T + a0 + lane);
+    }
+}
+
+__device__ __forceinline__ bool rows_needed(const Half &s) { return (s.needy[0] | s.needy[1] | s.copied[0] | s.copied[1]) != 0u; }
+
+template <int A_T>
+__device__ __forceinline__ void rows_half(const DevSim &d, int w, int a0, Half &s, Rows &b) {
+#pragma clang fp contract(off)
+    const int tid = threadIdx.x, wave = tid >> 6, lane = tid & 63;
+    const size_t WA = (size_t)d.W * A_T;
+    const int r0 = d.road_off[w];
+    const int R = d.road_off[w + 1] - r0;
+    const unsigned long long needy = (unsigned long long)s.needy[0] | (unsigned long long)s.needy[1] << 32;
+    const unsigned long long copied = (unsigned long long)s.copied[0] | (unsigned long long)s.copied[1] << 32;
+    if (wave == 0 && ((copied >> lane) & 1ull)) {
+        const size_t i = (size_t)w * A_T + a0 + lane;
+        const float move = s.p0[lane], margin = s.p2[lane];
+        const int from = __float_as_int(s.p1[lane]), set = from >> 8;
+        const size_t src = (size_t)w * A_T + a0 + (from & 255);
+        const int ncp = s.ncp[lane];
+        float t = 1.f;
+        const unsigned short *cr = d.cp_road + ((size_t)set * WA + src) * NCP;
+        const float *ct = d.cp_T + ((size_t)set * WA + src) * NCP;
+        unsigned int fmax = 0u;
+        for (int q = 0; q < ncp; q++) {
+            t = ct[q];
+            fmax = rank_cand::running_max(fmax, cr[q]);
+            b.first[q][lane] = (unsigned short)fmax;
+            b.thr[q][lane] = rank_cand::cp_threshold(t, move, margin);
+        }
+        d.rk_rec[i] = make_float4(move, t, __int_as_float(ncp | GD_RK_REC_ROW), 0.f);
+    }
+    if (needy != 0ull) {
+        constexpr int BASE = (127 - 2) << 4;
+        unsigned int *hist = b.hist[wave];
+        int turn = 0;
+        for (unsigned long long rest = needy; rest != 0ull; rest &= rest - 1ull, turn++) {
+            if ((turn & 3) != wave) continue;
+            const int al = __ffsll((long long)rest) - 1;
+            const float bx = s.p0[al], by = s.p1[al], mg = s.p2[al];
+#pragma unroll
+            for (int k = 0; k < 4; k++) hist[k * 64 + lane] = 0u;
+            if (lane == 0) { b.first[0][al] = (unsigned short)((K / 32) * 32); b.thr[0][al] = __builtin_inff(); }
+            const float ratio = exp2f(log2f(fmaxf((float)R / 256.f, 1.f)) / (float)(NCP - 2));
+            float pf = 256.f, tlast = __builtin_inff();
+            int pq = 256, q = 1;
+            float2 nxt = lane < R ? d.road_xy[r0 + lane] : make_float2(0.f, 0.f);
+            for (int rb = 0; rb < R; rb += 64) {
+                const float2 xy = nxt;
+                if (rb + 64 + lane < R) nxt = d.road_xy[r0 + rb + 64 + lane];
+                if (rb + lane < R) {
+                    const float dx = xy.x - bx, dy = xy.y - by;
+                    const float d2 = __builtin_fmaf(dx, dx, dy * dy);
+                    atomicAdd(&hist[min(255, max(0, (int)(__float_as_uint(d2) >> 19) - BASE))], 1u);
+                }
+                if (rb + 64 == pq && q < NCP && pq < R) {
+                    wave_sync();
+                    const uint4 h = reinterpret_cast<const uint4 *>(hist)[lane];
+                    const int own = (int)(h.x + h.y + h.z + h.w);
+                    const int incl = wave_incl_scan(own), excl = incl - own;
+                    int jb = 0, before = excl;
+                    if (before + (int)h.x < K) { before += (int)h.x; jb = 1;
+                        if (before + (int)h.y < K) { before += (int)h.y; jb = 2;
+                            if (before + (int)h.z < K) { jb = 3; } } }
+                    const unsigned long long cross = __ballot(excl < K && incl >= K);
+                    const int Lc = __ffsll((long long)cross) - 1;
+                    const int bucket = 4 * Lc + __builtin_amdgcn_readlane(jb, Lc);
+                    const float T = bucket >= 255 ? __builtin_inff() : __uint_as_float((unsigned int)(bucket + 1 + BASE) << 19);
+                    if (lane == 0) {
+                        const float reach = sqrtf(T) * 1.0001f + 1e-3f;
+                        float thr = reach * reach * 1.0001f * mg * 1.001f;
+                        if (!(thr >= 0.f)) thr = __builtin_inff();
+                        b.first[q][al] = (unsigned short)min(pq, 65535);
+                        b.thr[q][al] = thr;
+                    }
+                    tlast = T;
+                    q++;
+                    pf *= ratio;
+                    pq = max(pq + 64, ((int)pf + 63) & ~63);
+                }
+            }
+            if (lane == 0) {
+                s.ncp[al] = q;
+                d.rk_rec[(size_t)w * A_T + a0 + al] = make_float4(0.f, tlast < 1e30f ? tlast : 1.f, __int_as_float(q | GD_RK_REC_ROW), 0.f);
+            }
+        }
+    }
+    __syncthreads();
+    {
+        unsigned short *rowf = d.rk_cpf + ((size_t)w * A_T + a0) * NCP;
+        float *rowt = d.rk_cpt + ((size_t)w * A_T + a0) * NCP;
+        for (int e = tid; e < 64 * NCP; e += 256) {
+            const int ag = e / NCP, q = e - ag * NCP;
+            if (q < s.ncp[ag]) {
+                rowf[e] = b.first[q][ag];
+                rowt[e] = b.thr[q][ag];
+            }
+        }
+    }
+    __syncthreads();
+}
+
+}
+}
+#endif
```

New measurement: 71.35 million (median of 6 runs). +1.3%, better.
